# ben-hayes/neural-waveshaping-synthesis

Measured on AMD Instinct MI355X. Metric: audio_samples_per_sec, higher is better.
Workload: dtype f32 (fp16x2-split MFMA contractions = 22-bit products, fp32 accumulate; FiLM interpolation bf16x3-split MFMA = exact fp32 operands); 1 GPU; NEWT forward, vn checkpoint, FastNEWT LUT, batch 64/GPU x 500 frames (4 s @ 16 kHz), torch.rand F0/control, RNG draws on device; batch_per_gpu=64, frames=500, samples_per_utterance=64000, parallelism=batch-shard x1, exciter_opts=0, streams=2

## Files before the change

include/nws_hip.h:

```cpp
#ifndef NWS_HIP_H
#define NWS_HIP_H

#include <stddef.h>
#include <stdint.h>

#ifdef __cplusplus
extern "C" {
#endif

#define NWS_ABI_VERSION 6

#define NWS_N_HARMONICS 101
#define NWS_N_SHAPERS 64
#define NWS_HIDDEN 128
#define NWS_HOP 128
#define NWS_FIR_LEN 256
#define NWS_N_BANDS 129
#define NWS_FIR_HALF 128
#define NWS_SHAPER_WIDTH 8
#define NWS_FILM_CH 256

enum {
  NWS_OK = 0,
  NWS_ERR_UNSUPPORTED = -1,
  NWS_ERR_BAD_ARG = -2,
  NWS_ERR_WORKSPACE = -3
};

typedef struct NwsWeights {
  const float* gru_w_ih;
  const float* gru_w_hh;
  const float* gru_b_ih;
  const float* gru_b_hh;
  const float* proj_w;
  const float* proj_b;
  const float* mixer_w;
  const float* mixer_b;
  const void* mixer_frags;
  const float* newt_mlp_w[4];
  const float* newt_mlp_b[4];
  const float* newt_ln_g[3];
  const float* newt_ln_b[3];
  const float* hgen_w[4];
  const float* hgen_b[4];
  const float* hgen_ln_g[3];
  const float* hgen_ln_b[3];
  const void* mlp_frags;
  const float* shaper_in_scale;
  const float* shaper_w0;
  const float* shaper_b0;
  const float* shaper_w2;
  const float* shaper_b2;
  const float* shaper_w4;
  const float* shaper_b4;
  const float* shaper_w6;
  const float* shaper_b6;
  const float* shaper_turns;
  const float* lut;
  const float* lut_pairs;
  int32_t lut_size;
  float lut_min;
  float lut_max;
  const float* newt_out_w;
  const float* newt_out_b;
  const float* noise_window;
  int32_t exciter_opts;
  const float* exciter_bound;
} NwsWeights;
#define NWS_EXCITER_VALU_FILM 1
#define NWS_EXCITER_ONE_TERM 2
#define NWS_EXCITER_HYBRID 4
#define NWS_EXCITER_HYBRID_W 8
#define NWS_EXCITER_BANK_NOFRACT 16

int nws_abi_version(void);
size_t nws_sizeof(int which);
const char* nws_error_string(int code);

int nws_selftest_mfma(int32_t* bad_out , void* stream);

int nws_sin(const float* x, float* y, int64_t n, void* stream);

int nws_phase_carry(const float* f0, const float* f0_up, int B, int T, double* carry , void* stream);

int nws_exciter_newt(const NwsWeights* w, const float* f0, const float* f0_up, const double* carry,
                     const float* phase_u, const float* rand_phase, const float* film, int B, int T,
                     float sample_rate, float* exciter_out, float* newt_out, void* stream);
int nws_exciter_newt_add(const NwsWeights* w, const float* f0, const float* f0_up, const double* carry,
                         const float* phase_u, const float* rand_phase, const float* film, const float* add_in, int B,
                         int T, float sample_rate, float* exciter_out, float* newt_out, void* stream);

int nws_control_gru(const NwsWeights* w, const float* control, int B, int C, int T, float* gru_out, void* stream);
int nws_control_gru_state(const NwsWeights* w, const float* control, int B, int C, int T, const float* h0, float* gru_out,
                          float* hT, void* stream);
int nws_control_gru_carry(const NwsWeights* w, const float* control, const float* f0, int B, int C, int T, float* gru_out,
                          double* carry_out, void* stream);
int nws_control_gru_batched(const NwsWeights* w, const float* control, int B, int C, int T, const float* h0, float* gru_out,
                            float* hT, void* stream);

int nws_frame_mlps(const NwsWeights* w, const float* gru_out, const float* fir_design, int B, int T,
                   float* emb_out, float* film_out, float* H_out, float* fir_out, void* stream);

#define NWS_MLP_FRAGS_BYTES 1474560
int nws_mlp_frags(const NwsWeights* w, const float* fir_design , void* frags_out, void* stream);

int nws_fir_design_matrix(const float* window , float* D_out, void* stream);

int nws_fir_noise(const float* fir , const float* noise , const float* add_in ,
                  int B, int T, float* out , void* stream);
int nws_fir_noise_window(const float* fir, const float* noise, int noise_len, int origin, const float* add_in, int B, int T,
                         float* out, void* stream);

int nws_fir_noise_grad(const float* noise , const float* grad_out , int B, int T,
                       float* grad_fir , void* stream);
int nws_fir_from_h_grad(const float* grad_fir , const float* fir_design , int B, int T,
                        float* grad_H , void* stream);
int nws_sum_batch_time(const float* x , int B, int C, int T, float* out , void* stream);

typedef struct NwsReverbPlan {
  int32_t L;
  int32_t N1;
  int32_t N2;
  int32_t Lc;
  int32_t hist;
  int32_t nblk;
  int32_t reserved[2];
} NwsReverbPlan;

int nws_reverb_plan(int N, int ir_len_plus1, NwsReverbPlan* plan );
int nws_reverb_plan_serves(const NwsReverbPlan* plan, int N, int ir_len_plus1);
size_t nws_reverb_table_bytes(const NwsReverbPlan* plan);
size_t nws_reverb_spectrum_bytes(const NwsReverbPlan* plan);
size_t nws_reverb_workspace_bytes(const NwsReverbPlan* plan, int B);
int nws_reverb_build_tables(const NwsReverbPlan* plan, void* tables, void* stream);
int nws_reverb_ir_spectrum(const NwsReverbPlan* plan, const void* tables, const float* ir, int ir_len,
                           void* spectrum, void* workspace, size_t workspace_bytes, void* stream);
int nws_reverb(const NwsReverbPlan* plan, const void* tables, const void* spectrum, const float* x ,
               int B, int N, float* y , void* workspace, size_t workspace_bytes, void* stream);

size_t nws_reverb_grad_workspace_bytes(const NwsReverbPlan* plan, int B, int want_ir);
int nws_reverb_grad_x(const NwsReverbPlan* plan, const void* tables, const void* spectrum, const float* g ,
                      int B, int N, float* dx , void* workspace, size_t workspace_bytes, void* stream);
int nws_reverb_grad_ir(const NwsReverbPlan* plan, const void* tables, const float* x , const float* g ,
                       int B, int N, int ir_len, float* dir , void* workspace, size_t workspace_bytes,
                       void* stream);

int nws_reverb_linear_chunk(const NwsReverbPlan* plan, const void* tables, const void* spectrum, const float* x, int B, int M,
                            const float* tail_in, float* tail_out, int tail_len, float* y, void* workspace,
                            size_t workspace_bytes, void* stream);

size_t nws_stream_state_bytes(int B, int max_frames, int ir_len, const NwsReverbPlan* plan);
int nws_stream_reset(void* state, size_t state_bytes, void* stream);
int nws_stream_out_samples(int K, int first, int final);
long long nws_stream_noise_start(int first, long long frames_seen);
int nws_stream_noise_draws(int K, int first, long long frames_seen);
int nws_stream_step(const NwsWeights* w, const float* fir_design, const NwsReverbPlan* plan, const void* reverb_tables,
                    const void* reverb_spectrum, void* state, size_t state_bytes, int B, int max_frames, const float* f0 ,
                    const float* control , int C, int K, int first, int final, long long frames_seen,
                    long long nz_prev_start, float sample_rate, const float* phase_u, const float* rand_phase,
                    const float* noise_new, const float* noise_all, int noise_all_len, const float* ir, int ir_len,
                    float* out , float* pre_out , void* stream);
int nws_stream_reverb_tail(const NwsReverbPlan* plan, const void* reverb_tables, const void* reverb_spectrum, void* state,
                           size_t state_bytes, int B, int max_frames, int ir_len, float* tail_out ,
                           void* workspace, size_t workspace_bytes, void* stream);

size_t nws_stream_counters_offset(int B, int max_frames, int ir_len);
size_t nws_stream_slot_state_bytes(int B, int max_frames, int ir_len);
#define NWS_SLOT_START 1
#define NWS_SLOT_STOP 2
#define NWS_SLOT_RELEASE 4
#define NWS_SLOT_ACTIVE 8
int nws_stream_step_slots(const NwsWeights* w, const float* fir_design, void* state, size_t state_bytes, int B, int max_frames,
                          const float* f0 , const float* control , int C, int K, long long frames_seen,
                          long long nz_prev_start, float sample_rate, const float* phase_u, const float* rand_phase,
                          const float* noise_new, const float* noise_all, int noise_all_len, const float* ir, int ir_len,
                          const int* events , float* out , float* pre_out ,
                          void* stream);

int nws_oscillator(const float* f0_up, const double* carry, const float* phase_u, const float* rand_phase, int B, int N,
                   float sample_rate, float* out, void* stream);
int nws_newt_apply(const NwsWeights* w, const float* exciter, const float* film, int B, int T, float* out, void* stream);
int nws_td_mlp(const float* x, int B, int in_size, int hidden, int out_size, int depth, int T, const float* const* w,
               const float* const* b, const float* const* ln_g, const float* const* ln_b, float ln_eps, float leaky_slope,
               float* y, void* stream);
size_t nws_td_mlp_grad_workspace_bytes(int B, int in_size, int hidden, int out_size, int depth, int T, int want_params);
int nws_td_mlp_grad(const float* x, const float* grad_y, int B, int in_size, int hidden, int out_size, int depth, int T,
                    const float* const* w, const float* const* b, const float* const* ln_g, const float* const* ln_b,
                    float ln_eps, float leaky_slope, float* grad_x , float* const* grad_w, float* const* grad_b,
                    float* const* grad_ln_g, float* const* grad_ln_b, void* workspace, size_t workspace_bytes, void* stream);
int nws_td_layer_norm(const float* x, const float* gain, const float* bias, int B, int C, int T, float eps, float* y,
                      void* stream);
int nws_film(const float* x, const float* gamma, const float* beta, int64_t n, float* y, void* stream);
int nws_fir_from_h(const float* H, const float* fir_design , int B, int T, float* fir_out, void* stream);

int nws_shaper_table(const NwsWeights* w, int table_size, float table_min, float table_max, float* table_out, void* stream);

#define NWS_MIXER_FRAGS_BYTES 28672
int nws_mixer_frags(const float* mixer_w, const float* mixer_b, void* frags_out, void* stream);
int nws_exciter_bound(const float* mixer_w, const float* mixer_b, float* bound_out , void* stream);
#define NWS_SHAPER_TURNS_ROW 176
int nws_shaper_turns(const NwsWeights* w, float* table_out , void* stream);

int nws_lut_pairs(const float* table , int table_size, float* pairs_out , void* stream);

int nws_shaper_apply(const NwsWeights* w, const float* x, int64_t B, int64_t N, float* y, void* stream);

typedef struct NwsForwardAux {
  const float* fir_design;
  const NwsReverbPlan* plan;
  const void* reverb_tables;
  const void* reverb_spectrum;
} NwsForwardAux;

size_t nws_forward_workspace_bytes(const NwsReverbPlan* plan, int B, int T);
int nws_forward(const NwsWeights* w, const NwsForwardAux* aux, const float* f0 , const float* control ,
                int B, int C, int T, float sample_rate, const float* phase_u, const float* rand_phase,
                const float* noise, float* out , void* workspace, size_t workspace_bytes, void* stream);

size_t nws_forward_control_bytes(int B, int T);
int nws_forward_control(const NwsWeights* w, const float* f0, const float* control, int B, int C, int T, int batched_gru,
                        void* workspace, size_t workspace_bytes, void* stream);
int nws_forward_audio(const NwsWeights* w, const NwsForwardAux* aux, const float* f0, int B, int T, float sample_rate,
                      const float* phase_u, const float* rand_phase, const float* noise, float* out, void* workspace,
                      size_t workspace_bytes, void* stream);

int nws_forward_audio_ev(const NwsWeights* w, const NwsForwardAux* aux, const float* f0, int B, int T, float sample_rate,
                         const float* phase_u, const float* rand_phase, const float* noise, float* out, void* workspace,
                         size_t workspace_bytes, void* stream, void* wait_before_exciter, void* record_after_exciter);

int nws_forward_audio_pre(const NwsWeights* w, const NwsForwardAux* aux, const float* f0, int B, int T, float sample_rate,
                          const float* phase_u, const float* rand_phase, const float* noise, void* workspace,
                          size_t workspace_bytes, void* stream);
int nws_forward_reverb_rows(const NwsForwardAux* aux, int B, int T, int row0, int nrows, float* out, void* workspace,
                            size_t workspace_bytes, void* stream);
int nws_forward_audio_blocks(const NwsWeights* w, const NwsForwardAux* aux, const float* f0, int B, int T, float sample_rate,
                             const float* phase_u, const float* rand_phase, const float* noise, float* out, void* workspace,
                             size_t workspace_bytes, void* stream, const int32_t* row0, const int32_t* nrows,
                             void* const* events , int nblocks);

size_t nws_loudness_dft_bytes(int n_fft);
int nws_loudness_dft_matrix(int n_fft, float* dft_out, void* stream);
int nws_loudness_frames(int N, int hop);
size_t nws_loudness_workspace_bytes(int B, int N, int n_fft, int hop);
int nws_loudness(const float* audio, int B, int N, int n_fft, int hop, const float* dft, float amin, float top_db,
                 int normalise, float* out, void* workspace, size_t workspace_bytes, void* stream);

int nws_pyin_frames(int N, int hop);
int nws_pyin_dims(double sample_rate, double fmin, double fmax, int frame_length, int hop, int32_t* dims);
size_t nws_pyin_table_bytes(double sample_rate, double fmin, double fmax, int frame_length, int hop);
int nws_pyin_table(double sample_rate, double fmin, double fmax, int frame_length, int hop, double* table_host);
size_t nws_pyin_workspace_bytes(int B, int N, double sample_rate, double fmin, double fmax, int frame_length, int hop);
int nws_pyin_cmnd(const float* audio, int B, int N, double sample_rate, double fmin, double fmax, int frame_length, int hop,
                  float* yin, void* stream);
int nws_pyin_observe(const float* yin, int B, int T, double sample_rate, double fmin, double fmax, int frame_length, int hop,
                     const double* table, int* cand_bin, double* cand_prob, int* count, double* voiced_prob, void* stream);
int nws_pyin_viterbi(const int* cand_bin, const double* cand_prob, const int* count, const double* voiced_prob, int B, int T,
                     double sample_rate, double fmin, double fmax, int frame_length, int hop, const double* table,
                     int fill_unvoiced, float fill_value, int* states, float* f0, void* workspace, size_t workspace_bytes,
                     void* stream);
int nws_pyin(const float* audio, int B, int N, double sample_rate, double fmin, double fmax, int frame_length, int hop,
             const double* table, int fill_unvoiced, float fill_value, float* f0, double* voiced_prob, int* states,
             void* workspace, size_t workspace_bytes, void* stream);

int nws_resample_dims(int sr_in, int sr_out, int32_t* dims);
int64_t nws_resample_length(int64_t N, int sr_in, int sr_out);
size_t nws_resample_bank_bytes(int sr_in, int sr_out);
int nws_resample_bank(int sr_in, int sr_out, float* bank_host);
int nws_resample(const float* x, int B, int N, int sr_in, int sr_out, const float* bank_dev, float* y, void* stream);

int nws_mfcc_dims(double sample_rate, int n_fft, int n_mfcc, int n_mels, int32_t* dims);
size_t nws_mfcc_table_bytes(double sample_rate, int n_fft, int n_mfcc, int n_mels);
int nws_mfcc_table(double sample_rate, int n_fft, int n_mfcc, int n_mels, float* table_host);
size_t nws_mfcc_workspace_bytes(int B, int N, int n_fft, int hop, int n_mels);
int nws_mfcc(const float* audio, int B, int N, double sample_rate, int n_fft, int hop, int n_mfcc, int n_mels, const float* dft,
             const float* table, float* out, void* workspace, size_t workspace_bytes, void* stream);

#define NWS_STFT_LOSS_MAX_RES 8
size_t nws_stft_loss_dft_bytes(int n_fft, int win_length);
int nws_stft_loss_dft_matrix(int n_fft, int win_length, float* dft_out, void* stream);
size_t nws_stft_loss_workspace_bytes(int B, int N, int R, const int* n_ffts, const int* hops);
int nws_stft_loss(const float* x, const float* y, int B, int N, int R, const int* n_ffts, const int* hops, const int* win_lengths,
                  const float* const* dfts, float w_sc, float w_log_mag, float w_lin_mag, float eps, float* out, void* workspace,
                  size_t workspace_bytes, void* stream);

size_t nws_stft_grad_workspace_bytes(int B, int N, int R, const int* n_ffts, const int* hops, const int* win_lengths);
int nws_stft_grad(const float* x, const float* y, int B, int N, int R, const int* n_ffts, const int* hops, const int* win_lengths,
                  const float* const* dfts, float w_sc, float w_log_mag, float w_lin_mag, float eps, float* grad_out, void* workspace,
                  size_t workspace_bytes, void* stream);

typedef struct NwsShaperDesc {
  int32_t n_shapers, width, depth, lut_size;
  float lut_min, lut_max;
  const float* in_scale;
  const float* w[8];
  const float* b[8];
  const float* lut;
} NwsShaperDesc;

typedef struct NwsGenericModel {
  int32_t control_size;
  int32_t gru_hidden, embedding, n_harmonics, n_shapers;
  int32_t hop;
  int32_t newt_mlp_depth;
  int32_t hgen_depth, hgen_hidden;
  int32_t fir_len;
  int32_t out_channels;
  int32_t ir_len;
  float ln_eps, leaky_slope;
  const float *gru_w_ih, *gru_w_hh, *gru_b_ih, *gru_b_hh;
  const float *proj_w, *proj_b;
  const float *mixer_w, *mixer_b;
  const float* newt_mlp_w[8];
  const float* newt_mlp_b[8];
  const float* newt_ln_g[8];
  const float* newt_ln_b[8];
  const float* hgen_w[8];
  const float* hgen_b[8];
  const float* hgen_ln_g[8];
  const float* hgen_ln_b[8];
  const float *newt_out_w, *newt_out_b;
  const float* noise_window;
  const float* ir;
  NwsShaperDesc shaper;
} NwsGenericModel;

size_t nws_g_gru_workspace_bytes(int hidden);
int nws_g_gru(const float* w_ih, const float* w_hh, const float* b_ih, const float* b_hh, const float* control, int B,
              int C_total, int C_in, int hidden, int T, const float* h0, float* out, float* hT, void* workspace,
              size_t workspace_bytes, void* stream);
int nws_g_bth_to_bht(const float* x, int B, int T, int H, float* y, void* stream);
int nws_g_phase(const float* f0, const float* f0_up, int B, int T, int hop, float sample_rate, float* f0_up_out,
                float* phase_out, void* stream);
int nws_g_upsample(const float* x, int64_t rows, int T, int hop, float* y, void* stream);
int nws_g_oscillator(const float* f0_up, const float* phase, const float* phase_u, const float* rand_phase, int K, int B, int N,
                     float sample_rate, float* out, void* stream);
int nws_g_conv1x1(const float* x, const float* w, const float* bias, int B, int Cin, int Cout, int N, float* y, void* stream);
int nws_g_shaper_apply(const NwsShaperDesc* d, const float* x, int64_t rows, int64_t N, float* y, void* stream);
int nws_g_shaper_table(const NwsShaperDesc* d, int table_size, float table_min, float table_max, float* table_out, void* stream);
int nws_g_film_shaper(const NwsShaperDesc* d, const float* exciter, const float* film, int B, int T, int hop, float* out,
                      void* stream);
int nws_g_fir_design(const float* H, const float* window, int fir_len, int B, int T, float* fir_out, void* stream);
int nws_g_fir_noise(const float* fir, const float* noise, int fir_len, int hop, int B, int T, const float* add_in,
                    int add_channels, float* out, void* stream);
int nws_g_reverb_direct(const float* x, const float* ir, int ir_len, int B, int N, float* y, void* stream);

size_t nws_forward_generic_workspace_bytes(const NwsGenericModel* m, int B, int T);
int nws_forward_generic(const NwsGenericModel* m, const float* f0, const float* control, int B, int C, int T, float sample_rate,
                        const float* phase_u, const float* rand_phase, const float* noise, const NwsReverbPlan* plan,
                        const void* reverb_tables, const void* reverb_spectrum, void* reverb_workspace,
                        size_t reverb_workspace_bytes, float* out, void* workspace, size_t workspace_bytes, void* stream);


#define NWS_N_STAGES 6
int nws_profile_begin(int slots, unsigned stage_mask);
int nws_profile_collect(float* ms_out , int* n_out );
int nws_profile_end(void);

int nws_peer_push(int n, void* const* dst, const void* src, size_t bytes, void* const* streams, void* const* events);
int nws_events_wait(int n, void* const* events);
int nws_streams_wait(int n, void* const* streams);

int nws_queue_probe(void* stream_hold, void* stream_touch, int groups, int spin_us, unsigned long long* scratch, float* frac_out );

#ifdef __cplusplus
}
#endif
#endif
```

neural-waveshaping-synthesis_amd/_cops.py:

```python
from __future__ import annotations

import ctypes as C

import torch

from . import _lib
from ._lib import NwsForwardAux, NwsGenericModel, NwsReverbPlan, NwsShaperDesc, NwsWeights, check, ptr

HOP = _lib.HOP


def _stream(dev):
    return torch.cuda.current_stream(dev).cuda_stream


def _struct(desc: torch.Tensor, cls):
    return cls.from_buffer_copy(desc.numpy())


def _plan(plan: torch.Tensor | None):
    return NwsReverbPlan(*plan.tolist()[:6]) if plan is not None else None


def _ref(struct):
    return C.byref(struct) if struct is not None else None


def _aux(fir_design, plan, tables, spectrum) -> NwsForwardAux:
    aux = NwsForwardAux()
    aux.fir_design = ptr(fir_design)
    aux.plan = C.pointer(_plan(plan))
    aux.reverb_tables = ptr(tables)
    aux.reverb_spectrum = ptr(spectrum)
    return aux


def _new(like: torch.Tensor, *shape, dtype=torch.float32):
    return torch.empty(shape, dtype=dtype, device=like.device)


def _ptrs(tensors):
    return (C.c_void_p * max(1, len(tensors)))(*[t.data_ptr() for t in tensors])


def _pyin_dims(cfg, table=None):
    dims = (C.c_int32 * 8)()
    L = _lib.lib()
    if L.nws_pyin_dims(*cfg, dims) != 0:
        raise RuntimeError(f"pyin: unsupported configuration (sample_rate, fmin, fmax, frame_length, hop) = {cfg}: at most 512 "
                           "lags (frame_length <= 1024), 1024 pitch bins and a transition window of 127; hop <= frame_length")
    n = L.nws_pyin_table_bytes(*cfg) // 8
    if isinstance(table, torch.Tensor) and (not table.is_cuda or table.dtype != torch.float64 or table.numel() != n):
        raise RuntimeError("pyin: table does not belong to this configuration (expected a float64 CUDA tensor of nws_pyin_table)")
    return (*dims, n)


def _resample_dims(sr_in, sr_out):
    dims = (C.c_int32 * 6)()
    if not (1 <= sr_in < 2 ** 31 and 1 <= sr_out < 2 ** 31) or _lib.lib().nws_resample_dims(sr_in, sr_out, dims) != 0:
        raise RuntimeError(f"resample: unsupported rates {sr_in} -> {sr_out}: integers >= 1 whose weight bank (sr_out / gcd rows) "
                           "stays below 64 MB")
    return tuple(dims)


def _mfcc_dims(sample_rate, n_fft, n_mfcc, n_mels):
    dims = (C.c_int32 * 8)()
    ok = all(0 <= v < 2 ** 31 for v in (n_fft, n_mfcc, n_mels))
    if not ok or _lib.lib().nws_mfcc_dims(sample_rate, n_fft, n_mfcc, n_mels, dims) != 0:
        raise RuntimeError(f"mfcc: unsupported configuration (sample_rate {sample_rate}, n_fft {n_fft}, n_mfcc {n_mfcc}, n_mels "
                           f"{n_mels}): sample_rate > 0, n_fft a power of two in [64, 2048], 1 <= n_mfcc <= n_mels <= 1024")
    return tuple(dims)


class CtypesOps:
    def abi_version(self):
        return int(_lib.lib().nws_abi_version())

    def forward(self, wdesc, f0, control, phase_u, rand_phase, noise, fir_design, plan, reverb_tables, reverb_spectrum,
                workspace, sample_rate):
        B, Cc, T = control.shape
        aux = _aux(fir_design, plan, reverb_tables, reverb_spectrum)
        with torch.cuda.device(f0.device):
            out = _new(f0, B, T * HOP)
            check(_lib.lib().nws_forward(C.byref(_struct(wdesc, NwsWeights)), C.byref(aux), ptr(f0), ptr(control), B, Cc, T,
                                         sample_rate, ptr(phase_u), ptr(rand_phase), ptr(noise), ptr(out), ptr(workspace),
                                         workspace.numel(), _stream(f0.device)), "nws_forward")
        return out

    def forward_control(self, wdesc, f0, control, workspace, batched_gru):
        B, Cc, T = control.shape
        with torch.cuda.device(f0.device):
            check(_lib.lib().nws_forward_control(C.byref(_struct(wdesc, NwsWeights)), ptr(f0), ptr(control), B, Cc, T,
                                                 1 if batched_gru else 0, ptr(workspace), workspace.numel(), _stream(f0.device)),
                  "nws_forward_control")

    def forward_audio(self, wdesc, f0, phase_u, rand_phase, noise, fir_design, plan, reverb_tables, reverb_spectrum, workspace,
                      sample_rate, out, wait_event, record_event):
        B, _, T = f0.shape
        aux = _aux(fir_design, plan, reverb_tables, reverb_spectrum)
        with torch.cuda.device(f0.device):
            if out is None:
                out = _new(f0, B, T * HOP)
            check(_lib.lib().nws_forward_audio_ev(C.byref(_struct(wdesc, NwsWeights)), C.byref(aux), ptr(f0), B, T, sample_rate,
                                                  ptr(phase_u), ptr(rand_phase), ptr(noise), ptr(out), ptr(workspace),
                                                  workspace.numel(), _stream(f0.device), wait_event or None, record_event or None),
                  "nws_forward_audio_ev")
        return out

    def forward_audio_pre(self, wdesc, f0, phase_u, rand_phase, noise, fir_design, plan, reverb_tables, reverb_spectrum,
                          workspace, sample_rate):
        B, _, T = f0.shape
        aux = _aux(fir_design, plan, reverb_tables, reverb_spectrum)
        with torch.cuda.device(f0.device):
            check(_lib.lib().nws_forward_audio_pre(C.byref(_struct(wdesc, NwsWeights)), C.byref(aux), ptr(f0), B, T, sample_rate,
                                                   ptr(phase_u), ptr(rand_phase), ptr(noise), ptr(workspace), workspace.numel(),
                                                   _stream(f0.device)), "nws_forward_audio_pre")

    def forward_audio_blocks(self, wdesc, f0, phase_u, rand_phase, noise, fir_design, plan, reverb_tables, reverb_spectrum,
                             workspace, sample_rate, out, row0, nrows, events):
        B, _, T = f0.shape
        n = len(row0)
        aux = _aux(fir_design, plan, reverb_tables, reverb_spectrum)
        with torch.cuda.device(f0.device):
            check(_lib.lib().nws_forward_audio_blocks(C.byref(_struct(wdesc, NwsWeights)), C.byref(aux), ptr(f0), B, T, sample_rate,
                                                      ptr(phase_u), ptr(rand_phase), ptr(noise), ptr(out), ptr(workspace),
                                                      workspace.numel(), _stream(f0.device), (C.c_int32 * n)(*row0),
                                                      (C.c_int32 * n)(*nrows), (C.c_void_p * n)(*events) if events else None, n),
                  "nws_forward_audio_blocks")

    def forward_reverb_rows(self, fir_design, plan, reverb_tables, reverb_spectrum, workspace, T, row0, nrows, out):
        aux = _aux(fir_design, plan, reverb_tables, reverb_spectrum)
        with torch.cuda.device(out.device):
            check(_lib.lib().nws_forward_reverb_rows(C.byref(aux), out.shape[0], T, row0, nrows, ptr(out), ptr(workspace),
                                                     workspace.numel(), _stream(out.device)), "nws_forward_reverb_rows")

    def phase_carry(self, f0, f0_up):
        src = f0 if f0 is not None else f0_up
        B = src.shape[0]
        T = src.shape[-1] if f0 is not None else src.shape[-1] // HOP
        with torch.cuda.device(src.device):
            carry = _new(src, B, T * HOP // 32, dtype=torch.float64)
            check(_lib.lib().nws_phase_carry(ptr(f0), ptr(f0_up), B, T, ptr(carry), _stream(src.device)), "nws_phase_carry")
        return carry

    def exciter_newt(self, wdesc, f0, f0_up, carry, phase_u, rand_phase, film, sample_rate, want_exciter, want_newt):
        src = f0 if f0 is not None else f0_up
        B = src.shape[0]
        T = src.shape[-1] if f0 is not None else src.shape[-1] // HOP
        with torch.cuda.device(src.device):
            exc = _new(src, B, _lib.N_SHAPERS, T * HOP) if want_exciter else None
            out = _new(src, B, T * HOP) if want_newt else None
            check(_lib.lib().nws_exciter_newt(C.byref(_struct(wdesc, NwsWeights)), ptr(f0), ptr(f0_up), ptr(carry), ptr(phase_u),
                                              ptr(rand_phase), ptr(film), B, T, sample_rate, ptr(exc), ptr(out),
                                              _stream(src.device)), "nws_exciter_newt")
        return exc, out

    def oscillator(self, f0_up, phase_u, rand_phase, sample_rate):
        B, N = f0_up.shape
        with torch.cuda.device(f0_up.device):
            st = _stream(f0_up.device)
            carry = _new(f0_up, B, N // 32, dtype=torch.float64)
            out = _new(f0_up, B, _lib.N_HARMONICS, N)
            check(_lib.lib().nws_phase_carry(None, ptr(f0_up), B, N // HOP, ptr(carry), st), "nws_phase_carry")
            check(_lib.lib().nws_oscillator(ptr(f0_up), ptr(carry), ptr(phase_u), ptr(rand_phase), B, N, sample_rate, ptr(out), st),
                  "nws_oscillator")
        return out

    def control_gru(self, wdesc, control, h0, batched):
        B, Cc, T = control.shape
        fn = _lib.lib().nws_control_gru_batched if batched else _lib.lib().nws_control_gru_state
        with torch.cuda.device(control.device):
            out = _new(control, B, T, _lib.HIDDEN)
            hT = _new(control, B, _lib.HIDDEN)
            check(fn(C.byref(_struct(wdesc, NwsWeights)), ptr(control), B, Cc, T, ptr(h0), ptr(out), ptr(hT),
                     _stream(control.device)), "nws_control_gru")
        return out, hT

    def frame_mlps(self, wdesc, gru_out, fir_design, want_emb, want_H):
        B, T, _ = gru_out.shape
        with torch.cuda.device(gru_out.device):
            emb = _new(gru_out, B, _lib.HIDDEN, T) if want_emb else None
            film = _new(gru_out, B, T, _lib.FILM_CH)
            H = _new(gru_out, B, T, _lib.N_BANDS) if want_H else None
            fir = _new(gru_out, B, T, _lib.FIR_HALF)
            check(_lib.lib().nws_frame_mlps(C.byref(_struct(wdesc, NwsWeights)), ptr(gru_out), ptr(fir_design), B, T, ptr(emb),
                                            ptr(film), ptr(H), ptr(fir), _stream(gru_out.device)), "nws_frame_mlps")
        return emb, film, H, fir

    def fir_noise(self, fir, noise, add_in, origin):
        B, T, _ = fir.shape
        with torch.cuda.device(fir.device):
            out = _new(fir, B, T * HOP)
            if origin < 0:
                check(_lib.lib().nws_fir_noise(ptr(fir), ptr(noise), ptr(add_in), B, T, ptr(out), _stream(fir.device)), "nws_fir_noise")
            else:
                check(_lib.lib().nws_fir_noise_window(ptr(fir), ptr(noise), noise.numel(), origin, ptr(add_in), B, T, ptr(out),
                                                      _stream(fir.device)), "nws_fir_noise_window")
        return out

    def fir_from_h(self, H, fir_design):
        B, _, T = H.shape
        with torch.cuda.device(H.device):
            fir = _new(H, B, T, _lib.FIR_HALF)
            check(_lib.lib().nws_fir_from_h(ptr(H), ptr(fir_design), B, T, ptr(fir), _stream(H.device)), "nws_fir_from_h")
        return fir

    def fir_noise_grad(self, noise, grad_out):
        B, N = grad_out.shape
        T = N // HOP
        if N != T * HOP or T < 2 or noise.numel() != N - 1:
            raise RuntimeError(f"fir_noise_grad: grad_out {tuple(grad_out.shape)} must be (B, 128 T) with T >= 2 and noise "
                               f"{tuple(noise.shape)} its {N - 1} samples")
        with torch.cuda.device(grad_out.device):
            grad_fir = _new(grad_out, B, T, _lib.FIR_HALF)
            check(_lib.lib().nws_fir_noise_grad(ptr(noise), ptr(grad_out), B, T, ptr(grad_fir), _stream(grad_out.device)),
                  "nws_fir_noise_grad")
        return grad_fir

    def fir_from_h_grad(self, grad_fir, fir_design):
        B, T, _ = grad_fir.shape
        with torch.cuda.device(grad_fir.device):
            grad_H = _new(grad_fir, B, _lib.N_BANDS, T)
            check(_lib.lib().nws_fir_from_h_grad(ptr(grad_fir), ptr(fir_design), B, T, ptr(grad_H), _stream(grad_fir.device)),
                  "nws_fir_from_h_grad")
        return grad_H

    def sum_batch_time(self, x):
        B, Cc, T = x.shape
        with torch.cuda.device(x.device):
            out = _new(x, Cc)
            check(_lib.lib().nws_sum_batch_time(ptr(x), B, Cc, T, ptr(out), _stream(x.device)), "nws_sum_batch_time")
        return out

    def reverb(self, plan, tables, spectrum, x):
        B, N = x.shape
        p = _plan(plan)
        with torch.cuda.device(x.device):
            nbytes = _lib.lib().nws_reverb_workspace_bytes(C.byref(p), B)
            ws = _new(x, nbytes, dtype=torch.uint8)
            y = torch.empty_like(x)
            check(_lib.lib().nws_reverb(C.byref(p), ptr(tables), ptr(spectrum), ptr(x), B, N, ptr(y), ptr(ws), nbytes,
                                        _stream(x.device)), "nws_reverb")
        return y

    def reverb_grad_x(self, plan, tables, spectrum, grad_out):
        B, N = grad_out.shape
        p = _plan(plan)
        with torch.cuda.device(grad_out.device):
            nbytes = _lib.lib().nws_reverb_grad_workspace_bytes(C.byref(p), B, 0)
            ws = _new(grad_out, nbytes, dtype=torch.uint8)
            dx = torch.empty_like(grad_out)
            check(_lib.lib().nws_reverb_grad_x(C.byref(p), ptr(tables), ptr(spectrum), ptr(grad_out), B, N, ptr(dx), ptr(ws), nbytes,
                                               _stream(grad_out.device)), "nws_reverb_grad_x")
        return dx

    def reverb_grad_ir(self, plan, tables, x, grad_out, ir_len):
        B, N = x.shape
        if tuple(grad_out.shape) != (B, N):
            raise RuntimeError(f"reverb_grad_ir: x {tuple(x.shape)} and grad_out {tuple(grad_out.shape)} differ in shape")
        p = _plan(plan)
        with torch.cuda.device(x.device):
            nbytes = _lib.lib().nws_reverb_grad_workspace_bytes(C.byref(p), B, 1)
            ws = _new(x, nbytes, dtype=torch.uint8)
            dir_ = _new(x, ir_len)
            check(_lib.lib().nws_reverb_grad_ir(C.byref(p), ptr(tables), ptr(x), ptr(grad_out), B, N, ir_len, ptr(dir_), ptr(ws),
                                                nbytes, _stream(x.device)), "nws_reverb_grad_ir")
        return dir_

    def reverb_linear_chunk(self, plan, tables, spectrum, x, tail_in):
        B, M = x.shape
        p = _plan(plan)
        with torch.cuda.device(x.device):
            nfl = (2 * ((B + 1) // 2) + B) * p.L
            ws = _new(x, nfl)
            y, tail_out = torch.empty_like(x), torch.empty_like(tail_in)
            check(_lib.lib().nws_reverb_linear_chunk(C.byref(p), ptr(tables), ptr(spectrum), ptr(x), B, M, ptr(tail_in),
                                                     ptr(tail_out), tail_in.shape[1], ptr(y), ptr(ws), nfl * 4, _stream(x.device)),
                  "nws_reverb_linear_chunk")
        return y, tail_out

    def shaper_apply(self, wdesc, x):
        with torch.cuda.device(x.device):
            y = torch.empty_like(x)
            check(_lib.lib().nws_shaper_apply(C.byref(_struct(wdesc, NwsWeights)), ptr(x), x.shape[0], x.shape[2], ptr(y),
                                              _stream(x.device)), "nws_shaper_apply")
        return y

    def shaper_table(self, wdesc, like, size, tmin, tmax):
        with torch.cuda.device(like.device):
            table = _new(like, _lib.N_SHAPERS, size)
            check(_lib.lib().nws_shaper_table(C.byref(_struct(wdesc, NwsWeights)), size, tmin, tmax, ptr(table), _stream(like.device)),
                  "nws_shaper_table")
        return table

    def newt_apply(self, wdesc, exciter, film):
        B, _, N = exciter.shape
        T = film.shape[2]
        if film.shape[1] != _lib.FILM_CH or N != T * HOP:
            raise RuntimeError(f"NEWT: exciter {tuple(exciter.shape)} and FiLM parameters {tuple(film.shape)} disagree")
        with torch.cuda.device(exciter.device):
            out = _new(exciter, B, 1, N)
            check(_lib.lib().nws_newt_apply(C.byref(_struct(wdesc, NwsWeights)), ptr(exciter), ptr(film), B, T, ptr(out),
                                            _stream(exciter.device)), "nws_newt_apply")
        return out

    def td_mlp(self, x, weights, biases, ln_w, ln_b, eps, slope):
        B, in_size, T = x.shape
        hidden, out_size = weights[0].shape[0], weights[-1].shape[0]
        with torch.cuda.device(x.device):
            y = _new(x, B, out_size, T)
            check(_lib.lib().nws_td_mlp(ptr(x), B, in_size, hidden, out_size, len(weights), T, _ptrs(weights), _ptrs(biases),
                                        _ptrs(ln_w), _ptrs(ln_b), eps, slope, ptr(y), _stream(x.device)), "nws_td_mlp")
        return y

    def td_mlp_grad(self, x, grad_y, weights, biases, ln_w, ln_b, eps, slope, want_params):
        B, in_size, T = x.shape
        depth = len(weights)
        hidden, out_size = weights[0].shape[0], weights[-1].shape[0]
        if tuple(grad_y.shape) != (B, out_size, T):
            raise RuntimeError(f"td_mlp_grad: grad_y {tuple(grad_y.shape)} is not ({B}, {out_size}, {T})")
        if len(biases) != depth or len(ln_w) != depth - 1 or len(ln_b) != depth - 1:
            raise RuntimeError("td_mlp_grad: inconsistent layer lists")
        L = _lib.lib()
        with torch.cuda.device(x.device):
            grad_x = torch.empty_like(x)
            gw, gb, gg, gl, ws, nbytes = [], [], [], [], None, 0
            if want_params:
                gw, gb = [torch.empty_like(t) for t in weights], [torch.empty_like(t) for t in biases]
                gg, gl = [torch.empty_like(t) for t in ln_w], [torch.empty_like(t) for t in ln_b]
                nbytes = L.nws_td_mlp_grad_workspace_bytes(B, in_size, hidden, out_size, depth, T, 1)
                ws = _new(x, max(nbytes, 1), dtype=torch.uint8)
            none = None
            check(L.nws_td_mlp_grad(ptr(x), ptr(grad_y), B, in_size, hidden, out_size, depth, T, _ptrs(weights), _ptrs(biases),
                                    _ptrs(ln_w), _ptrs(ln_b), eps, slope, ptr(grad_x), _ptrs(gw) if want_params else none,
                                    _ptrs(gb) if want_params else none, _ptrs(gg) if want_params else none,
                                    _ptrs(gl) if want_params else none, ptr(ws), nbytes, _stream(x.device)), "nws_td_mlp_grad")
        return [grad_x] + gw + gb + gg + gl

    def td_layer_norm(self, x, weight, bias, eps):
        with torch.cuda.device(x.device):
            y = torch.empty_like(x)
            check(_lib.lib().nws_td_layer_norm(ptr(x), ptr(weight), ptr(bias), x.shape[0], x.shape[1], x.shape[2], eps, ptr(y),
                                               _stream(x.device)), "nws_td_layer_norm")
        return y

    def film(self, x, gamma, beta):
        with torch.cuda.device(x.device):
            y = torch.empty_like(x)
            check(_lib.lib().nws_film(ptr(x), ptr(gamma), ptr(beta), x.numel(), ptr(y), _stream(x.device)), "nws_film")
        return y
# ... 321 lines not shown
```

neural-waveshaping-synthesis_amd/_lib.py:

```python
from __future__ import annotations

import ctypes as C
import os

_HERE = os.path.dirname(os.path.abspath(__file__))
LIB_PATH = os.path.join(_HERE, "libnws_hip.so")

PROBE_LIB_PATH = os.path.join(_HERE, "libnws_probe.so")

ABI_VERSION = 6
EXCITER_VALU_FILM = 1
EXCITER_ONE_TERM = 2
EXCITER_HYBRID = 4
EXCITER_HYBRID_W = 8
EXCITER_BANK_NOFRACT = 16
N_HARMONICS = 101
N_SHAPERS = 64
HIDDEN = 128
HOP = 128
FIR_LEN = 256
FIR_HALF = 128
MLP_FRAGS_BYTES = 1474560
N_BANDS = 129
FILM_CH = 256
SHAPER_WIDTH = 8
SHAPER_TURNS_ROW = 176
FIR_DESIGN_COLS = 132

_fp = C.c_void_p


class NwsWeights(C.Structure):
    _fields_ = [
        ("gru_w_ih", _fp), ("gru_w_hh", _fp), ("gru_b_ih", _fp), ("gru_b_hh", _fp),
        ("proj_w", _fp), ("proj_b", _fp),
        ("mixer_w", _fp), ("mixer_b", _fp), ("mixer_frags", _fp),
        ("newt_mlp_w", _fp * 4), ("newt_mlp_b", _fp * 4), ("newt_ln_g", _fp * 3), ("newt_ln_b", _fp * 3),
        ("hgen_w", _fp * 4), ("hgen_b", _fp * 4), ("hgen_ln_g", _fp * 3), ("hgen_ln_b", _fp * 3),
        ("mlp_frags", _fp),
        ("shaper_in_scale", _fp),
        ("shaper_w0", _fp), ("shaper_b0", _fp), ("shaper_w2", _fp), ("shaper_b2", _fp),
        ("shaper_w4", _fp), ("shaper_b4", _fp), ("shaper_w6", _fp), ("shaper_b6", _fp), ("shaper_turns", _fp),
        ("lut", _fp), ("lut_pairs", _fp), ("lut_size", C.c_int32), ("lut_min", C.c_float), ("lut_max", C.c_float),
        ("newt_out_w", _fp), ("newt_out_b", _fp),
        ("noise_window", _fp),
        ("exciter_opts", C.c_int32),
        ("exciter_bound", _fp),
    ]


class NwsReverbPlan(C.Structure):
    _fields_ = [("L", C.c_int32), ("N1", C.c_int32), ("N2", C.c_int32), ("Lc", C.c_int32), ("hist", C.c_int32), ("nblk", C.c_int32),
                ("reserved", C.c_int32 * 2)]

    def as_tensor(self):
        import torch
        return torch.tensor([self.L, self.N1, self.N2, self.Lc, self.hist, self.nblk, 0, 0], dtype=torch.int32)


class NwsForwardAux(C.Structure):
    _fields_ = [("fir_design", _fp), ("plan", C.POINTER(NwsReverbPlan)), ("reverb_tables", _fp),
                ("reverb_spectrum", _fp)]


class NwsShaperDesc(C.Structure):
    _fields_ = [("n_shapers", C.c_int32), ("width", C.c_int32), ("depth", C.c_int32), ("lut_size", C.c_int32),
                ("lut_min", C.c_float), ("lut_max", C.c_float),
                ("in_scale", _fp), ("w", _fp * 8), ("b", _fp * 8), ("lut", _fp)]


class NwsGenericModel(C.Structure):
    _fields_ = [("control_size", C.c_int32), ("gru_hidden", C.c_int32), ("embedding", C.c_int32), ("n_harmonics", C.c_int32),
                ("n_shapers", C.c_int32), ("hop", C.c_int32), ("newt_mlp_depth", C.c_int32), ("hgen_depth", C.c_int32),
                ("hgen_hidden", C.c_int32), ("fir_len", C.c_int32), ("out_channels", C.c_int32), ("ir_len", C.c_int32),
                ("ln_eps", C.c_float), ("leaky_slope", C.c_float),
                ("gru_w_ih", _fp), ("gru_w_hh", _fp), ("gru_b_ih", _fp), ("gru_b_hh", _fp),
                ("proj_w", _fp), ("proj_b", _fp), ("mixer_w", _fp), ("mixer_b", _fp),
                ("newt_mlp_w", _fp * 8), ("newt_mlp_b", _fp * 8), ("newt_ln_g", _fp * 8), ("newt_ln_b", _fp * 8),
                ("hgen_w", _fp * 8), ("hgen_b", _fp * 8), ("hgen_ln_g", _fp * 8), ("hgen_ln_b", _fp * 8),
                ("newt_out_w", _fp), ("newt_out_b", _fp), ("noise_window", _fp), ("ir", _fp),
                ("shaper", NwsShaperDesc)]


_PYIN_CFG = (C.c_double, C.c_double, C.c_double, C.c_int, C.c_int)

_MFCC_CFG = (C.c_double, C.c_int, C.c_int, C.c_int)

_PROTOTYPES = {
    "nws_abi_version": (C.c_int, []),
    "nws_sizeof": (C.c_size_t, [C.c_int]),
    "nws_error_string": (C.c_char_p, [C.c_int]),
    "nws_selftest_mfma": (C.c_int, [_fp, _fp]),
    "nws_peer_push": (C.c_int, [C.c_int, C.POINTER(C.c_void_p), _fp, C.c_size_t, C.POINTER(C.c_void_p), C.POINTER(C.c_void_p)]),
    "nws_events_wait": (C.c_int, [C.c_int, C.POINTER(C.c_void_p)]),
    "nws_streams_wait": (C.c_int, [C.c_int, C.POINTER(C.c_void_p)]),
    "nws_queue_probe": (C.c_int, [_fp, _fp, C.c_int, C.c_int, _fp, C.POINTER(C.c_float)]),
    "nws_debug_queue_busy": (C.c_int, [C.c_int, C.c_int, _fp, _fp]),
    "nws_sin": (C.c_int, [_fp, _fp, C.c_int64, _fp]),
    "nws_phase_carry": (C.c_int, [_fp, _fp, C.c_int, C.c_int, _fp, _fp]),
    "nws_exciter_newt": (C.c_int, [C.POINTER(NwsWeights), _fp, _fp, _fp, _fp, _fp, _fp, C.c_int, C.c_int, C.c_float,
                                   _fp, _fp, _fp]),
    "nws_exciter_newt_add": (C.c_int, [C.POINTER(NwsWeights), _fp, _fp, _fp, _fp, _fp, _fp, _fp, C.c_int, C.c_int, C.c_float,
                                       _fp, _fp, _fp]),
    "nws_control_gru": (C.c_int, [C.POINTER(NwsWeights), _fp, C.c_int, C.c_int, C.c_int, _fp, _fp]),
    "nws_control_gru_state": (C.c_int, [C.POINTER(NwsWeights), _fp, C.c_int, C.c_int, C.c_int, _fp, _fp, _fp, _fp]),
    "nws_control_gru_carry": (C.c_int, [C.POINTER(NwsWeights), _fp, _fp, C.c_int, C.c_int, C.c_int, _fp, _fp, _fp]),
    "nws_control_gru_batched": (C.c_int, [C.POINTER(NwsWeights), _fp, C.c_int, C.c_int, C.c_int, _fp, _fp, _fp, _fp]),
    "nws_frame_mlps": (C.c_int, [C.POINTER(NwsWeights), _fp, _fp, C.c_int, C.c_int, _fp, _fp, _fp, _fp, _fp]),
    "nws_mlp_frags": (C.c_int, [C.POINTER(NwsWeights), _fp, _fp, _fp]),
    "nws_debug_frame_mlps_kernel": (C.c_int, [C.c_int]),
    "nws_fir_design_matrix": (C.c_int, [_fp, _fp, _fp]),
    "nws_fir_noise": (C.c_int, [_fp, _fp, _fp, C.c_int, C.c_int, _fp, _fp]),
    "nws_fir_noise_window": (C.c_int, [_fp, _fp, C.c_int, C.c_int, _fp, C.c_int, C.c_int, _fp, _fp]),
    "nws_fir_noise_grad": (C.c_int, [_fp, _fp, C.c_int, C.c_int, _fp, _fp]),
    "nws_fir_from_h_grad": (C.c_int, [_fp, _fp, C.c_int, C.c_int, _fp, _fp]),
    "nws_sum_batch_time": (C.c_int, [_fp, C.c_int, C.c_int, C.c_int, _fp, _fp]),
    "nws_reverb_linear_chunk": (C.c_int, [C.POINTER(NwsReverbPlan), _fp, _fp, _fp, C.c_int, C.c_int, _fp, _fp, C.c_int, _fp, _fp,
                                          C.c_size_t, _fp]),
    "nws_reverb_plan": (C.c_int, [C.c_int, C.c_int, C.POINTER(NwsReverbPlan)]),
    "nws_reverb_plan_serves": (C.c_int, [C.POINTER(NwsReverbPlan), C.c_int, C.c_int]),
    "nws_reverb_table_bytes": (C.c_size_t, [C.POINTER(NwsReverbPlan)]),
    "nws_reverb_spectrum_bytes": (C.c_size_t, [C.POINTER(NwsReverbPlan)]),
    "nws_reverb_workspace_bytes": (C.c_size_t, [C.POINTER(NwsReverbPlan), C.c_int]),
    "nws_reverb_build_tables": (C.c_int, [C.POINTER(NwsReverbPlan), _fp, _fp]),
    "nws_reverb_ir_spectrum": (C.c_int, [C.POINTER(NwsReverbPlan), _fp, _fp, C.c_int, _fp, _fp, C.c_size_t, _fp]),
    "nws_reverb": (C.c_int, [C.POINTER(NwsReverbPlan), _fp, _fp, _fp, C.c_int, C.c_int, _fp, _fp, C.c_size_t, _fp]),
    "nws_reverb_grad_workspace_bytes": (C.c_size_t, [C.POINTER(NwsReverbPlan), C.c_int, C.c_int]),
    "nws_reverb_grad_x": (C.c_int, [C.POINTER(NwsReverbPlan), _fp, _fp, _fp, C.c_int, C.c_int, _fp, _fp, C.c_size_t, _fp]),
    "nws_reverb_grad_ir": (C.c_int, [C.POINTER(NwsReverbPlan), _fp, _fp, _fp, C.c_int, C.c_int, C.c_int, _fp, _fp, C.c_size_t, _fp]),
    "nws_shaper_table": (C.c_int, [C.POINTER(NwsWeights), C.c_int, C.c_float, C.c_float, _fp, _fp]),
    "nws_mixer_frags": (C.c_int, [_fp, _fp, _fp, _fp]),
    "nws_exciter_bound": (C.c_int, [_fp, _fp, _fp, _fp]),
    "nws_shaper_turns": (C.c_int, [_fp, _fp, _fp]),
    "nws_lut_pairs": (C.c_int, [_fp, C.c_int, _fp, _fp]),
    "nws_shaper_apply": (C.c_int, [C.POINTER(NwsWeights), _fp, C.c_int64, C.c_int64, _fp, _fp]),
    "nws_forward_workspace_bytes": (C.c_size_t, [C.POINTER(NwsReverbPlan), C.c_int, C.c_int]),
    "nws_forward": (C.c_int, [C.POINTER(NwsWeights), C.POINTER(NwsForwardAux), _fp, _fp, C.c_int, C.c_int, C.c_int,
                              C.c_float, _fp, _fp, _fp, _fp, _fp, C.c_size_t, _fp]),
    "nws_forward_control_bytes": (C.c_size_t, [C.c_int, C.c_int]),
    "nws_forward_control": (C.c_int, [C.POINTER(NwsWeights), _fp, _fp, C.c_int, C.c_int, C.c_int, C.c_int, _fp, C.c_size_t, _fp]),
    "nws_forward_audio": (C.c_int, [C.POINTER(NwsWeights), C.POINTER(NwsForwardAux), _fp, C.c_int, C.c_int, C.c_float,
                                    _fp, _fp, _fp, _fp, _fp, C.c_size_t, _fp]),
    "nws_forward_audio_ev": (C.c_int, [C.POINTER(NwsWeights), C.POINTER(NwsForwardAux), _fp, C.c_int, C.c_int, C.c_float,
                                       _fp, _fp, _fp, _fp, _fp, C.c_size_t, _fp, _fp, _fp]),
    "nws_forward_audio_pre": (C.c_int, [C.POINTER(NwsWeights), C.POINTER(NwsForwardAux), _fp, C.c_int, C.c_int, C.c_float,
                                        _fp, _fp, _fp, _fp, C.c_size_t, _fp]),
    "nws_forward_reverb_rows": (C.c_int, [C.POINTER(NwsForwardAux), C.c_int, C.c_int, C.c_int, C.c_int, _fp, _fp, C.c_size_t, _fp]),
    "nws_forward_audio_blocks": (C.c_int, [C.POINTER(NwsWeights), C.POINTER(NwsForwardAux), _fp, C.c_int, C.c_int, C.c_float, _fp, _fp, _fp, _fp,
                                           _fp, C.c_size_t, _fp, C.POINTER(C.c_int32), C.POINTER(C.c_int32), C.POINTER(C.c_void_p), C.c_int]),
    "nws_loudness_dft_bytes": (C.c_size_t, [C.c_int]),
    "nws_loudness_dft_matrix": (C.c_int, [C.c_int, _fp, _fp]),
    "nws_loudness_frames": (C.c_int, [C.c_int, C.c_int]),
    "nws_loudness_workspace_bytes": (C.c_size_t, [C.c_int, C.c_int, C.c_int, C.c_int]),
    "nws_loudness": (C.c_int, [_fp, C.c_int, C.c_int, C.c_int, C.c_int, _fp, C.c_float, C.c_float, C.c_int, _fp, _fp,
                               C.c_size_t, _fp]),
    "nws_pyin_frames": (C.c_int, [C.c_int, C.c_int]),
    "nws_pyin_dims": (C.c_int, [*_PYIN_CFG, C.POINTER(C.c_int32)]),
    "nws_pyin_table_bytes": (C.c_size_t, [*_PYIN_CFG]),
    "nws_pyin_table": (C.c_int, [*_PYIN_CFG, C.c_void_p]),
    "nws_pyin_workspace_bytes": (C.c_size_t, [C.c_int, C.c_int, *_PYIN_CFG]),
    "nws_pyin_cmnd": (C.c_int, [_fp, C.c_int, C.c_int, *_PYIN_CFG, _fp, _fp]),
    "nws_pyin_observe": (C.c_int, [_fp, C.c_int, C.c_int, *_PYIN_CFG, _fp, _fp, _fp, _fp, _fp, _fp]),
    "nws_pyin_viterbi": (C.c_int, [_fp, _fp, _fp, _fp, C.c_int, C.c_int, *_PYIN_CFG, _fp, C.c_int, C.c_float, _fp, _fp, _fp,
                                   C.c_size_t, _fp]),
    "nws_pyin": (C.c_int, [_fp, C.c_int, C.c_int, *_PYIN_CFG, _fp, C.c_int, C.c_float, _fp, _fp, _fp, _fp, C.c_size_t, _fp]),
    "nws_resample_dims": (C.c_int, [C.c_int, C.c_int, C.POINTER(C.c_int32)]),
    "nws_resample_length": (C.c_int64, [C.c_int64, C.c_int, C.c_int]),
    "nws_resample_bank_bytes": (C.c_size_t, [C.c_int, C.c_int]),
    "nws_resample_bank": (C.c_int, [C.c_int, C.c_int, C.c_void_p]),
    "nws_resample": (C.c_int, [_fp, C.c_int, C.c_int, C.c_int, C.c_int, _fp, _fp, _fp]),
    "nws_mfcc_dims": (C.c_int, [*_MFCC_CFG, C.POINTER(C.c_int32)]),
    "nws_mfcc_table_bytes": (C.c_size_t, [*_MFCC_CFG]),
    "nws_mfcc_table": (C.c_int, [*_MFCC_CFG, C.c_void_p]),
    "nws_mfcc_workspace_bytes": (C.c_size_t, [C.c_int, C.c_int, C.c_int, C.c_int, C.c_int]),
    "nws_mfcc": (C.c_int, [_fp, C.c_int, C.c_int, C.c_double, C.c_int, C.c_int, C.c_int, C.c_int, _fp, _fp, _fp, _fp, C.c_size_t,
                           _fp]),
    "nws_stft_loss_dft_bytes": (C.c_size_t, [C.c_int, C.c_int]),
    "nws_stft_loss_dft_matrix": (C.c_int, [C.c_int, C.c_int, _fp, _fp]),
    "nws_stft_loss_workspace_bytes": (C.c_size_t, [C.c_int, C.c_int, C.c_int, C.POINTER(C.c_int), C.POINTER(C.c_int)]),
    "nws_stft_loss": (C.c_int, [_fp, _fp, C.c_int, C.c_int, C.c_int, C.POINTER(C.c_int), C.POINTER(C.c_int), C.POINTER(C.c_int),
                                C.POINTER(_fp), C.c_float, C.c_float, C.c_float, C.c_float, _fp, _fp, C.c_size_t, _fp]),
    "nws_stft_grad_workspace_bytes": (C.c_size_t, [C.c_int, C.c_int, C.c_int, C.POINTER(C.c_int), C.POINTER(C.c_int),
                                                   C.POINTER(C.c_int)]),
    "nws_stft_grad": (C.c_int, [_fp, _fp, C.c_int, C.c_int, C.c_int, C.POINTER(C.c_int), C.POINTER(C.c_int), C.POINTER(C.c_int),
                                C.POINTER(_fp), C.c_float, C.c_float, C.c_float, C.c_float, _fp, _fp, C.c_size_t, _fp]),
    "nws_oscillator": (C.c_int, [_fp, _fp, _fp, _fp, C.c_int, C.c_int, C.c_float, _fp, _fp]),
    "nws_newt_apply": (C.c_int, [C.POINTER(NwsWeights), _fp, _fp, C.c_int, C.c_int, _fp, _fp]),
    "nws_td_mlp": (C.c_int, [_fp, C.c_int, C.c_int, C.c_int, C.c_int, C.c_int, C.c_int, C.POINTER(_fp), C.POINTER(_fp),
                             C.POINTER(_fp), C.POINTER(_fp), C.c_float, C.c_float, _fp, _fp]),
    "nws_td_mlp_grad_workspace_bytes": (C.c_size_t, [C.c_int, C.c_int, C.c_int, C.c_int, C.c_int, C.c_int, C.c_int]),
    "nws_td_mlp_grad": (C.c_int, [_fp, _fp, C.c_int, C.c_int, C.c_int, C.c_int, C.c_int, C.c_int, C.POINTER(_fp), C.POINTER(_fp),
                                  C.POINTER(_fp), C.POINTER(_fp), C.c_float, C.c_float, _fp, C.POINTER(_fp), C.POINTER(_fp),
                                  C.POINTER(_fp), C.POINTER(_fp), _fp, C.c_size_t, _fp]),
    "nws_td_layer_norm": (C.c_int, [_fp, _fp, _fp, C.c_int, C.c_int, C.c_int, C.c_float, _fp, _fp]),
    "nws_film": (C.c_int, [_fp, _fp, _fp, C.c_int64, _fp, _fp]),
    "nws_fir_from_h": (C.c_int, [_fp, _fp, C.c_int, C.c_int, _fp, _fp]),
    "nws_g_gru_workspace_bytes": (C.c_size_t, [C.c_int]),
    "nws_g_gru": (C.c_int, [_fp, _fp, _fp, _fp, _fp, C.c_int, C.c_int, C.c_int, C.c_int, C.c_int, _fp, _fp, _fp, _fp,
                            C.c_size_t, _fp]),
    "nws_g_bth_to_bht": (C.c_int, [_fp, C.c_int, C.c_int, C.c_int, _fp, _fp]),
    "nws_g_phase": (C.c_int, [_fp, _fp, C.c_int, C.c_int, C.c_int, C.c_float, _fp, _fp, _fp]),
    "nws_g_upsample": (C.c_int, [_fp, C.c_int64, C.c_int, C.c_int, _fp, _fp]),
    "nws_g_oscillator": (C.c_int, [_fp, _fp, _fp, _fp, C.c_int, C.c_int, C.c_int, C.c_float, _fp, _fp]),
    "nws_g_conv1x1": (C.c_int, [_fp, _fp, _fp, C.c_int, C.c_int, C.c_int, C.c_int, _fp, _fp]),
    "nws_g_shaper_apply": (C.c_int, [C.POINTER(NwsShaperDesc), _fp, C.c_int64, C.c_int64, _fp, _fp]),
    "nws_g_shaper_table": (C.c_int, [C.POINTER(NwsShaperDesc), C.c_int, C.c_float, C.c_float, _fp, _fp]),
    "nws_g_film_shaper": (C.c_int, [C.POINTER(NwsShaperDesc), _fp, _fp, C.c_int, C.c_int, C.c_int, _fp, _fp]),
    "nws_g_fir_design": (C.c_int, [_fp, _fp, C.c_int, C.c_int, C.c_int, _fp, _fp]),
    "nws_g_fir_noise": (C.c_int, [_fp, _fp, C.c_int, C.c_int, C.c_int, C.c_int, _fp, C.c_int, _fp, _fp]),
    "nws_g_reverb_direct": (C.c_int, [_fp, _fp, C.c_int, C.c_int, C.c_int, _fp, _fp]),
    "nws_forward_generic_workspace_bytes": (C.c_size_t, [C.POINTER(NwsGenericModel), C.c_int, C.c_int]),
    "nws_debug_generic_exciter_plan": (C.c_int, [C.POINTER(NwsGenericModel), C.c_int, C.c_int, C.POINTER(C.c_int)]),
    "nws_debug_generic_gru_plan": (C.c_int, [C.c_int, C.c_int, C.POINTER(C.c_int)]),
    "nws_forward_generic": (C.c_int, [C.POINTER(NwsGenericModel), _fp, _fp, C.c_int, C.c_int, C.c_int, C.c_float, _fp, _fp, _fp,
                                      C.POINTER(NwsReverbPlan), _fp, _fp, _fp, C.c_size_t, _fp, _fp, C.c_size_t, _fp]),
    "nws_stream_state_bytes": (C.c_size_t, [C.c_int, C.c_int, C.c_int, C.POINTER(NwsReverbPlan)]),
    "nws_stream_reset": (C.c_int, [_fp, C.c_size_t, _fp]),
    "nws_stream_out_samples": (C.c_int, [C.c_int, C.c_int, C.c_int]),
    "nws_stream_noise_start": (C.c_longlong, [C.c_int, C.c_longlong]),
    "nws_stream_noise_draws": (C.c_int, [C.c_int, C.c_int, C.c_longlong]),
    "nws_stream_step": (C.c_int, [C.POINTER(NwsWeights), _fp, C.POINTER(NwsReverbPlan), _fp, _fp, _fp, C.c_size_t, C.c_int, C.c_int,
                                  _fp, _fp, C.c_int, C.c_int, C.c_int, C.c_int, C.c_longlong, C.c_longlong, C.c_float, _fp, _fp,
                                  _fp, _fp, C.c_int, _fp, C.c_int, _fp, _fp, _fp]),
    "nws_stream_counters_offset": (C.c_size_t, [C.c_int, C.c_int, C.c_int]),
    "nws_stream_slot_state_bytes": (C.c_size_t, [C.c_int, C.c_int, C.c_int]),
    "nws_stream_step_slots": (C.c_int, [C.POINTER(NwsWeights), _fp, _fp, C.c_size_t, C.c_int, C.c_int, _fp, _fp, C.c_int, C.c_int,
                                        C.c_longlong, C.c_longlong, C.c_float, _fp, _fp, _fp, _fp, C.c_int, _fp, C.c_int, _fp, _fp,
                                        _fp, _fp]),
    "nws_stream_reverb_tail": (C.c_int, [C.POINTER(NwsReverbPlan), _fp, _fp, _fp, C.c_size_t, C.c_int, C.c_int, C.c_int, _fp, _fp,
                                         C.c_size_t, _fp]),
    "nws_profile_begin": (C.c_int, [C.c_int, C.c_uint]),
    "nws_profile_collect": (C.c_int, [C.POINTER(C.c_float), C.POINTER(C.c_int)]),
    "nws_profile_end": (C.c_int, []),
}

_PROBE_PROTOTYPES = {
    "nws_coexec_pk_probe": (C.c_int, [C.c_int, C.c_int, _fp, _fp]),
    "nws_coexec_pk_probe2": (C.c_int, [C.c_int, C.c_int, _fp, _fp]),
    "nws_coexec_pk_probe_mixed": (C.c_int, [C.c_int, C.c_int, C.c_int, _fp, _fp, _fp]),
    "nws_coexec_mfma_load": (C.c_int, [C.c_int, C.c_int, C.c_int, _fp, _fp]),
}

STAGE_NAMES = ("phase_carry", "control_gru", "frame_mlps", "exciter_newt", "fir_noise", "reverb")

EXPORTED_SYMBOLS = tuple(_PROTOTYPES)
PROBE_SYMBOLS = tuple(_PROBE_PROTOTYPES)

_lib = None
_probe = None


class NwsError(RuntimeError):
    pass


def lib():
    global _lib
    if _lib is None:
        if not os.path.exists(LIB_PATH):
            raise NwsError(
                f"{LIB_PATH} not found: build the HIP kernels first "
                "(python __graft_entry__.py build, or python neural-waveshaping-synthesis_amd/build.py). "
                "There is no CPU/PyTorch fallback for the NEWT forward path.")
        handle = C.CDLL(LIB_PATH)
        for name, (res, args) in _PROTOTYPES.items():
            fn = getattr(handle, name)
            fn.restype = res
            fn.argtypes = args
        if handle.nws_abi_version() != ABI_VERSION:
            raise NwsError(f"{LIB_PATH} has ABI version {handle.nws_abi_version()}, this package binds version "
                           f"{ABI_VERSION}: rebuild it (python __graft_entry__.py build)")
        for which, struct in enumerate((NwsWeights, NwsReverbPlan, NwsForwardAux, NwsShaperDesc, NwsGenericModel)):
            if handle.nws_sizeof(which) != C.sizeof(struct):
                raise NwsError(f"struct layout mismatch for {struct.__name__}: library {handle.nws_sizeof(which)} B, "
                               f"binding {C.sizeof(struct)} B")
        _lib = handle
    return _lib


def probe_lib():
    global _probe
    if _probe is None:
        if not os.path.exists(PROBE_LIB_PATH):
            raise NwsError(f"{PROBE_LIB_PATH} not found: python neural-waveshaping-synthesis_amd/build.py builds it next to libnws_hip.so")
        handle = C.CDLL(PROBE_LIB_PATH)
        for name, (res, args) in _PROBE_PROTOTYPES.items():
            fn = getattr(handle, name)
            fn.restype = res
            fn.argtypes = args
        _probe = handle
    return _probe


# ... 17 lines not shown
```

neural-waveshaping-synthesis_amd/csrc/fir_noise.hip:

```cpp
#include "nws_common.h"
#include "fir_spectral_fft.h"

template <>
struct SpOps<f32x2> {
  static __device__ __forceinline__ f32x2 fma(f32x2 a, f32x2 b, f32x2 c) { return __builtin_elementwise_fma(a, b, c); }
  static __device__ __forceinline__ f32x2 of(float v) { return f32x2{v, v}; }
  static __device__ __forceinline__ f32x2 at(const float* p) { return *reinterpret_cast<const f32x2*>(p); }
};

namespace {

constexpr int kL = NWS_FIR_LEN;
constexpr int kHop = NWS_HOP;
constexpr int kHalf = NWS_FIR_HALF;
constexpr int kHopsPerBlock = 4;

struct NoiseLds {
  float taps[kHopsPerBlock + 1][kL];
  float taps1[kHopsPerBlock + 1][kL];
  float sig[(kHopsPerBlock + 1) * kHop + kHop];
};

__device__ __forceinline__ float padded_noise(const float* __restrict__ noise, int len, int origin, int i) {
  int s = i - origin;
  if (s < 0) s = -s;
  if (s > len - 1) s = 2 * (len - 1) - s;
  s = s < 0 ? 0 : s;
  return noise[s];
}

__device__ __forceinline__ float row_noise(const float* __restrict__ noise, int lo, int hi, int origin, int i) {
  int s = i - origin;
  if (s < lo) s = 2 * lo - s;
  if (s > hi) s = 2 * hi - s;
  s = s < 0 ? 0 : s;
  return noise[s];
}

template <bool ROWS>
__global__ __launch_bounds__(256) void fir_noise_kernel(const float* __restrict__ fir, const float* __restrict__ noise,
                                                        const float* __restrict__ add_in, int T, int len, int origin,
                                                        float* __restrict__ out, const int4* __restrict__ rows) {
  __shared__ __attribute__((aligned(16))) NoiseLds L;
  const int tid = threadIdx.x, lane = tid & 63, wave = tid >> 6;
  const int half = lane >> 5, q = lane & 31;
  const int b = blockIdx.y;
  const int t0 = blockIdx.x * kHopsPerBlock;
  const int N = T * kHop;
  int4 rb = make_int4(0, 0, 0, 0);
  if constexpr (ROWS) rb = rows[b];
  const int t_lo = ROWS ? rb.z : 0;

  for (int e = tid; e < (kHopsPerBlock + 1) * kL; e += 256) {
    const int fr = e >> 8, k = e & 255;
    const int t = t0 - 1 + fr;
    const int d = k >= kHalf ? k - kHalf : kHalf - k;
    const float v = (t >= t_lo && t < T && d < kHalf) ? fir[((size_t)b * T + t) * kHalf + d] : 0.0f;
    L.taps[fr][k] = v;
    L.taps1[fr][(k + 1) & 255] = v;
  }
  for (int e = tid; e < (kHopsPerBlock + 1) * kHop + kHop; e += 256) {
    const int i = (t0 - 1) * kHop + e;
    float v = 0.0f;
    if (i >= 0 && i < N + kL - 1) v = ROWS ? row_noise(noise, rb.x, rb.y, origin, i) : padded_noise(noise, len, origin, i);
    L.sig[e] = v;
  }
  __syncthreads();

  const int t = t0 + wave;
  if (t >= T) return;
  const int slot = wave + 1 - half;
  const int nb = half * kHop + 4 * q;
  const float* f = &L.sig[slot * kHop];
  const float* h = L.taps[slot];

  const float* h1 = L.taps1[slot];
  f32x2 a0 = {0.0f, 0.0f}, a1 = {0.0f, 0.0f}, a2 = {0.0f, 0.0f}, a3 = {0.0f, 0.0f};
  float4 hi0 = *reinterpret_cast<const float4*>(&h[nb & 255]);
  float4 hi1 = *reinterpret_cast<const float4*>(&h1[nb & 255]);
#pragma unroll 4
  for (int m0 = 0; m0 < kL; m0 += 4) {
    const float4 lo0 = *reinterpret_cast<const float4*>(&h[(nb - m0 - 4) & 255]);
    const float4 lo1 = *reinterpret_cast<const float4*>(&h1[(nb - m0 - 4) & 255]);
    const float4 fv = *reinterpret_cast<const float4*>(&f[m0]);
    const f32x2 fs0 = {fv.y, fv.x}, fs1 = {fv.w, fv.z};
    a1 = fma2(fs0, f32x2{hi0.x, hi0.y}, a1);
    a3 = fma2(fs0, f32x2{hi0.z, hi0.w}, a3);
    a1 = fma2(fs1, f32x2{lo0.z, lo0.w}, a1);
    a3 = fma2(fs1, f32x2{hi0.x, hi0.y}, a3);
    a0 = fma2(fs0, f32x2{hi1.x, hi1.y}, a0);
    a2 = fma2(fs0, f32x2{hi1.z, hi1.w}, a2);
    a0 = fma2(fs1, f32x2{lo1.z, lo1.w}, a0);
    a2 = fma2(fs1, f32x2{hi1.x, hi1.y}, a2);
    hi0 = lo0;
    hi1 = lo1;
  }
  const float y0 = a0.x + a0.y, y1 = a1.x + a1.y, y2 = a2.x + a2.y, y3 = a3.x + a3.y;
  const float o0 = y0 + nws_swap_halves(y0);
  const float o1 = y1 + nws_swap_halves(y1);
  const float o2 = y2 + nws_swap_halves(y2);
  const float o3 = y3 + nws_swap_halves(y3);
  if (half == 0) {
    const float inv = t == t_lo ? 1.0f : 0.5f;
    const size_t o = (size_t)b * N + (size_t)t * kHop + 4 * q;
    float4 r = make_float4(o0 * inv, o1 * inv, o2 * inv, o3 * inv);
    if (add_in != nullptr) {
      const float4 a = *reinterpret_cast<const float4*>(&add_in[o]);
      r.x = a.x + r.x;
      r.y = a.y + r.y;
      r.z = a.z + r.z;
      r.w = a.w + r.w;
    }
    *reinterpret_cast<float4*>(&out[o]) = r;
  }
}

constexpr int kSpWaves = 4;
constexpr int kSpUtt = 2 * kSpWaves;
constexpr int kSpPairs = 4;
constexpr int kSpHops = 2 * kSpPairs - 1;

struct SpectralLds {
  float4 sd[kSpPairs][9][16];
  float4 tw[256];
  f32x2 x[kSpWaves][kSpPairs * kSpPlane];
};

__device__ __forceinline__ void sp_wave_sync() {
  __builtin_amdgcn_fence(__ATOMIC_RELEASE, "wavefront");
  __builtin_amdgcn_wave_barrier();
  __builtin_amdgcn_fence(__ATOMIC_ACQUIRE, "wavefront");
}

template <class T>
__device__ __forceinline__ void sp_transpose(T (&v)[16], T* x, int l) {
#pragma unroll
  for (int k = 0; k < 16; ++k) x[k * kSpRow + l] = v[k];
  sp_wave_sync();
#pragma unroll
  for (int j = 0; j < 16; ++j) v[j] = x[l * kSpRow + j];
  sp_wave_sync();
}
template <bool INV, class T>
__device__ __forceinline__ void sp_fft256(C16T<T>& z, const float* tw, T* x, int l) {
  sp_pass1<INV>(z, tw);
  sp_transpose(z.re, x, l);
  sp_transpose(z.im, x, l);
  sp_dft16<INV>(z);
}

__device__ __forceinline__ f32x2 sp_shfl(f32x2 v, int src) { return f32x2{__shfl(v.x, src, 64), __shfl(v.y, src, 64)}; }
__device__ __forceinline__ f32x2 sp_select(bool c, f32x2 a, f32x2 b) { return f32x2{c ? a.x : b.x, c ? a.y : b.y}; }

__device__ __forceinline__ void sp_filter_spectrum(C16T<f32x2>& z, const f32x2 (&ua)[8], const f32x2 (&ub)[8], const float* tw,
                                                   f32x2* x, int lane, int l) {
  const int src = (lane & 48) | ((16 - l) & 15);
  const f32x2 zero = {0.0f, 0.0f};
#pragma unroll
  for (int j = 0; j < 8; ++j) {
    z.re[j] = ua[j];
    z.im[j] = ub[j];
  }
#pragma unroll
  for (int j = 8; j < 16; ++j) {
    const f32x2 ma = sp_shfl(ua[15 - j], src), mb = sp_shfl(ub[15 - j], src);
    const f32x2 oa = j == 8 ? zero : ua[(16 - j) & 7], ob = j == 8 ? zero : ub[(16 - j) & 7];
    z.re[j] = sp_select(l == 0, oa, ma);
    z.im[j] = sp_select(l == 0, ob, mb);
  }
  sp_fft256<false>(z, tw, x, l);
}

__global__ __launch_bounds__(64 * kSpWaves, 3) void fir_noise_spectral_kernel(const float* __restrict__ fir,
                                                                             const float* __restrict__ noise,
                                                                             const float* __restrict__ add_in, int B, int T, int len,
                                                                             int origin, float* __restrict__ out, int nruns, int total) {
  __shared__ __attribute__((aligned(16))) SpectralLds L;
  const int tid = threadIdx.x, lane = tid & 63, wave = tid >> 6;
  const int g = lane >> 4, l = lane & 15;
  const int per_xcd = gridDim.x >> 3;
  const int id = (blockIdx.x & 7) * per_xcd + (blockIdx.x >> 3);
  if (id >= total) return;
  const int run = id % nruns;
  const int b0 = (id / nruns) * kSpUtt + 2 * wave, b1 = b0 + 1;
  const int t0 = run * kSpHops;
  const int ta = t0 - 1 + 2 * g, tb = ta + 1;
  const int N = T * kHop;
  const bool oka = ta >= 0 && ta < T, okb = tb < T;
  const int tac = ta < 0 ? 0 : (ta < T ? ta : T - 1), tbc = tb < T ? tb : T - 1;

  const int bc0 = b0 < B ? b0 : B - 1, bc1 = b1 < B ? b1 : B - 1;
  const float* rowa0 = &fir[((size_t)bc0 * T + tac) * kHalf + l];
  const float* rowb0 = &fir[((size_t)bc0 * T + tbc) * kHalf + l];
  const float* rowa1 = &fir[((size_t)bc1 * T + tac) * kHalf + l];
  const float* rowb1 = &fir[((size_t)bc1 * T + tbc) * kHalf + l];
  f32x2 ua[8], ub[8];
#pragma unroll
  for (int j = 0; j < 8; ++j) {
    ua[j] = f32x2{rowa0[16 * j], rowa1[16 * j]};
    ub[j] = f32x2{rowb0[16 * j], rowb1[16 * j]};
  }
  {
    float c, s;
    sp_twiddle((tid & 15) * (tid >> 4), c, s);
    L.tw[tid] = make_float4(c, c, s, s);
  }
  const float* tw = reinterpret_cast<const float*>(&L.tw[l]);
  __syncthreads();

  f32x2* x = &L.x[wave][g * kSpPlane];
  if (wave == 0) {
    C16 z;
    float* xs = reinterpret_cast<float*>(x);
#pragma unroll
    for (int j = 0; j < 16; ++j) {
      const int i0 = kHop * ta + 16 * j + l, i1 = i0 + kHop;
      const bool in0 = i0 >= 0 && i0 < N + kL - 1, in1 = i1 >= 0 && i1 < N + kL - 1;
      const float v0 = padded_noise(noise, len, origin, in0 ? i0 : origin);
      const float v1 = padded_noise(noise, len, origin, in1 ? i1 : origin);
      z.re[j] = in0 ? v0 : 0.0f;
      z.im[j] = in1 ? v1 : 0.0f;
    }
    sp_fft256<false>(z, tw, xs, l);
    float mr[16], mi[16];
    auto mirror = [&](const float (&v)[16], float (&m)[16]) {
#pragma unroll
      for (int j = 0; j < 16; ++j) xs[l + 16 * j] = v[j];
      sp_wave_sync();
#pragma unroll
      for (int j = 0; j < 16; ++j) m[j] = xs[(256 - (l + 16 * j)) & 255];
      sp_wave_sync();
    };
    mirror(z.re, mr);
    mirror(z.im, mi);
    const float c = (l & 1) ? -(1.0f / 512.0f) : (1.0f / 512.0f);
#pragma unroll
    for (int j = 0; j < 9; ++j)
      L.sd[g][j][l] = make_float4(c * (z.re[j] + mr[j]), c * (z.im[j] - mi[j]), c * (z.re[j] - mr[j]), c * (z.im[j] + mi[j]));
  }
  const f32x2 zero = {0.0f, 0.0f};
#pragma unroll
  for (int j = 0; j < 8; ++j) {
    ua[j] = sp_select(oka, ua[j], zero);
    ub[j] = sp_select(okb, ub[j], zero);
  }
  C16T<f32x2> z;
  sp_filter_spectrum(z, ua, ub, tw, x, lane, l);
  __syncthreads();

  const bool has_add = add_in != nullptr;
  const bool sta = g > 0 && ta < T, stb = tb < T;
  const size_t oa0 = (size_t)bc0 * N + (size_t)tac * kHop + l, ob0 = (size_t)bc0 * N + (size_t)tbc * kHop + l;
  const size_t oa1 = (size_t)bc1 * N + (size_t)tac * kHop + l, ob1 = (size_t)bc1 * N + (size_t)tbc * kHop + l;
  f32x2 adda[8], addb[8];
  if (has_add) {
#pragma unroll
    for (int j = 0; j < 8; ++j) {
      adda[j] = f32x2{add_in[oa0 + 16 * j], add_in[oa1 + 16 * j]};
      addb[j] = f32x2{add_in[ob0 + 16 * j], add_in[ob1 + 16 * j]};
    }
  }
  const float4* sdm = &L.sd[g][l == 0 ? 1 : 0][(16 - l) & 15];
#pragma unroll
  for (int j = 0; j < 16; ++j) {
    const f32x2 ga = z.re[j], gb = z.im[j];
    if (j < 9) {
      const float4 sd = L.sd[g][j][l];
      z.re[j] = f32x2{fmaf(ga.x, sd.x, gb.x * sd.z), fmaf(ga.y, sd.x, gb.y * sd.z)};
      z.im[j] = f32x2{fmaf(ga.x, sd.y, gb.x * sd.w), fmaf(ga.y, sd.y, gb.y * sd.w)};
    } else {
      const float4 sd = sdm[(15 - j) * 16];
      z.re[j] = f32x2{fmaf(ga.x, sd.x, -(gb.x * sd.z)), fmaf(ga.y, sd.x, -(gb.y * sd.z))};
      z.im[j] = f32x2{fmaf(gb.x, sd.w, -(ga.x * sd.y)), fmaf(gb.y, sd.w, -(ga.y * sd.y))};
    }
  }
  sp_fft256<true>(z, tw, x, l);
  const float invb = tb == 0 ? 1.0f : 0.5f;
  f32x2 ha[8], hb[8];
#pragma unroll
  for (int j = 0; j < 8; ++j) {
    const f32x2 ya0 = sp_select(oka, z.re[j], zero), ya1 = sp_select(oka, z.re[j + 8], zero);
    const f32x2 yb0 = sp_select(okb, z.im[j], zero), yb1 = sp_select(okb, z.im[j + 8], zero);
    const f32x2 prev = sp_shfl(yb1, (lane - 16) & 63);
    ha[j] = (ya0 + prev) * 0.5f;
    hb[j] = (yb0 + ya1) * invb;
    if (has_add) {
      ha[j] = adda[j] + ha[j];
      hb[j] = addb[j] + hb[j];
    }
  }
  if (sta) {
    if (b0 < B) {
#pragma unroll
      for (int j = 0; j < 8; ++j) out[oa0 + 16 * j] = ha[j].x;
    }
    if (b1 < B) {
#pragma unroll
      for (int j = 0; j < 8; ++j) out[oa1 + 16 * j] = ha[j].y;
    }
  }
  if (stb) {
    if (b0 < B) {
#pragma unroll
      for (int j = 0; j < 8; ++j) out[ob0 + 16 * j] = hb[j].x;
    }
    if (b1 < B) {
#pragma unroll
      for (int j = 0; j < 8; ++j) out[ob1 + 16 * j] = hb[j].y;
    }
  }
}

}

extern "C" int nws_fir_noise_window(const float* fir, const float* noise, int noise_len, int origin, const float* add_in,
                                    int B, int T, float* out, void* stream) {
  if (!fir || !noise || !out || B <= 0 || T <= 0 || noise_len < 2 || origin < 0) return NWS_ERR_BAD_ARG;
  if (B > 65535) return NWS_ERR_UNSUPPORTED;
  if (B >= 16) {
    const long long nruns = (T + kSpHops - 1) / kSpHops, total = nruns * ((B + kSpUtt - 1) / kSpUtt);
    if (total > (1ll << 30)) return NWS_ERR_UNSUPPORTED;
    const dim3 grid((unsigned)(8 * ((total + 7) / 8)));
    fir_noise_spectral_kernel<<<grid, 64 * kSpWaves, 0, (hipStream_t)stream>>>(fir, noise, add_in, B, T, noise_len, origin, out,
                                                                             (int)nruns, (int)total);
    NWS_CHECK_LAUNCH();
    return NWS_OK;
  }
  const dim3 grid((T + kHopsPerBlock - 1) / kHopsPerBlock, B);
  fir_noise_kernel<false><<<grid, 256, 0, (hipStream_t)stream>>>(fir, noise, add_in, T, noise_len, origin, out, nullptr);
  NWS_CHECK_LAUNCH();
  return NWS_OK;
}

extern "C" int nws_fir_noise_window_rows(const float* fir, const float* noise, int origin, const int4* rows, int B, int T,
                                         float* out, void* stream) {
  if (!fir || !noise || !out || !rows || B <= 0 || T <= 0 || origin < 0) return NWS_ERR_BAD_ARG;
  if (B > 65535) return NWS_ERR_UNSUPPORTED;
  const dim3 grid((T + kHopsPerBlock - 1) / kHopsPerBlock, B);
  fir_noise_kernel<true><<<grid, 256, 0, (hipStream_t)stream>>>(fir, noise, nullptr, T, 0, origin, out, rows);
  NWS_CHECK_LAUNCH();
  return NWS_OK;
}

extern "C" int nws_fir_noise(const float* fir, const float* noise, const float* add_in, int B, int T, float* out,
                             void* stream) {
  return nws_fir_noise_window(fir, noise, T * kHop - 1, kL / 2, add_in, B, T, out, stream);
}
```

neural-waveshaping-synthesis_amd/csrc/forward.hip:

```cpp
#include "nws_common.h"

namespace {

struct Carve {
  char* p;
  size_t left;
  bool ok = true;
  void* take(size_t bytes) {
    bytes = (bytes + 255) & ~size_t(255);
    if (bytes > left) {
      ok = false;
      return nullptr;
    }
    void* r = p;
    p += bytes;
    left -= bytes;
    return r;
  }
};

size_t aligned(size_t b) { return (b + 255) & ~size_t(255); }

constexpr int kStages = 6;
struct Profile {
  int slots = 0;
  int used = 0;
  unsigned mask = 0;
  hipEvent_t* ev = nullptr;
} g_prof;

inline hipEvent_t* prof_events(int stage) {
  if (g_prof.ev == nullptr || g_prof.used >= g_prof.slots || !(g_prof.mask & (1u << stage))) return nullptr;
  return g_prof.ev + ((size_t)g_prof.used * kStages + stage) * 2;
}

}

extern "C" {

size_t nws_forward_workspace_bytes(const NwsReverbPlan* plan, int B, int T) {
  if (!plan || B <= 0 || T <= 0) return 0;
  const size_t N = (size_t)T * NWS_HOP;
  size_t total = 0;
  total += aligned((size_t)B * (N / 32) * sizeof(double));
  total += aligned((size_t)B * T * NWS_HIDDEN * sizeof(float));
  total += aligned((size_t)B * T * NWS_FILM_CH * sizeof(float));
  total += aligned((size_t)B * T * NWS_FIR_HALF * sizeof(float));
  total += aligned((size_t)B * N * sizeof(float));
  total += aligned((size_t)B * N * sizeof(float));
  total += aligned(nws_reverb_workspace_bytes(plan, B));
  return total;
}

}

namespace {

struct Arena {
  double* carry;
  float *gru_out, *film, *fir, *noise_out, *pre;
  void* rv_ws;
  size_t rv_bytes;
  bool ok;
};

Arena carve_arena(const NwsReverbPlan* plan, void* workspace, size_t bytes, int B, int T, bool head_only) {
  const size_t N = (size_t)T * NWS_HOP;
  Carve cv{static_cast<char*>(workspace), bytes};
  Arena a{};
  a.carry = static_cast<double*>(cv.take((size_t)B * (N / 32) * sizeof(double)));
  a.gru_out = static_cast<float*>(cv.take((size_t)B * T * NWS_HIDDEN * sizeof(float)));
  if (!head_only) {
    a.film = static_cast<float*>(cv.take((size_t)B * T * NWS_FILM_CH * sizeof(float)));
    a.fir = static_cast<float*>(cv.take((size_t)B * T * NWS_FIR_HALF * sizeof(float)));
    a.noise_out = static_cast<float*>(cv.take((size_t)B * N * sizeof(float)));
    a.pre = static_cast<float*>(cv.take((size_t)B * N * sizeof(float)));
    a.rv_bytes = nws_reverb_workspace_bytes(plan, B);
    a.rv_ws = cv.take(a.rv_bytes);
  }
  a.ok = cv.ok;
  return a;
}

#define NWS_STAGE(idx, call)                                   \
  do {                                                         \
    hipEvent_t* e__ = prof_events(idx);                        \
    if (e__) (void)hipEventRecord(e__[0], st);                 \
    rc = (call);                                               \
    if (e__) (void)hipEventRecord(e__[1], st);                 \
    if (rc != NWS_OK) return rc;                               \
  } while (0)

int control_half(const NwsWeights* w, const float* f0, const float* control, int B, int C, int T, int batched_gru,
                 const Arena& a, void* stream) {
  hipStream_t st = (hipStream_t)stream;
  int rc = NWS_OK;
  if (batched_gru) {
    NWS_STAGE(0, nws_phase_carry(f0, nullptr, B, T, a.carry, stream));
    NWS_STAGE(1, nws_control_gru_batched(w, control, B, C, T, nullptr, a.gru_out, nullptr, stream));
  } else {
    NWS_STAGE(0, NWS_OK);
    NWS_STAGE(1, nws_control_gru_carry(w, control, f0, B, C, T, a.gru_out, a.carry, stream));
  }
  return NWS_OK;
}

int audio_half(const NwsWeights* w, const NwsForwardAux* aux, const float* f0, int B, int T, float sample_rate,
               const float* phase_u, const float* rand_phase, const float* noise, float* out, const Arena& a, void* stream,
               void* wait_before_exciter = nullptr, void* record_after_exciter = nullptr, bool with_reverb = true) {
  hipStream_t st = (hipStream_t)stream;
  int rc = NWS_OK;
  const size_t N = (size_t)T * NWS_HOP;
  NWS_STAGE(2, nws_frame_mlps(w, a.gru_out, aux->fir_design, B, T, nullptr, a.film, nullptr, a.fir, stream));
  NWS_STAGE(4, nws_fir_noise(a.fir, noise, nullptr, B, T, a.noise_out, stream));
  if (wait_before_exciter != nullptr) {
    const hipError_t e = hipStreamWaitEvent(st, (hipEvent_t)wait_before_exciter, 0);
    if (e != hipSuccess) return (int)e;
  }
  NWS_STAGE(3, nws_exciter_newt_add(w, f0, nullptr, a.carry, phase_u, rand_phase, a.film, a.noise_out, B, T, sample_rate, nullptr, a.pre, stream));
  if (record_after_exciter != nullptr) {
    const hipError_t e = hipEventRecord((hipEvent_t)record_after_exciter, st);
    if (e != hipSuccess) return (int)e;
  }
  if (with_reverb)
    NWS_STAGE(5, nws_reverb(aux->plan, aux->reverb_tables, aux->reverb_spectrum, a.pre, B, (int)N, out, a.rv_ws, a.rv_bytes, stream));
  if (g_prof.ev != nullptr && g_prof.used < g_prof.slots) ++g_prof.used;
  return NWS_OK;
}
#undef NWS_STAGE

bool aux_ok(const NwsForwardAux* aux) {
  return aux && aux->plan && aux->fir_design && aux->reverb_tables && aux->reverb_spectrum;
}

}

extern "C" {

size_t nws_sizeof(int which) {
  switch (which) {
    case 0: return sizeof(NwsWeights);
    case 1: return sizeof(NwsReverbPlan);
    case 2: return sizeof(NwsForwardAux);
    case 3: return sizeof(NwsShaperDesc);
    case 4: return sizeof(NwsGenericModel);
    default: return 0;
  }
}

size_t nws_forward_control_bytes(int B, int T) {
  if (B <= 0 || T <= 0) return 0;
  const size_t N = (size_t)T * NWS_HOP;
  return aligned((size_t)B * (N / 32) * sizeof(double)) + aligned((size_t)B * T * NWS_HIDDEN * sizeof(float));
}

int nws_forward(const NwsWeights* w, const NwsForwardAux* aux, const float* f0, const float* control, int B, int C,
                int T, float sample_rate, const float* phase_u, const float* rand_phase, const float* noise, float* out,
                void* workspace, size_t workspace_bytes, void* stream) {
  if (!w || !aux_ok(aux)) return NWS_ERR_BAD_ARG;
  if (!f0 || !control || !phase_u || !rand_phase || !noise || !out || !workspace) return NWS_ERR_BAD_ARG;
  if (B <= 0 || T < 2 || C < 2) return NWS_ERR_BAD_ARG;
  if (T > (1 << 23) || !nws_reverb_plan_serves(aux->plan, T * NWS_HOP, 0)) return NWS_ERR_BAD_ARG;
  const Arena a = carve_arena(aux->plan, workspace, workspace_bytes, B, T, false);
  if (!a.ok) return NWS_ERR_WORKSPACE;
  const int rc = control_half(w, f0, control, B, C, T, 0, a, stream);
  if (rc != NWS_OK) return rc;
  return audio_half(w, aux, f0, B, T, sample_rate, phase_u, rand_phase, noise, out, a, stream);
}

int nws_forward_control(const NwsWeights* w, const float* f0, const float* control, int B, int C, int T, int batched_gru,
                        void* workspace, size_t workspace_bytes, void* stream) {
  if (!w || !f0 || !control || !workspace) return NWS_ERR_BAD_ARG;
  if (B <= 0 || T < 2 || C < 2) return NWS_ERR_BAD_ARG;
  const Arena a = carve_arena(nullptr, workspace, workspace_bytes, B, T, true);
  if (!a.ok) return NWS_ERR_WORKSPACE;
  return control_half(w, f0, control, B, C, T, batched_gru, a, stream);
}

int nws_forward_audio(const NwsWeights* w, const NwsForwardAux* aux, const float* f0, int B, int T, float sample_rate,
                      const float* phase_u, const float* rand_phase, const float* noise, float* out, void* workspace,
                      size_t workspace_bytes, void* stream) {
  if (!w || !aux_ok(aux)) return NWS_ERR_BAD_ARG;
  if (!f0 || !phase_u || !rand_phase || !noise || !out || !workspace) return NWS_ERR_BAD_ARG;
  if (B <= 0 || T < 2) return NWS_ERR_BAD_ARG;
  if (T > (1 << 23) || !nws_reverb_plan_serves(aux->plan, T * NWS_HOP, 0)) return NWS_ERR_BAD_ARG;
  const Arena a = carve_arena(aux->plan, workspace, workspace_bytes, B, T, false);
  if (!a.ok) return NWS_ERR_WORKSPACE;
  return audio_half(w, aux, f0, B, T, sample_rate, phase_u, rand_phase, noise, out, a, stream);
}

int nws_forward_audio_ev(const NwsWeights* w, const NwsForwardAux* aux, const float* f0, int B, int T, float sample_rate,
                         const float* phase_u, const float* rand_phase, const float* noise, float* out, void* workspace,
                         size_t workspace_bytes, void* stream, void* wait_before_exciter, void* record_after_exciter) {
  if (!w || !aux_ok(aux)) return NWS_ERR_BAD_ARG;
  if (!f0 || !phase_u || !rand_phase || !noise || !out || !workspace) return NWS_ERR_BAD_ARG;
  if (B <= 0 || T < 2) return NWS_ERR_BAD_ARG;
  if (T > (1 << 23) || !nws_reverb_plan_serves(aux->plan, T * NWS_HOP, 0)) return NWS_ERR_BAD_ARG;
  const Arena a = carve_arena(aux->plan, workspace, workspace_bytes, B, T, false);
  if (!a.ok) return NWS_ERR_WORKSPACE;
  return audio_half(w, aux, f0, B, T, sample_rate, phase_u, rand_phase, noise, out, a, stream, wait_before_exciter,
                    record_after_exciter);
}

int nws_forward_audio_pre(const NwsWeights* w, const NwsForwardAux* aux, const float* f0, int B, int T, float sample_rate,
                          const float* phase_u, const float* rand_phase, const float* noise, void* workspace,
                          size_t workspace_bytes, void* stream) {
  if (!w || !aux_ok(aux)) return NWS_ERR_BAD_ARG;
  if (!f0 || !phase_u || !rand_phase || !noise || !workspace) return NWS_ERR_BAD_ARG;
  if (B <= 0 || T < 2) return NWS_ERR_BAD_ARG;
  if (T > (1 << 23) || !nws_reverb_plan_serves(aux->plan, T * NWS_HOP, 0)) return NWS_ERR_BAD_ARG;
  const Arena a = carve_arena(aux->plan, workspace, workspace_bytes, B, T, false);
  if (!a.ok) return NWS_ERR_WORKSPACE;
  return audio_half(w, aux, f0, B, T, sample_rate, phase_u, rand_phase, noise, nullptr, a, stream, nullptr, nullptr, false);
}

int nws_forward_reverb_rows(const NwsForwardAux* aux, int B, int T, int row0, int nrows, float* out ,
                            void* workspace, size_t workspace_bytes, void* stream) {
  if (!aux_ok(aux) || !out || !workspace || B <= 0 || T < 2 || row0 < 0 || nrows <= 0 || row0 + nrows > B) return NWS_ERR_BAD_ARG;
  const Arena a = carve_arena(aux->plan, workspace, workspace_bytes, B, T, false);
  if (!a.ok) return NWS_ERR_WORKSPACE;
  const size_t N = (size_t)T * NWS_HOP;
  if (row0 & 1) return NWS_ERR_BAD_ARG;
  const size_t per_pair = 2 * (size_t)aux->plan->nblk * (size_t)aux->plan->L * sizeof(float);
  char* rv = static_cast<char*>(a.rv_ws) + (size_t)(row0 / 2) * per_pair;
  const size_t left = a.rv_bytes - (size_t)(row0 / 2) * per_pair;
  return nws_reverb(aux->plan, aux->reverb_tables, aux->reverb_spectrum, a.pre + (size_t)row0 * N, nrows, (int)N, out + (size_t)row0 * N, rv,
                    left, stream);
}

int nws_forward_audio_blocks(const NwsWeights* w, const NwsForwardAux* aux, const float* f0, int B, int T, float sample_rate,
                             const float* phase_u, const float* rand_phase, const float* noise, float* out, void* workspace,
                             size_t workspace_bytes, void* stream, const int32_t* row0, const int32_t* nrows, void* const* events,
                             int nblocks) {
  if (!row0 || !nrows || nblocks <= 0 || !out) return NWS_ERR_BAD_ARG;
  int next = 0;
  for (int q = 0; q < nblocks; ++q) {
    if (row0[q] != next || nrows[q] <= 0 || ((nrows[q] & 1) && q != nblocks - 1)) return NWS_ERR_BAD_ARG;
    next += nrows[q];
  }
  if (next != B) return NWS_ERR_BAD_ARG;
  int rc = nws_forward_audio_pre(w, aux, f0, B, T, sample_rate, phase_u, rand_phase, noise, workspace, workspace_bytes, stream);
  if (rc != NWS_OK) return rc;
  for (int q = 0; q < nblocks; ++q) {
    rc = nws_forward_reverb_rows(aux, B, T, row0[q], nrows[q], out, workspace, workspace_bytes, stream);
    if (rc != NWS_OK) return rc;
    if (events != nullptr && events[q] != nullptr) {
      const hipError_t e = hipEventRecord((hipEvent_t)events[q], (hipStream_t)stream);
      if (e != hipSuccess) return (int)e;
    }
  }
  return NWS_OK;
}

int nws_profile_begin(int slots, unsigned stage_mask) {
  nws_profile_end();
  if (slots <= 0) return NWS_ERR_BAD_ARG;
  g_prof.ev = new hipEvent_t[(size_t)slots * kStages * 2];
  for (size_t i = 0; i < (size_t)slots * kStages * 2; ++i) {
    hipError_t e = hipEventCreateWithFlags(&g_prof.ev[i], hipEventDisableSystemFence);
    if (e != hipSuccess) return (int)e;
  }
  g_prof.slots = slots;
  g_prof.used = 0;
  g_prof.mask = stage_mask;
  return NWS_OK;
}

int nws_profile_collect(float* ms_out, int* n_out) {
  if (!ms_out || !n_out) return NWS_ERR_BAD_ARG;
  const int n = g_prof.used;
  for (int i = 0; i < n; ++i)
    for (int s = 0; s < kStages; ++s) {
      float ms = -1.0f;
      if (g_prof.mask & (1u << s)) {
        hipEvent_t* e = g_prof.ev + ((size_t)i * kStages + s) * 2;
        hipError_t err = hipEventSynchronize(e[1]);
        if (err != hipSuccess) return (int)err;
        err = hipEventElapsedTime(&ms, e[0], e[1]);
        if (err != hipSuccess) return (int)err;
      }
      ms_out[(size_t)i * kStages + s] = ms;
    }
  *n_out = n;
  g_prof.used = g_prof.slots;
  return NWS_OK;
}

int nws_profile_end(void) {
  if (g_prof.ev != nullptr) {
    for (size_t i = 0; i < (size_t)g_prof.slots * kStages * 2; ++i) (void)hipEventDestroy(g_prof.ev[i]);
    delete[] g_prof.ev;
  }
  g_prof = Profile();
  return NWS_OK;
}

}
```

neural-waveshaping-synthesis_amd/csrc/nws_common.h:

```cpp
#pragma once

#include <hip/hip_runtime.h>
#include <stdint.h>

#include "../../include/nws_hip.h"
#include "../../include/nws_hip_debug.h"

#define NWS_WAVE 64

typedef float f32x2 __attribute__((ext_vector_type(2)));
typedef float f32x4 __attribute__((ext_vector_type(4)));
typedef float f32x16 __attribute__((ext_vector_type(16)));

#define NWS_CHECK_LAUNCH()                      \
  do {                                          \
    hipError_t e__ = hipGetLastError();         \
    if (e__ != hipSuccess) return (int)e__;     \
  } while (0)

inline bool nws_first_use_on_device(unsigned long long& mask) {
  int d = 0;
  if (hipGetDevice(&d) != hipSuccess || d < 0 || d > 63) return true;
  if ((mask >> d) & 1ull) return false;
  mask |= 1ull << d;
// ... 215 lines not shown
  }
  hs[tid] = 256 * p + tid < ir_len ? ir[256 * p + tid] : 0.0f;
  __syncthreads();
  float acc0 = 0.0f, acc1 = 0.0f;
#pragma unroll 8
  for (int i = 0; i < 256; i += 4) {
    const float4 h4 = *reinterpret_cast<const float4*>(&hs[i]);
    acc0 = nws_fma_scalar(h4.x, xs[tid + 255 - i], acc0);
    acc1 = nws_fma_scalar(h4.y, xs[tid + 254 - i], acc1);
    acc0 = nws_fma_scalar(h4.z, xs[tid + 253 - i], acc0);
    acc1 = nws_fma_scalar(h4.w, xs[tid + 252 - i], acc1);
  }
  return nws_add_scalar(acc0, acc1);
}

struct NwsStreamNoiseWin {
  float* nzwin;
  const float* noise_new;
  const float* noise_all;
  long long* counters;
  int nz_shift, nz_keep, n_new, noise_all_len, first, K;
};
template <int NT, bool ADVANCE = true>
__device__ __forceinline__ void nws_stream_noise_window_block(const NwsStreamNoiseWin& Z, int tid) {
  const int Tw = Z.first ? Z.K : Z.K + 1;
  const long long F = Z.counters[1] + Z.counters[3];
  __syncthreads();
  if (ADVANCE && tid == 0) {
    Z.counters[0] += Z.counters[2];
    Z.counters[1] = F;
    Z.counters[2] = 0;
    Z.counters[3] = 0;
  }
  if (Z.noise_all != nullptr) {
    const long long A0 = Z.first ? 0 : F - 1;
    const long long start = A0 <= 0 ? 0 : 128 * (A0 - 1);
    const int want = 128 * (Tw + 1) + 1;
    for (int i = tid; i < want; i += NT) Z.nzwin[i] = start + i < Z.noise_all_len ? Z.noise_all[start + i] : 0.0f;
  } else {
    for (int i0 = 0; i0 < Z.nz_keep; i0 += NT) {
      const int i = i0 + tid;
      const float v = i < Z.nz_keep ? Z.nzwin[i + Z.nz_shift] : 0.0f;
      __syncthreads();
      if (i < Z.nz_keep) Z.nzwin[i] = v;
      __syncthreads();
    }
    for (int i = tid; i < Z.n_new; i += NT) Z.nzwin[Z.nz_keep + i] = Z.noise_new[i];
  }
}

struct NwsStreamSide {
  const float* ring;
  const float* ir;
  float* partial;
  const long long* counters;
  int ir_len, M, B, parts;
  const float* f0_new;
  float* prev_f0;
  const float* prev_film;
  const float* prev_fir;
  double* S;
  float* f0_w;
  float* film_w;
  float* fir_w;
  double* carry;
  int K, first, final;
  long long* gru_flag;
  long long* counters_rw;
  const float* gru_out;
  int out_T, out_off;
  NwsStreamNoiseWin win;
  const int* ev;
  int* vage;
  int4* nzrows;
  float* film_junk;
  float* fir_junk;
  int n_len;
};

__device__ __forceinline__ void nws_stream_head_block_slots(const NwsStreamSide& H, int b, int tid, double* wave_tot) {
  const int K = H.K, Tw = H.first ? K : K + 1, off = H.first ? 0 : 1;
  const int e = H.ev[b];
  for (int i = tid; i < Tw; i += 256) {
    int s;
    if (e & NWS_SLOT_RELEASE) s = -1;
    else if (!(e & NWS_SLOT_ACTIVE)) s = -2;
    else if (e & NWS_SLOT_START) s = i < off ? 0 : i - off;
    else s = i < off ? -1 : i - off;
    H.f0_w[(size_t)b * Tw + i] = s >= 0 ? H.f0_new[(size_t)b * K + s] : (s == -1 ? H.prev_f0[b] : 0.0f);
  }
  const bool hold = (e & NWS_SLOT_RELEASE) != 0;
  const int rows = !(e & NWS_SLOT_ACTIVE) ? Tw : ((e & NWS_SLOT_START) ? 0 : off);
  for (int i = tid; i < rows * NWS_FILM_CH; i += 256) {
    const int c = i % NWS_FILM_CH;
    H.film_w[(size_t)b * Tw * NWS_FILM_CH + i] = (hold || (e & NWS_SLOT_ACTIVE)) ? H.prev_film[(size_t)b * NWS_FILM_CH + c] : 0.0f;
  }
  for (int i = tid; i < rows * NWS_FIR_HALF; i += 256) {
    const int c = i % NWS_FIR_HALF;
    H.fir_w[(size_t)b * Tw * NWS_FIR_HALF + i] = (hold || (e & NWS_SLOT_ACTIVE)) ? H.prev_fir[(size_t)b * NWS_FIR_HALF + c] : 0.0f;
  }
  if (tid == 0) {
    const int age = (e & NWS_SLOT_START) ? 0 : H.vage[b];
    const int lo = 256 - 128 * (age < 2 ? age : 2);
    const int hi = (e & NWS_SLOT_STOP) ? 128 * (Tw + 1) - 2 : H.n_len - 1;
    const bool live = !H.first && (e & NWS_SLOT_ACTIVE);
    H.nzrows[b] = make_int4(live ? lo : 0, live ? hi : H.n_len - 1, (!H.first && (e & NWS_SLOT_START)) ? 1 : 0, 0);
    H.vage[b] = (e & NWS_SLOT_ACTIVE) ? (age + K < (1 << 20) ? age + K : (1 << 20)) : 0;
  }
  __syncthreads();
  if (tid == 0) H.prev_f0[b] = H.f0_w[(size_t)b * Tw + Tw - 1];
  nws_phase_carry_block<4>(H.f0_w, nullptr, Tw, H.carry, b, tid, wave_tot);
  __syncthreads();
  const int nch = 4 * Tw;
  double* cb = H.carry + (size_t)b * nch;
  if (!H.first) {
    const bool start = (e & NWS_SLOT_START) != 0;
    const double base = start ? cb[4] : cb[2], s0 = start ? 0.0 : H.S[b];
    __syncthreads();
    for (int c = tid; c < nch; c += 256) cb[c] = start ? cb[c] - base : s0 + (cb[c] - base);
    __syncthreads();
  }
  if (!H.final && tid == 0) H.S[b] = cb[nch - 2];
}

__device__ __forceinline__ void nws_stream_head_block(const NwsStreamSide& H, int b, int tid, double* wave_tot) {
  if (H.ev != nullptr) {
    nws_stream_head_block_slots(H, b, tid, wave_tot);
    return;
  }
  const int K = H.K, Tw = H.first ? K : K + 1, off = H.first ? 0 : 1;
  for (int i = tid; i < Tw; i += 256) H.f0_w[(size_t)b * Tw + i] = (i < off) ? H.prev_f0[b] : H.f0_new[(size_t)b * K + i - off];
  if (off) {
    for (int c = tid; c < NWS_FILM_CH; c += 256) H.film_w[(size_t)b * Tw * NWS_FILM_CH + c] = H.prev_film[(size_t)b * NWS_FILM_CH + c];
    for (int c = tid; c < NWS_FIR_HALF; c += 256) H.fir_w[(size_t)b * Tw * NWS_FIR_HALF + c] = H.prev_fir[(size_t)b * NWS_FIR_HALF + c];
  }
  __syncthreads();
  if (tid == 0) H.prev_f0[b] = H.f0_new[(size_t)b * K + K - 1];
  nws_phase_carry_block<4>(H.f0_w, nullptr, Tw, H.carry, b, tid, wave_tot);
  __syncthreads();
  const int nch = 4 * Tw;
  double* cb = H.carry + (size_t)b * nch;
  if (!H.first) {
    const double base = cb[2], s0 = H.S[b];
    __syncthreads();
    for (int c = tid; c < nch; c += 256) cb[c] = s0 + (cb[c] - base);
    __syncthreads();
  }
  if (!H.final && tid == 0) H.S[b] = cb[nch - 2];
}

extern "C" __attribute__((visibility("hidden"))) int nws_fir_noise_window_rows(const float* fir, const float* noise, int origin,
                                                                               const int4* rows, int B, int T, float* out,
                                                                               void* stream);
extern "C" __attribute__((visibility("hidden"))) int nws_control_gru_stream(const NwsWeights* w, const float* control, int B, int C,
                                                                            int T, const float* h0, float* gru_out, float* hT,
                                                                            const NwsStreamSide* side, void* stream);
extern "C" __attribute__((visibility("hidden"))) int nws_frame_mlps_stream(const NwsWeights* w, const float* gru_out, int B, int T,
                                                                           float* film_w, float* fir_w, int out_T, int out_off,
                                                                           const NwsStreamNoiseWin* win, void* stream);
extern "C" __attribute__((visibility("hidden"))) int nws_stft_power_pass(const float* audio, int B, int N, int n_fft, int hop,
                                                                         const float* dft, float* power, unsigned* max_bits,
                                                                         void* stream);
```

neural-waveshaping-synthesis_amd/csrc/torch_ops.cpp:

```cpp
#include <ATen/ATen.h>
#include <ATen/hip/impl/HIPGuardImplMasqueradingAsCUDA.h>
#include <ATen/hip/impl/HIPStreamMasqueradingAsCUDA.h>
#include <torch/library.h>

#include <algorithm>
#include <cstdlib>
#include <tuple>
#include <vector>

#include "../../include/nws_hip.h"
#include "../../include/nws_hip_debug.h"

namespace {

using at::Tensor;
using OptTensor = c10::optional<at::Tensor>;

const NwsWeights* weights_of(const Tensor& wdesc) {
  TORCH_CHECK(wdesc.device().is_cpu() && wdesc.scalar_type() == at::kByte && wdesc.is_contiguous() &&
                  (size_t)wdesc.numel() == sizeof(NwsWeights),
              "wdesc: expected a contiguous CPU uint8 tensor of ", sizeof(NwsWeights), " bytes (one NwsWeights struct), got ",
              wdesc.sizes(), " ", wdesc.scalar_type(), " on ", wdesc.device());
  return reinterpret_cast<const NwsWeights*>(wdesc.data_ptr());
}

void check_dev(const Tensor& t, const char* name, at::ScalarType st = at::kFloat) {
  TORCH_CHECK(t.is_cuda(), name, " lives on ", t.device(),
              ": the NEWT forward path only runs as HIP kernels on an AMD GPU (there is no CPU fallback)");
  TORCH_CHECK(t.scalar_type() == st, name, ": expected ", st, ", got ", t.scalar_type());
  TORCH_CHECK(t.is_contiguous(), name, ": expected a contiguous tensor");
}

void check_same_device(const Tensor& a, const char* an, const Tensor& b, const char* bn) {
  TORCH_CHECK(a.device() == b.device(), an, " is on ", a.device(), " but ", bn, " is on ", b.device(),
              ": all tensors of one call must live on the same GPU");
}

void nws_check(int rc, const char* what) {
  TORCH_CHECK(rc == NWS_OK, what, " failed (", rc, "): ", nws_error_string(rc));
}

const float* fptr(const OptTensor& t) { return t.has_value() ? t->data_ptr<float>() : nullptr; }

struct Launch {
  c10::hip::HIPGuardMasqueradingAsCUDA guard;
  void* stream;
  explicit Launch(const Tensor& t)
      : guard(t.device()), stream(c10::hip::getCurrentHIPStreamMasqueradingAsCUDA(t.device().index()).stream()) {}
};

NwsReverbPlan plan_of(const Tensor& plan) {
  TORCH_CHECK(plan.device().is_cpu() && plan.scalar_type() == at::kInt && plan.is_contiguous() && plan.numel() == 8,
              "plan: expected a CPU int32 tensor [L, N1, N2, Lc, hist, nblk, 0, 0] (the NwsReverbPlan of nws_reverb_plan)");
  const int32_t* p = plan.data_ptr<int32_t>();
  return NwsReverbPlan{p[0], p[1], p[2], p[3], p[4], p[5], {p[6], p[7]}};
}

void check_reverb_buffers(const NwsReverbPlan& plan, const Tensor& tables, const Tensor& spectrum) {
  TORCH_CHECK(plan.L > 0 && plan.N1 > 0 && plan.N2 > 0 && (int64_t)plan.N1 * plan.N2 == plan.L, "plan: inconsistent [L, N1, N2] = [",
              plan.L, ", ", plan.N1, ", ", plan.N2, "]");
  TORCH_CHECK((size_t)tables.numel() * tables.element_size() == nws_reverb_table_bytes(&plan), "reverb_tables: ",
              (size_t)tables.numel() * tables.element_size(), " bytes, the plan (L = ", plan.L, ") needs ", nws_reverb_table_bytes(&plan));
  TORCH_CHECK((size_t)spectrum.numel() * spectrum.element_size() == nws_reverb_spectrum_bytes(&plan), "reverb_spectrum: ",
              (size_t)spectrum.numel() * spectrum.element_size(), " bytes, the plan (L = ", plan.L, ") needs ",
              nws_reverb_spectrum_bytes(&plan), " (Sre | Sim | ir_)");
}

struct Aux {
  NwsReverbPlan plan;
  NwsForwardAux aux;
  Aux(const Tensor& fir_design, const Tensor& plan_t, const Tensor& tables, const Tensor& spectrum) : plan(plan_of(plan_t)) {
    check_dev(fir_design, "fir_design");
    check_dev(tables, "reverb_tables");
    check_dev(spectrum, "reverb_spectrum");
    TORCH_CHECK(fir_design.numel() == NWS_FIR_LEN * 132, "fir_design: expected (256, 132)");
    check_reverb_buffers(plan, tables, spectrum);
    aux.fir_design = fir_design.data_ptr<float>();
    aux.plan = &plan;
    aux.reverb_tables = tables.data_ptr();
    aux.reverb_spectrum = spectrum.data_ptr();
  }
};

void check_inputs(const Tensor& f0, const Tensor& control, int64_t& B, int64_t& C, int64_t& T) {
  check_dev(f0, "f0");
  check_dev(control, "control");
  check_same_device(f0, "f0", control, "control");
  TORCH_CHECK(f0.dim() == 3 && f0.size(1) == 1, "f0: expected (B, 1, T), got ", f0.sizes());
  TORCH_CHECK(control.dim() == 3 && control.size(1) >= 2, "control: expected (B, C>=2, T), got ", control.sizes());
  B = f0.size(0);
  T = f0.size(2);
  C = control.size(1);
  TORCH_CHECK(control.size(0) == B && control.size(2) == T, "f0 ", f0.sizes(), " and control ", control.sizes(),
              " disagree on batch / frames");
  TORCH_CHECK(T >= 2, "need at least 2 control frames (reflect padding of the noise STFT, generators.py:31)");
}

void check_draws(const Tensor& phase_u, const Tensor& rand_phase, const Tensor& noise, int64_t T, const Tensor& like) {
  check_dev(phase_u, "phase_u");
  check_dev(rand_phase, "rand_phase");
  check_dev(noise, "noise");
  check_same_device(like, "f0", phase_u, "phase_u");
  check_same_device(like, "f0", noise, "noise");
  check_same_device(like, "f0", rand_phase, "osc.rand_phase");
  TORCH_CHECK(phase_u.numel() == NWS_N_HARMONICS, "phase_u: expected 101 elements, got ", phase_u.sizes());
  TORCH_CHECK(rand_phase.numel() == NWS_N_HARMONICS, "rand_phase: expected 101 elements, got ", rand_phase.sizes());
  TORCH_CHECK(noise.numel() == NWS_HOP * T - 1, "noise: expected ", NWS_HOP * T - 1, " elements, got ", noise.sizes());
}

struct AudioShape {
  int64_t B, T;
  AudioShape(const Tensor& f0, const Tensor& phase_u, const Tensor& rand_phase, const Tensor& noise, const Tensor& workspace) {
    check_dev(f0, "f0");
    TORCH_CHECK(f0.dim() == 3 && f0.size(1) == 1 && f0.size(2) >= 2, "f0: expected (B, 1, T>=2), got ", f0.sizes());
    B = f0.size(0);
    T = f0.size(2);
    check_draws(phase_u, rand_phase, noise, T, f0);
    check_dev(workspace, "workspace", at::kByte);
    check_same_device(f0, "f0", workspace, "workspace");
  }
};

struct AudioArgs : AudioShape, Aux {
  AudioArgs(const Tensor& f0, const Tensor& phase_u, const Tensor& rand_phase, const Tensor& noise, const Tensor& fir_design,
            const Tensor& plan_t, const Tensor& tables, const Tensor& spectrum, const Tensor& workspace)
      : AudioShape(f0, phase_u, rand_phase, noise, workspace), Aux(fir_design, plan_t, tables, spectrum) {}
};

Tensor forward(const Tensor& wdesc, const Tensor& f0, const Tensor& control, const Tensor& phase_u, const Tensor& rand_phase,
               const Tensor& noise, const Tensor& fir_design, const Tensor& plan, const Tensor& reverb_tables,
               const Tensor& reverb_spectrum, Tensor& workspace, double sample_rate) {
  const NwsWeights* w = weights_of(wdesc);
  int64_t B, C, T;
  check_inputs(f0, control, B, C, T);
  check_draws(phase_u, rand_phase, noise, T, f0);
  check_dev(workspace, "workspace", at::kByte);
  check_same_device(f0, "f0", workspace, "workspace");
  Aux a(fir_design, plan, reverb_tables, reverb_spectrum);
  check_same_device(f0, "f0", fir_design, "the model's tables");
  Launch L(f0);
  Tensor out = at::empty({B, T * NWS_HOP}, f0.options());
  nws_check(nws_forward(w, &a.aux, f0.data_ptr<float>(), control.data_ptr<float>(), (int)B, (int)C, (int)T, (float)sample_rate,
                        phase_u.data_ptr<float>(), rand_phase.data_ptr<float>(), noise.data_ptr<float>(), out.data_ptr<float>(),
                        workspace.data_ptr(), (size_t)workspace.numel(), L.stream),
            "nws_forward");
  return out;
}

void forward_control(const Tensor& wdesc, const Tensor& f0, const Tensor& control, Tensor& workspace, bool batched_gru) {
  const NwsWeights* w = weights_of(wdesc);
  int64_t B, C, T;
  check_inputs(f0, control, B, C, T);
  check_dev(workspace, "workspace", at::kByte);
  check_same_device(f0, "f0", workspace, "workspace");
  Launch L(f0);
  nws_check(nws_forward_control(w, f0.data_ptr<float>(), control.data_ptr<float>(), (int)B, (int)C, (int)T, batched_gru ? 1 : 0,
                                workspace.data_ptr(), (size_t)workspace.numel(), L.stream),
            "nws_forward_control");
}

Tensor forward_audio(const Tensor& wdesc, const Tensor& f0, const Tensor& phase_u, const Tensor& rand_phase, const Tensor& noise,
                     const Tensor& fir_design, const Tensor& plan, const Tensor& reverb_tables, const Tensor& reverb_spectrum,
                     Tensor& workspace, double sample_rate, const OptTensor& out_opt, int64_t wait_event, int64_t record_event) {
  const NwsWeights* w = weights_of(wdesc);
  AudioArgs a(f0, phase_u, rand_phase, noise, fir_design, plan, reverb_tables, reverb_spectrum, workspace);
  const int64_t B = a.B, T = a.T;
  Launch L(f0);
  Tensor out;
  if (out_opt.has_value()) {
    out = *out_opt;
    check_dev(out, "out");
    check_same_device(f0, "f0", out, "out");
    TORCH_CHECK(out.dim() == 2 && out.size(0) == B && out.size(1) == T * NWS_HOP, "out: expected (", B, ", ", T * NWS_HOP, ")");
  } else {
    out = at::empty({B, T * NWS_HOP}, f0.options());
  }
  nws_check(nws_forward_audio_ev(w, &a.aux, f0.data_ptr<float>(), (int)B, (int)T, (float)sample_rate, phase_u.data_ptr<float>(),
                                 rand_phase.data_ptr<float>(), noise.data_ptr<float>(), out.data_ptr<float>(), workspace.data_ptr(),
                                 (size_t)workspace.numel(), L.stream, reinterpret_cast<void*>(wait_event),
                                 reinterpret_cast<void*>(record_event)),
            "nws_forward_audio");
  return out;
}

void forward_audio_pre(const Tensor& wdesc, const Tensor& f0, const Tensor& phase_u, const Tensor& rand_phase, const Tensor& noise,
                       const Tensor& fir_design, const Tensor& plan, const Tensor& reverb_tables, const Tensor& reverb_spectrum,
                       Tensor& workspace, double sample_rate) {
  const NwsWeights* w = weights_of(wdesc);
  AudioArgs a(f0, phase_u, rand_phase, noise, fir_design, plan, reverb_tables, reverb_spectrum, workspace);
  const int64_t B = a.B, T = a.T;
  Launch L(f0);
  nws_check(nws_forward_audio_pre(w, &a.aux, f0.data_ptr<float>(), (int)B, (int)T, (float)sample_rate, phase_u.data_ptr<float>(),
                                  rand_phase.data_ptr<float>(), noise.data_ptr<float>(), workspace.data_ptr(),
                                  (size_t)workspace.numel(), L.stream), "nws_forward_audio_pre");
}

void forward_reverb_rows(const Tensor& fir_design, const Tensor& plan, const Tensor& reverb_tables, const Tensor& reverb_spectrum,
                         Tensor& workspace, int64_t T, int64_t row0, int64_t nrows, Tensor& out) {
  check_dev(workspace, "workspace", at::kByte);
  check_dev(out, "out");
  check_same_device(out, "out", workspace, "workspace");
  TORCH_CHECK(out.dim() == 2 && out.size(1) == T * NWS_HOP, "out: expected (B, ", T * NWS_HOP, "), got ", out.sizes());
  TORCH_CHECK(row0 >= 0 && nrows > 0 && row0 + nrows <= out.size(0) && (row0 & 1) == 0, "forward_reverb_rows: bad row block");
  Aux a(fir_design, plan, reverb_tables, reverb_spectrum);
  Launch L(out);
  nws_check(nws_forward_reverb_rows(&a.aux, (int)out.size(0), (int)T, (int)row0, (int)nrows, out.data_ptr<float>(), workspace.data_ptr(),
                                    (size_t)workspace.numel(), L.stream), "nws_forward_reverb_rows");
}

void forward_audio_blocks(const Tensor& wdesc, const Tensor& f0, const Tensor& phase_u, const Tensor& rand_phase, const Tensor& noise,
                          const Tensor& fir_design, const Tensor& plan, const Tensor& reverb_tables, const Tensor& reverb_spectrum,
                          Tensor& workspace, double sample_rate, Tensor& out, at::IntArrayRef row0, at::IntArrayRef nrows,
                          at::IntArrayRef events) {
  const NwsWeights* w = weights_of(wdesc);
  AudioArgs a(f0, phase_u, rand_phase, noise, fir_design, plan, reverb_tables, reverb_spectrum, workspace);
  const int64_t B = a.B, T = a.T;
  check_dev(out, "out");
  check_same_device(f0, "f0", out, "out");
  TORCH_CHECK(out.dim() == 2 && out.size(0) == B && out.size(1) == T * NWS_HOP && out.is_contiguous(), "out: expected a contiguous (", B, ", ",
              T * NWS_HOP, "), got ", out.sizes());
  TORCH_CHECK(!row0.empty() && row0.size() == nrows.size() && (events.empty() || events.size() == row0.size()),
              "forward_audio_blocks: row0 / nrows / events must have one entry per block");
  std::vector<int32_t> r0(row0.begin(), row0.end()), nr(nrows.begin(), nrows.end());
  std::vector<void*> ev(events.size());
  for (size_t q = 0; q < events.size(); ++q) ev[q] = reinterpret_cast<void*>(static_cast<uintptr_t>(events[q]));
  Launch L(f0);
  nws_check(nws_forward_audio_blocks(w, &a.aux, f0.data_ptr<float>(), (int)B, (int)T, (float)sample_rate, phase_u.data_ptr<float>(),
                                     rand_phase.data_ptr<float>(), noise.data_ptr<float>(), out.data_ptr<float>(), workspace.data_ptr(),
                                     (size_t)workspace.numel(), L.stream, r0.data(), nr.data(), ev.empty() ? nullptr : ev.data(), (int)r0.size()),
            "nws_forward_audio_blocks");
}

Tensor phase_carry(const OptTensor& f0, const OptTensor& f0_up) {
  TORCH_CHECK(f0.has_value() != f0_up.has_value(), "phase_carry: give exactly one of f0 (B, T) and f0_up (B, 128 T)");
  const Tensor& src = f0.has_value() ? *f0 : *f0_up;
  check_dev(src, f0.has_value() ? "f0" : "f0_up");
  TORCH_CHECK(src.dim() == 2, "phase_carry: expected a 2-D tensor, got ", src.sizes());
  const int64_t B = src.size(0);
  TORCH_CHECK(f0.has_value() || src.size(1) % NWS_HOP == 0, "f0_up: the sample count must be a multiple of ", NWS_HOP);
  const int64_t T = f0.has_value() ? src.size(1) : src.size(1) / NWS_HOP;
  Launch L(src);
  Tensor carry = at::empty({B, T * NWS_HOP / 32}, src.options().dtype(at::kDouble));
  nws_check(nws_phase_carry(fptr(f0), fptr(f0_up), (int)B, (int)T, carry.data_ptr<double>(), L.stream), "nws_phase_carry");
  return carry;
}

std::tuple<Tensor, Tensor> exciter_newt(const Tensor& wdesc, const OptTensor& f0, const OptTensor& f0_up, const Tensor& carry,
                                        const Tensor& phase_u, const Tensor& rand_phase, const OptTensor& film,
                                        double sample_rate, bool want_exciter, bool want_newt) {
  const NwsWeights* w = weights_of(wdesc);
  TORCH_CHECK(f0.has_value() != f0_up.has_value(), "exciter_newt: give exactly one of f0 (B, T) and f0_up (B, 128 T)");
  TORCH_CHECK(want_exciter || want_newt, "exciter_newt: nothing to compute");
  const Tensor& src = f0.has_value() ? *f0 : *f0_up;
  check_dev(src, "f0");
  check_dev(carry, "carry", at::kDouble);
  check_dev(phase_u, "phase_u");
  check_dev(rand_phase, "rand_phase");
  check_same_device(src, "f0", carry, "carry");
  check_same_device(src, "f0", phase_u, "phase_u");
  TORCH_CHECK(src.dim() == 2, "exciter_newt: f0 / f0_up must be 2-D, got ", src.sizes());
  const int64_t B = src.size(0);
  const int64_t T = f0.has_value() ? src.size(1) : src.size(1) / NWS_HOP;
  const int64_t N = T * NWS_HOP;
  TORCH_CHECK(f0.has_value() || src.size(1) == N, "f0_up: the sample count must be a multiple of ", NWS_HOP);
  TORCH_CHECK(carry.numel() == B * (N / 32), "carry: expected (", B, ", ", N / 32, "), got ", carry.sizes());
  TORCH_CHECK(phase_u.numel() == NWS_N_HARMONICS && rand_phase.numel() == NWS_N_HARMONICS, "phase_u / rand_phase: 101 elements each");
  if (want_newt) {
    TORCH_CHECK(film.has_value(), "exciter_newt: the waveshaper bank needs the FiLM parameters (film)");
    check_dev(*film, "film");
    check_same_device(src, "f0", *film, "film");
    TORCH_CHECK(film->numel() == B * T * NWS_FILM_CH, "film: expected (", B, ", ", T, ", 256), got ", film->sizes());
  }
  Launch L(src);
  Tensor exc = want_exciter ? at::empty({B, NWS_N_SHAPERS, N}, src.options()) : at::empty({0}, src.options());
  Tensor out = want_newt ? at::empty({B, N}, src.options()) : at::empty({0}, src.options());
  nws_check(nws_exciter_newt(w, fptr(f0), fptr(f0_up), carry.data_ptr<double>(), phase_u.data_ptr<float>(),
                             rand_phase.data_ptr<float>(), fptr(film), (int)B, (int)T, (float)sample_rate,
                             want_exciter ? exc.data_ptr<float>() : nullptr, want_newt ? out.data_ptr<float>() : nullptr, L.stream),
            "nws_exciter_newt");
  return {exc, out};
}

Tensor oscillator(const Tensor& f0_up, const Tensor& phase_u, const Tensor& rand_phase, double sample_rate) {
  check_dev(f0_up, "f0");
  check_dev(phase_u, "phase_u");
  check_dev(rand_phase, "rand_phase");
  check_same_device(f0_up, "f0", phase_u, "phase_u");
  check_same_device(f0_up, "f0", rand_phase, "rand_phase");
  TORCH_CHECK(f0_up.dim() == 2, "HarmonicOscillator: expected f0 of shape (B, N), got ", f0_up.sizes());
  TORCH_CHECK(f0_up.size(1) % NWS_HOP == 0 && f0_up.size(1) > 0,
              "HarmonicOscillator on the HIP path: the sample count must be a multiple of ", NWS_HOP, ", got ", f0_up.size(1));
  TORCH_CHECK(phase_u.numel() == NWS_N_HARMONICS && rand_phase.numel() == NWS_N_HARMONICS,
              "kernels are specialised for 101 harmonics (gin/models/newt.gin)");
  const int64_t B = f0_up.size(0), N = f0_up.size(1);
  Launch L(f0_up);
  Tensor carry = at::empty({B, N / 32}, f0_up.options().dtype(at::kDouble));
  nws_check(nws_phase_carry(nullptr, f0_up.data_ptr<float>(), (int)B, (int)(N / NWS_HOP), carry.data_ptr<double>(), L.stream),
            "nws_phase_carry");
  Tensor out = at::empty({B, NWS_N_HARMONICS, N}, f0_up.options());
  nws_check(nws_oscillator(f0_up.data_ptr<float>(), carry.data_ptr<double>(), phase_u.data_ptr<float>(),
                           rand_phase.data_ptr<float>(), (int)B, (int)N, (float)sample_rate, out.data_ptr<float>(), L.stream),
            "nws_oscillator");
  return out;
}

std::tuple<Tensor, Tensor> control_gru(const Tensor& wdesc, const Tensor& control, const OptTensor& h0, bool batched) {
  const NwsWeights* w = weights_of(wdesc);
  check_dev(control, "control");
  TORCH_CHECK(control.dim() == 3 && control.size(1) >= 2, "control: expected (B, C>=2, T), got ", control.sizes());
  const int64_t B = control.size(0), C = control.size(1), T = control.size(2);
  TORCH_CHECK(T >= 1, "control: need at least one frame");
  if (h0.has_value()) {
    check_dev(*h0, "h0");
    check_same_device(control, "control", *h0, "h0");
    TORCH_CHECK(h0->numel() == B * NWS_HIDDEN, "h0: expected (", B, ", 128), got ", h0->sizes());
  }
  Launch L(control);
  Tensor out = at::empty({B, T, NWS_HIDDEN}, control.options());
  Tensor hT = at::empty({B, NWS_HIDDEN}, control.options());
  if (batched)
    nws_check(nws_control_gru_batched(w, control.data_ptr<float>(), (int)B, (int)C, (int)T, fptr(h0), out.data_ptr<float>(),
                                      hT.data_ptr<float>(), L.stream), "nws_control_gru_batched");
  else
    nws_check(nws_control_gru_state(w, control.data_ptr<float>(), (int)B, (int)C, (int)T, fptr(h0), out.data_ptr<float>(),
                                    hT.data_ptr<float>(), L.stream), "nws_control_gru_state");
  return {out, hT};
}

std::tuple<Tensor, Tensor, Tensor, Tensor> frame_mlps(const Tensor& wdesc, const Tensor& gru_out, const Tensor& fir_design,
                                                       bool want_emb, bool want_H) {
  const NwsWeights* w = weights_of(wdesc);
  check_dev(gru_out, "gru_out");
  check_dev(fir_design, "fir_design");
  check_same_device(gru_out, "gru_out", fir_design, "fir_design");
  TORCH_CHECK(gru_out.dim() == 3 && gru_out.size(2) == NWS_HIDDEN, "gru_out: expected (B, T, 128), got ", gru_out.sizes());
  TORCH_CHECK(fir_design.numel() == NWS_FIR_LEN * 132, "fir_design: expected (256, 132)");
  const int64_t B = gru_out.size(0), T = gru_out.size(1);
  Launch L(gru_out);
  const auto o = gru_out.options();
  Tensor emb = want_emb ? at::empty({B, NWS_HIDDEN, T}, o) : at::empty({0}, o);
  Tensor film = at::empty({B, T, NWS_FILM_CH}, o);
  Tensor H = want_H ? at::empty({B, T, NWS_N_BANDS}, o) : at::empty({0}, o);
  Tensor fir = at::empty({B, T, NWS_FIR_HALF}, o);
  nws_check(nws_frame_mlps(w, gru_out.data_ptr<float>(), fir_design.data_ptr<float>(), (int)B, (int)T,
                           want_emb ? emb.data_ptr<float>() : nullptr, film.data_ptr<float>(),
                           want_H ? H.data_ptr<float>() : nullptr, fir.data_ptr<float>(), L.stream), "nws_frame_mlps");
  return {emb, film, H, fir};
}

Tensor fir_noise(const Tensor& fir, const Tensor& noise, const OptTensor& add_in, int64_t origin) {
  check_dev(fir, "fir");
  check_dev(noise, "noise");
  check_same_device(fir, "fir", noise, "noise");
  TORCH_CHECK(fir.dim() == 3 && fir.size(2) == NWS_FIR_HALF, "fir: expected (B, T, 128) upper half-taps (nws_frame_mlps), got ", fir.sizes());
  const int64_t B = fir.size(0), T = fir.size(1);
  if (add_in.has_value()) {
    check_dev(*add_in, "add_in");
    check_same_device(fir, "fir", *add_in, "add_in");
    TORCH_CHECK(add_in->numel() == B * T * NWS_HOP, "add_in: expected (", B, ", ", T * NWS_HOP, "), got ", add_in->sizes());
  }
  Launch L(fir);
  Tensor out = at::empty({B, T * NWS_HOP}, fir.options());
  if (origin < 0) {
    TORCH_CHECK(noise.numel() == T * NWS_HOP - 1, "noise: expected ", T * NWS_HOP - 1, " samples, got ", noise.sizes());
    nws_check(nws_fir_noise(fir.data_ptr<float>(), noise.data_ptr<float>(), fptr(add_in), (int)B, (int)T, out.data_ptr<float>(),
                            L.stream), "nws_fir_noise");
  } else {
    nws_check(nws_fir_noise_window(fir.data_ptr<float>(), noise.data_ptr<float>(), (int)noise.numel(), (int)origin, fptr(add_in),
                                   (int)B, (int)T, out.data_ptr<float>(), L.stream), "nws_fir_noise_window");
  }
  return out;
}

Tensor fir_from_h(const Tensor& H, const Tensor& fir_design) {
  check_dev(H, "H");
  check_dev(fir_design, "fir_design");
  check_same_device(H, "H", fir_design, "fir_design");
  TORCH_CHECK(H.dim() == 3 && H.size(1) == NWS_N_BANDS, "FIRNoiseSynth: expected H of shape (B, 129, T), got ", H.sizes());
  TORCH_CHECK(fir_design.numel() == NWS_FIR_LEN * 132, "fir_design: expected (256, 132)");
  Launch L(H);
  Tensor fir = at::empty({H.size(0), H.size(2), NWS_FIR_HALF}, H.options());
  nws_check(nws_fir_from_h(H.data_ptr<float>(), fir_design.data_ptr<float>(), (int)H.size(0), (int)H.size(2), fir.data_ptr<float>(),
                           L.stream), "nws_fir_from_h");
  return fir;
}

Tensor fir_noise_grad(const Tensor& noise, const Tensor& grad_out) {
  check_dev(noise, "noise");
  check_dev(grad_out, "grad_out");
  check_same_device(grad_out, "grad_out", noise, "noise");
  TORCH_CHECK(grad_out.dim() == 2 && grad_out.size(1) % NWS_HOP == 0 && grad_out.size(1) >= 2 * NWS_HOP,
              "fir_noise_grad: expected grad_out (B, 128 T) with T >= 2, got ", grad_out.sizes());
  const int64_t B = grad_out.size(0), T = grad_out.size(1) / NWS_HOP;
  TORCH_CHECK(noise.numel() == T * NWS_HOP - 1, "noise: expected ", T * NWS_HOP - 1, " samples, got ", noise.sizes());
  Launch L(grad_out);
  Tensor grad_fir = at::empty({B, T, NWS_FIR_HALF}, grad_out.options());
  nws_check(nws_fir_noise_grad(noise.data_ptr<float>(), grad_out.data_ptr<float>(), (int)B, (int)T, grad_fir.data_ptr<float>(),
                               L.stream), "nws_fir_noise_grad");
  return grad_fir;
}

Tensor fir_from_h_grad(const Tensor& grad_fir, const Tensor& fir_design) {
  check_dev(grad_fir, "grad_fir");
  check_dev(fir_design, "fir_design");
  check_same_device(grad_fir, "grad_fir", fir_design, "fir_design");
  TORCH_CHECK(grad_fir.dim() == 3 && grad_fir.size(2) == NWS_FIR_HALF, "fir_from_h_grad: expected grad_fir (B, T, 128), got ", grad_fir.sizes());
  TORCH_CHECK(fir_design.numel() == NWS_FIR_LEN * 132, "fir_design: expected (256, 132)");
  Launch L(grad_fir);
  Tensor grad_H = at::empty({grad_fir.size(0), NWS_N_BANDS, grad_fir.size(1)}, grad_fir.options());
  nws_check(nws_fir_from_h_grad(grad_fir.data_ptr<float>(), fir_design.data_ptr<float>(), (int)grad_fir.size(0), (int)grad_fir.size(1),
                                grad_H.data_ptr<float>(), L.stream), "nws_fir_from_h_grad");
  return grad_H;
}

Tensor sum_batch_time(const Tensor& x) {
  check_dev(x, "x");
  TORCH_CHECK(x.dim() == 3, "sum_batch_time: expected (B, C, T), got ", x.sizes());
  Launch L(x);
  Tensor out = at::empty({x.size(1)}, x.options());
  nws_check(nws_sum_batch_time(x.data_ptr<float>(), (int)x.size(0), (int)x.size(1), (int)x.size(2), out.data_ptr<float>(), L.stream),
            "nws_sum_batch_time");
  return out;
}

Tensor reverb(const Tensor& plan_t, const Tensor& tables, const Tensor& spectrum, const Tensor& x) {
  NwsReverbPlan plan = plan_of(plan_t);
  check_dev(x, "x");
  check_dev(tables, "reverb_tables");
  check_dev(spectrum, "reverb_spectrum");
  check_same_device(x, "x", tables, "reverb tables");
  check_same_device(x, "x", spectrum, "reverb.ir spectrum");
  TORCH_CHECK(x.dim() == 2, "Reverb: expected (B, N), got ", x.sizes());
  check_reverb_buffers(plan, tables, spectrum);
  const int64_t B = x.size(0), N = x.size(1);
  TORCH_CHECK(nws_reverb_plan_serves(&plan, (int)N, 0), "Reverb: the plan [L ", plan.L, ", Lc ", plan.Lc, ", hist ", plan.hist, ", nblk ", plan.nblk,
              "] was not made for ", N, " samples");
  Launch L(x);
  const size_t nbytes = nws_reverb_workspace_bytes(&plan, (int)B);
  Tensor ws = at::empty({(int64_t)nbytes}, x.options().dtype(at::kByte));
  Tensor y = at::empty_like(x);
  nws_check(nws_reverb(&plan, tables.data_ptr(), spectrum.data_ptr(), x.data_ptr<float>(), (int)B, (int)N, y.data_ptr<float>(),
                       ws.data_ptr(), nbytes, L.stream), "nws_reverb");
  return y;
}

Tensor reverb_grad_x(const Tensor& plan_t, const Tensor& tables, const Tensor& spectrum, const Tensor& grad_out) {
  NwsReverbPlan plan = plan_of(plan_t);
  check_dev(grad_out, "grad_out");
  check_dev(tables, "reverb_tables");
  check_dev(spectrum, "reverb_spectrum");
  check_same_device(grad_out, "grad_out", tables, "reverb tables");
  check_same_device(grad_out, "grad_out", spectrum, "reverb.ir spectrum");
  TORCH_CHECK(grad_out.dim() == 2, "reverb_grad_x: expected (B, N), got ", grad_out.sizes());
  check_reverb_buffers(plan, tables, spectrum);
  const int64_t B = grad_out.size(0), N = grad_out.size(1);
  TORCH_CHECK(nws_reverb_plan_serves(&plan, (int)N, 0), "reverb_grad_x: the plan [L ", plan.L, ", Lc ", plan.Lc, ", hist ", plan.hist,
              ", nblk ", plan.nblk, "] was not made for ", N, " samples");
  Launch L(grad_out);
  const size_t nbytes = nws_reverb_grad_workspace_bytes(&plan, (int)B, 0);
  Tensor ws = at::empty({(int64_t)nbytes}, grad_out.options().dtype(at::kByte));
  Tensor dx = at::empty_like(grad_out);
  nws_check(nws_reverb_grad_x(&plan, tables.data_ptr(), spectrum.data_ptr(), grad_out.data_ptr<float>(), (int)B, (int)N,
                              dx.data_ptr<float>(), ws.data_ptr(), nbytes, L.stream), "nws_reverb_grad_x");
  return dx;
}

Tensor reverb_grad_ir(const Tensor& plan_t, const Tensor& tables, const Tensor& x, const Tensor& grad_out, int64_t ir_len) {
  NwsReverbPlan plan = plan_of(plan_t);
  check_dev(x, "x");
  check_dev(grad_out, "grad_out");
  check_dev(tables, "reverb_tables");
  check_same_device(x, "x", tables, "reverb tables");
  check_same_device(x, "x", grad_out, "grad_out");
  TORCH_CHECK(x.dim() == 2 && grad_out.sizes() == x.sizes(), "reverb_grad_ir: x ", x.sizes(), " and grad_out ", grad_out.sizes(),
              " differ in shape");
  TORCH_CHECK((size_t)tables.numel() * tables.element_size() == nws_reverb_table_bytes(&plan), "reverb_tables: ",
              (size_t)tables.numel() * tables.element_size(), " bytes, the plan (L = ", plan.L, ") needs ", nws_reverb_table_bytes(&plan));
  const int64_t B = x.size(0), N = x.size(1);
  TORCH_CHECK(ir_len > 0 && ir_len < (1 << 30) && nws_reverb_plan_serves(&plan, (int)N, (int)ir_len + 1), "reverb_grad_ir: the plan [L ",
              plan.L, ", Lc ", plan.Lc, ", hist ", plan.hist, ", nblk ", plan.nblk, "] was not made for ", N, " samples and an impulse response of ",
              ir_len);
  Launch L(x);
  const size_t nbytes = nws_reverb_grad_workspace_bytes(&plan, (int)B, 1);
  Tensor ws = at::empty({(int64_t)nbytes}, x.options().dtype(at::kByte));
  Tensor dir = at::empty({ir_len}, x.options());
  nws_check(nws_reverb_grad_ir(&plan, tables.data_ptr(), x.data_ptr<float>(), grad_out.data_ptr<float>(), (int)B, (int)N, (int)ir_len,
                               dir.data_ptr<float>(), ws.data_ptr(), nbytes, L.stream), "nws_reverb_grad_ir");
  return dir;
}

std::tuple<Tensor, Tensor> reverb_linear_chunk(const Tensor& plan_t, const Tensor& tables, const Tensor& spectrum, const Tensor& x,
                                               const Tensor& tail_in) {
  NwsReverbPlan plan = plan_of(plan_t);
  check_dev(x, "x");
  check_dev(tail_in, "tail_in");
  check_dev(tables, "reverb_tables");
  check_dev(spectrum, "reverb_spectrum");
  check_same_device(x, "x", tail_in, "tail_in");
  check_same_device(x, "x", tables, "reverb tables");
  TORCH_CHECK(x.dim() == 2 && tail_in.dim() == 2 && tail_in.size(0) == x.size(0), "reverb_linear_chunk: x (B, M), tail_in (B, tail)");
  const int64_t B = x.size(0), M = x.size(1), tail_len = tail_in.size(1);
  check_reverb_buffers(plan, tables, spectrum);
  check_same_device(x, "x", spectrum, "reverb.ir spectrum");
  TORCH_CHECK(plan.Lc == 0, "reverb_linear_chunk: needs a direct plan (one transform of M + tail_len samples)");
  TORCH_CHECK(M + tail_len <= plan.L, "reverb_linear_chunk: chunk of ", M, " + tail of ", tail_len, " samples wraps around L = ", plan.L);
  Launch L(x);
  const size_t nbytes = (size_t)(2 * ((B + 1) / 2) * plan.L + B * plan.L) * sizeof(float);
  Tensor ws = at::empty({(int64_t)nbytes}, x.options().dtype(at::kByte));
  Tensor y = at::empty_like(x);
  Tensor tail_out = at::empty_like(tail_in);
  nws_check(nws_reverb_linear_chunk(&plan, tables.data_ptr(), spectrum.data_ptr(), x.data_ptr<float>(), (int)B, (int)M,
                                    tail_in.data_ptr<float>(), tail_out.data_ptr<float>(), (int)tail_len, y.data_ptr<float>(),
                                    ws.data_ptr(), nbytes, L.stream), "nws_reverb_linear_chunk");
  return {y, tail_out};
}

Tensor shaper_apply(const Tensor& wdesc, const Tensor& x) {
  const NwsWeights* w = weights_of(wdesc);
  check_dev(x, "x");
  TORCH_CHECK(x.dim() == 3 && x.size(1) == NWS_N_SHAPERS, "expected (B, 64, N), got ", x.sizes());
  Launch L(x);
  Tensor y = at::empty_like(x);
  nws_check(nws_shaper_apply(w, x.data_ptr<float>(), x.size(0), x.size(2), y.data_ptr<float>(), L.stream), "nws_shaper_apply");
// ... 617 lines not shown
  const int64_t B = exciter.size(0), N = exciter.size(2), T = film.size(2);
  TORCH_CHECK(T > 0 && N % T == 0, "NEWT: ", N, " samples are not a whole multiple of ", T, " control frames");
  TORCH_CHECK(mix_w.numel() % S == 0 && mix_b.numel() == mix_w.numel() / S, "NEWT: mixer weight ", mix_w.sizes(), " / bias ", mix_b.sizes());
  const int64_t O = mix_w.numel() / S;
  Launch L(exciter);
  Tensor shaped = at::empty_like(exciter);
  nws_check(nws_g_film_shaper(d, exciter.data_ptr<float>(), film.data_ptr<float>(), (int)B, (int)T, (int)(N / T),
                              shaped.data_ptr<float>(), L.stream), "nws_g_film_shaper");
  Tensor out = at::empty({B, O, N}, exciter.options());
  nws_check(nws_g_conv1x1(shaped.data_ptr<float>(), mix_w.data_ptr<float>(), mix_b.data_ptr<float>(), (int)B, (int)S, (int)O, (int)N,
                          out.data_ptr<float>(), L.stream), "nws_g_conv1x1");
  return out;
}

Tensor g_fir_noise(const Tensor& H, const Tensor& window, const Tensor& noise, int64_t hop) {
  check_dev(H, "H");
  check_dev(window, "window");
  check_dev(noise, "noise");
  check_same_device(H, "H", window, "noise_synth.window");
  check_same_device(H, "H", noise, "noise");
  const int64_t Lf = window.numel();
  TORCH_CHECK(H.dim() == 3 && H.size(1) == Lf / 2 + 1, "FIRNoiseSynth: expected H of shape (B, ", Lf / 2 + 1, ", T), got ", H.sizes());
  const int64_t B = H.size(0), T = H.size(2);
  TORCH_CHECK(noise.numel() == hop * T - 1, "noise: expected ", hop * T - 1, " samples, got ", noise.sizes());
  Launch L(H);
  Tensor fir = at::empty({B, T, Lf}, H.options());
  nws_check(nws_g_fir_design(H.data_ptr<float>(), window.data_ptr<float>(), (int)Lf, (int)B, (int)T, fir.data_ptr<float>(), L.stream),
            "nws_g_fir_design");
  Tensor out = at::empty({B, hop * T}, H.options());
  nws_check(nws_g_fir_noise(fir.data_ptr<float>(), noise.data_ptr<float>(), (int)Lf, (int)hop, (int)B, (int)T, nullptr, 0,
                            out.data_ptr<float>(), L.stream), "nws_g_fir_noise");
  return out;
}

Tensor g_reverb_direct(const Tensor& x, const Tensor& ir) {
  check_dev(x, "x");
  check_dev(ir, "reverb.ir");
  check_same_device(x, "x", ir, "reverb.ir");
  TORCH_CHECK(x.dim() == 2, "Reverb: expected (B, N), got ", x.sizes());
  Launch L(x);
  Tensor y = at::empty_like(x);
  nws_check(nws_g_reverb_direct(x.data_ptr<float>(), ir.data_ptr<float>(), (int)ir.numel(), (int)x.size(0), (int)x.size(1),
                                y.data_ptr<float>(), L.stream), "nws_g_reverb_direct");
  return y;
}

struct StepDims {
  int64_t B, K, C;
};

StepDims check_step_tensors(const char* op, const Tensor& f0, const Tensor& control, const Tensor& fir_design, const Tensor& state,
                            const Tensor& phase_u, const Tensor& rand_phase, const Tensor& ir, const Tensor& out) {
  check_dev(f0, "f0");
  check_dev(control, "control");
  check_dev(fir_design, "fir_design");
  check_dev(state, "state", at::kByte);
  check_dev(phase_u, "phase_u");
  check_dev(rand_phase, "rand_phase");
  check_dev(ir, "reverb.ir");
  check_dev(out, "out");
  check_same_device(f0, "f0", control, "control");
  check_same_device(f0, "f0", state, "state");
  check_same_device(f0, "f0", out, "out");
  check_same_device(f0, "f0", ir, "reverb.ir");
  TORCH_CHECK(f0.dim() == 2 && control.dim() == 3 && control.size(0) == f0.size(0) && control.size(2) == f0.size(1) && control.size(1) >= 2,
              op, ": f0 (B, K), control (B, C>=2, K); got ", f0.sizes(), " / ", control.sizes());
  return {f0.size(0), f0.size(1), control.size(1)};
}

void check_step_io(const char* op, const StepDims& d, bool first, bool final, int64_t frames_seen, const Tensor& phase_u,
                   const Tensor& rand_phase, const OptTensor& noise_new, const OptTensor& noise_all, const Tensor& out,
                   const OptTensor& pre_out) {
  TORCH_CHECK(phase_u.numel() == NWS_N_HARMONICS && rand_phase.numel() == NWS_N_HARMONICS, "phase_u / rand_phase: 101 elements each");
  TORCH_CHECK(noise_new.has_value() != noise_all.has_value(), op, ": give exactly one of noise_new and noise_all");
  const int M = nws_stream_out_samples((int)d.K, first, final);
  TORCH_CHECK(out.numel() == d.B * M, "out: expected (", d.B, ", ", M, "), got ", out.sizes());
  if (pre_out.has_value()) {
    check_dev(*pre_out, "pre_out");
    TORCH_CHECK(pre_out->numel() == d.B * M, "pre_out: expected (", d.B, ", ", M, ")");
  }
  if (noise_new.has_value()) {
    check_dev(*noise_new, "noise_new");
    TORCH_CHECK(noise_new->numel() >= nws_stream_noise_draws((int)d.K, first, frames_seen), "noise_new: expected ",
                nws_stream_noise_draws((int)d.K, first, frames_seen), " fresh samples");
  } else {
    check_dev(*noise_all, "noise_all");
  }
}

void stream_step(const Tensor& wdesc, const Tensor& fir_design, const OptTensor& plan_t, const OptTensor& tables,
                 const OptTensor& spectrum, Tensor& state, int64_t max_frames, const Tensor& f0, const Tensor& control, bool first,
                 bool final, int64_t frames_seen, int64_t nz_prev_start, double sample_rate, const Tensor& phase_u,
                 const Tensor& rand_phase, const OptTensor& noise_new, const OptTensor& noise_all, const Tensor& ir, Tensor& out,
                 const OptTensor& pre_out) {
  const NwsWeights* w = weights_of(wdesc);
  const StepDims d = check_step_tensors("stream_step", f0, control, fir_design, state, phase_u, rand_phase, ir, out);
  const int64_t B = d.B, K = d.K, C = d.C;
  TORCH_CHECK(K >= 1 && K <= max_frames, "stream_step: chunk of ", K, " frames, the stream was sized for ", max_frames);
  check_step_io("stream_step", d, first, final, frames_seen, phase_u, rand_phase, noise_new, noise_all, out, pre_out);
  NwsReverbPlan plan{};
  const bool fft = plan_t.has_value();
  if (fft) {
    TORCH_CHECK(tables.has_value() && spectrum.has_value(), "stream_step: plan without tables / spectrum");
    plan = plan_of(*plan_t);
    check_dev(*tables, "reverb_tables");
    check_dev(*spectrum, "reverb_spectrum");
    check_reverb_buffers(plan, *tables, *spectrum);
  }
  TORCH_CHECK((size_t)state.numel() >= nws_stream_state_bytes((int)B, (int)max_frames, (int)ir.numel(), fft ? &plan : nullptr),
              "stream_step: state blob too small");
  Launch L(f0);
  nws_check(nws_stream_step(w, fir_design.data_ptr<float>(), fft ? &plan : nullptr, fft ? tables->data_ptr() : nullptr,
                            fft ? spectrum->data_ptr() : nullptr, state.data_ptr(), (size_t)state.numel(), (int)B, (int)max_frames,
                            f0.data_ptr<float>(), control.data_ptr<float>(), (int)C, (int)K, first ? 1 : 0, final ? 1 : 0,
                            (long long)frames_seen, (long long)nz_prev_start, (float)sample_rate, phase_u.data_ptr<float>(),
                            rand_phase.data_ptr<float>(), fptr(noise_new), fptr(noise_all),
                            noise_all.has_value() ? (int)noise_all->numel() : 0, ir.data_ptr<float>(), (int)ir.numel(),
                            out.data_ptr<float>(), pre_out.has_value() ? pre_out->data_ptr<float>() : nullptr, L.stream),
            "nws_stream_step");
}

void stream_step_slots(const Tensor& wdesc, const Tensor& fir_design, Tensor& state, int64_t max_frames, const Tensor& f0,
                       const Tensor& control, int64_t frames_seen, int64_t nz_prev_start, double sample_rate, const Tensor& phase_u,
                       const Tensor& rand_phase, const OptTensor& noise_new, const OptTensor& noise_all, const Tensor& ir,
                       const Tensor& events, Tensor& out, const OptTensor& pre_out) {
  const NwsWeights* w = weights_of(wdesc);
  const StepDims d = check_step_tensors("stream_step_slots", f0, control, fir_design, state, phase_u, rand_phase, ir, out);
  const int64_t B = d.B, K = d.K, C = d.C;
  check_dev(events, "events", at::kInt);
  check_same_device(f0, "f0", events, "events");
  TORCH_CHECK(K >= 1 && K <= 16 && K <= max_frames, "stream_step_slots: hops of 1 .. 16 frames (sized for ", max_frames, "), got ", K);
  TORCH_CHECK(events.numel() == B, "stream_step_slots: events: one int32 word per slot, expected ", B, ", got ", events.numel());
  check_step_io("stream_step_slots", d, frames_seen == 0, false, frames_seen, phase_u, rand_phase, noise_new, noise_all, out, pre_out);
  TORCH_CHECK((size_t)state.numel() >= nws_stream_slot_state_bytes((int)B, (int)max_frames, (int)ir.numel()),
              "stream_step_slots: state blob too small");
  Launch L(f0);
  nws_check(nws_stream_step_slots(w, fir_design.data_ptr<float>(), state.data_ptr(), (size_t)state.numel(), (int)B, (int)max_frames,
                                  f0.data_ptr<float>(), control.data_ptr<float>(), (int)C, (int)K, (long long)frames_seen,
                                  (long long)nz_prev_start, (float)sample_rate, phase_u.data_ptr<float>(), rand_phase.data_ptr<float>(),
                                  fptr(noise_new), fptr(noise_all), noise_all.has_value() ? (int)noise_all->numel() : 0,
                                  ir.data_ptr<float>(), (int)ir.numel(), events.data_ptr<int>(), out.data_ptr<float>(),
                                  pre_out.has_value() ? pre_out->data_ptr<float>() : nullptr, L.stream),
            "nws_stream_step_slots");
}

int64_t abi_version() { return nws_abi_version(); }

}

TORCH_LIBRARY(newt_hip, m) {
  m.def("abi_version() -> int", &abi_version);
  m.def("forward(Tensor wdesc, Tensor f0, Tensor control, Tensor phase_u, Tensor rand_phase, Tensor noise, Tensor fir_design, "
        "Tensor plan, Tensor reverb_tables, Tensor reverb_spectrum, Tensor(a!) workspace, float sample_rate) -> Tensor", &forward);
  m.def("forward_control(Tensor wdesc, Tensor f0, Tensor control, Tensor(a!) workspace, bool batched_gru) -> ()", &forward_control);
  m.def("forward_audio(Tensor wdesc, Tensor f0, Tensor phase_u, Tensor rand_phase, Tensor noise, Tensor fir_design, Tensor plan, "
        "Tensor reverb_tables, Tensor reverb_spectrum, Tensor(a!) workspace, float sample_rate, Tensor? out, int wait_event, "
        "int record_event) -> Tensor", &forward_audio);
  m.def("forward_audio_pre(Tensor wdesc, Tensor f0, Tensor phase_u, Tensor rand_phase, Tensor noise, Tensor fir_design, Tensor plan, "
        "Tensor reverb_tables, Tensor reverb_spectrum, Tensor(a!) workspace, float sample_rate) -> ()", &forward_audio_pre);
  m.def("forward_audio_blocks(Tensor wdesc, Tensor f0, Tensor phase_u, Tensor rand_phase, Tensor noise, Tensor fir_design, Tensor plan, "
        "Tensor reverb_tables, Tensor reverb_spectrum, Tensor(a!) workspace, float sample_rate, Tensor(b!) out, int[] row0, int[] nrows, "
        "int[] events) -> ()", &forward_audio_blocks);
  m.def("forward_reverb_rows(Tensor fir_design, Tensor plan, Tensor reverb_tables, Tensor reverb_spectrum, Tensor(a!) workspace, int T, "
        "int row0, int nrows, Tensor(b!) out) -> ()", &forward_reverb_rows);
  m.def("phase_carry(Tensor? f0, Tensor? f0_up) -> Tensor", &phase_carry);
  m.def("exciter_newt(Tensor wdesc, Tensor? f0, Tensor? f0_up, Tensor carry, Tensor phase_u, Tensor rand_phase, Tensor? film, "
        "float sample_rate, bool want_exciter, bool want_newt) -> (Tensor, Tensor)", &exciter_newt);
  m.def("oscillator(Tensor f0_up, Tensor phase_u, Tensor rand_phase, float sample_rate) -> Tensor", &oscillator);
  m.def("control_gru(Tensor wdesc, Tensor control, Tensor? h0, bool batched) -> (Tensor, Tensor)", &control_gru);
  m.def("frame_mlps(Tensor wdesc, Tensor gru_out, Tensor fir_design, bool want_emb, bool want_H) -> (Tensor, Tensor, Tensor, Tensor)",
        &frame_mlps);
  m.def("fir_noise(Tensor fir, Tensor noise, Tensor? add_in, int origin) -> Tensor", &fir_noise);
  m.def("fir_from_h(Tensor H, Tensor fir_design) -> Tensor", &fir_from_h);
  m.def("fir_noise_grad(Tensor noise, Tensor grad_out) -> Tensor", &fir_noise_grad);
  m.def("fir_from_h_grad(Tensor grad_fir, Tensor fir_design) -> Tensor", &fir_from_h_grad);
  m.def("sum_batch_time(Tensor x) -> Tensor", &sum_batch_time);
  m.def("reverb(Tensor plan, Tensor tables, Tensor spectrum, Tensor x) -> Tensor", &reverb);
  m.def("reverb_grad_x(Tensor plan, Tensor tables, Tensor spectrum, Tensor grad_out) -> Tensor", &reverb_grad_x);
  m.def("reverb_grad_ir(Tensor plan, Tensor tables, Tensor x, Tensor grad_out, int ir_len) -> Tensor", &reverb_grad_ir);
  m.def("reverb_linear_chunk(Tensor plan, Tensor tables, Tensor spectrum, Tensor x, Tensor tail_in) -> (Tensor, Tensor)",
        &reverb_linear_chunk);
  m.def("shaper_apply(Tensor wdesc, Tensor x) -> Tensor", &shaper_apply);
  m.def("shaper_table(Tensor wdesc, Tensor like, int size, float tmin, float tmax) -> Tensor", &shaper_table);
  m.def("newt_apply(Tensor wdesc, Tensor exciter, Tensor film) -> Tensor", &newt_apply);
  m.def("td_mlp(Tensor x, Tensor[] weights, Tensor[] biases, Tensor[] ln_w, Tensor[] ln_b, float eps, float slope) -> Tensor", &td_mlp);
  m.def("td_mlp_grad(Tensor x, Tensor grad_y, Tensor[] weights, Tensor[] biases, Tensor[] ln_w, Tensor[] ln_b, float eps, float slope, "
        "bool want_params) -> Tensor[]", &td_mlp_grad);
  m.def("td_layer_norm(Tensor x, Tensor weight, Tensor bias, float eps) -> Tensor", &td_layer_norm);
  m.def("film(Tensor x, Tensor gamma, Tensor beta) -> Tensor", &film);
  m.def("sine(Tensor x) -> Tensor", &sine);
  m.def("forward_generic(Tensor gdesc, Tensor f0, Tensor control, Tensor phase_u, Tensor rand_phase, Tensor noise, Tensor? plan, "
        "Tensor? reverb_tables, Tensor? reverb_spectrum, Tensor(a!) reverb_workspace, Tensor(b!) workspace, float sample_rate) -> Tensor",
        &forward_generic);
  m.def("g_gru(Tensor w_ih, Tensor w_hh, Tensor b_ih, Tensor b_hh, Tensor control, Tensor? h0) -> (Tensor, Tensor)", &g_gru);
  m.def("g_oscillator(Tensor f0_up, Tensor phase_u, Tensor rand_phase, float sample_rate) -> Tensor", &g_oscillator);
  m.def("g_conv1x1(Tensor x, Tensor weight, Tensor? bias) -> Tensor", &g_conv1x1);
  m.def("g_upsample(Tensor x, int hop) -> Tensor", &g_upsample);
  m.def("g_shaper_apply(Tensor sdesc, Tensor x) -> Tensor", &g_shaper_apply);
  m.def("g_shaper_table(Tensor sdesc, Tensor like, int size, float tmin, float tmax) -> Tensor", &g_shaper_table);
  m.def("g_newt_apply(Tensor sdesc, Tensor exciter, Tensor film, Tensor mix_w, Tensor mix_b) -> Tensor", &g_newt_apply);
  m.def("g_fir_noise(Tensor H, Tensor window, Tensor noise, int hop) -> Tensor", &g_fir_noise);
  m.def("g_reverb_direct(Tensor x, Tensor ir) -> Tensor", &g_reverb_direct);
  m.def("stream_step(Tensor wdesc, Tensor fir_design, Tensor? plan, Tensor? reverb_tables, Tensor? reverb_spectrum, Tensor(a!) state, "
        "int max_frames, Tensor f0, Tensor control, bool first, bool final, int frames_seen, int nz_prev_start, float sample_rate, "
        "Tensor phase_u, Tensor rand_phase, Tensor? noise_new, Tensor? noise_all, Tensor ir, Tensor(b!) out, Tensor(c!)? pre_out) -> ()",
        &stream_step);
  m.def("stream_step_slots(Tensor wdesc, Tensor fir_design, Tensor(a!) state, int max_frames, Tensor f0, Tensor control, int frames_seen, "
        "int nz_prev_start, float sample_rate, Tensor phase_u, Tensor rand_phase, Tensor? noise_new, Tensor? noise_all, Tensor ir, "
        "Tensor events, Tensor(b!) out, Tensor(c!)? pre_out) -> ()",
        &stream_step_slots);
  m.def("loudness(Tensor audio, Tensor dft, int n_fft, int hop, float amin, float top_db, bool normalise) -> Tensor", &loudness);
  m.def("pyin_table(float sample_rate, float fmin, float fmax, int frame_length, int hop) -> Tensor", &pyin_table);
  m.def("pyin_cmnd(Tensor audio, float sample_rate, float fmin, float fmax, int frame_length, int hop) -> Tensor", &pyin_cmnd);
  m.def("pyin_observe(Tensor yin, Tensor table, float sample_rate, float fmin, float fmax, int frame_length, int hop) -> "
        "(Tensor, Tensor, Tensor, Tensor)", &pyin_observe);
  m.def("pyin_viterbi(Tensor cand_bin, Tensor cand_prob, Tensor count, Tensor voiced_prob, Tensor table, float sample_rate, "
        "float fmin, float fmax, int frame_length, int hop, bool fill_unvoiced, float fill_value) -> (Tensor, Tensor)", &pyin_viterbi);
  m.def("pyin(Tensor audio, Tensor table, float sample_rate, float fmin, float fmax, int frame_length, int hop, bool fill_unvoiced, "
        "float fill_value) -> (Tensor, Tensor, Tensor)", &pyin);
  m.def("resample_bank(int sr_in, int sr_out) -> Tensor", &resample_bank);
  m.def("resample(Tensor audio, Tensor bank, int sr_in, int sr_out) -> Tensor", &resample);
  m.def("mfcc_table(float sample_rate, int n_fft, int n_mfcc, int n_mels) -> Tensor", &mfcc_table);
  m.def("stft_loss_dft(int n_fft, int win_length) -> Tensor", &stft_loss_dft);
  m.def("stft_loss(Tensor x, Tensor y, Tensor[] dfts, int[] n_ffts, int[] hops, int[] win_lengths, float w_sc, float w_log_mag, "
        "float w_lin_mag, float eps) -> Tensor[]", &stft_loss);
  m.def("stft_loss_grad(Tensor x, Tensor y, Tensor[] dfts, int[] n_ffts, int[] hops, int[] win_lengths, float w_sc, float w_log_mag, "
        "float w_lin_mag, float eps) -> Tensor", &stft_loss_grad);
  m.def("mfcc(Tensor audio, Tensor dft, Tensor table, float sample_rate, int n_fft, int hop, int n_mfcc, int n_mels) -> Tensor", &mfcc);
}
```

neural-waveshaping-synthesis_amd/engine.py:

```python
from __future__ import annotations

import ctypes as C
import itertools
import math
import os
from typing import NamedTuple

import torch

from . import _lib
from ._lib import NwsReverbPlan, NwsWeights, check, ptr


def _req(t: torch.Tensor, name: str, numel: int | None = None) -> torch.Tensor:
    if not isinstance(t, torch.Tensor):
        raise TypeError(f"{name}: expected a tensor")
    if t.device.type != "cuda":
        raise _lib.NwsError(
            f"{name} lives on {t.device}: the NEWT forward path only runs as HIP kernels on an AMD GPU "
            "(move the model and inputs with .to('cuda')); there is no CPU fallback.")
    if t.dtype != torch.float32:
        raise TypeError(f"{name}: expected float32, got {t.dtype}")
    if not t.is_contiguous():
        raise ValueError(f"{name}: expected a contiguous tensor")
# ... 262 lines not shown
                turns = torch.empty((64, _lib.SHAPER_TURNS_ROW), dtype=torch.float32, device=dev)
                check(L.nws_shaper_turns(C.byref(w), ptr(turns), st), "nws_shaper_turns")
                keep.append(turns)
                w.shaper_turns = turns.data_ptr()
            table = getattr(m.newt, "lookup_table", None)
            if table is not None:
                size = int(m.newt.table_size)
                w.lut = P(table, "newt.lookup_table", 64 * size)
                pairs = torch.empty((64, size, 2), dtype=torch.float32, device=table.device)
                check(L.nws_lut_pairs(w.lut, size, ptr(pairs), st), "nws_lut_pairs")
                keep.append(pairs)
                w.lut_pairs = pairs.data_ptr()
                w.lut_size = size
                w.lut_min = float(m.newt.table_min)
                w.lut_max = float(m.newt.table_max)
            else:
                w.lut = None
                w.lut_pairs = None
                w.lut_size, w.lut_min, w.lut_max = 0, 0.0, 0.0
            w.exciter_opts = self.exciter_opts()
            if getattr(m.newt, "lookup_table", None) is None and self.bank_nofract_safe():
                w.exciter_opts |= _lib.EXCITER_BANK_NOFRACT
            w.newt_out_w = P(m.newt.mixer[0].weight, "newt.mixer.0.weight", 64)
            w.newt_out_b = P(m.newt.mixer[0].bias, "newt.mixer.0.bias", 1)
            w.noise_window = P(m.noise_synth.window, "noise_synth.window", 256)
            fd = torch.empty(_lib.FIR_LEN * _lib.FIR_DESIGN_COLS, dtype=torch.float32, device=dev)
            check(L.nws_fir_design_matrix(w.noise_window, ptr(fd), st), "nws_fir_design_matrix")
            keep.append(fd)
            w.mlp_frags = None
            if self.fp16_mlp_safe():
                frags = torch.empty(_lib.MLP_FRAGS_BYTES, dtype=torch.uint8, device=dev)
                check(L.nws_mlp_frags(C.byref(w), ptr(fd), ptr(frags), st), "nws_mlp_frags")
                keep.append(frags)
                w.mlp_frags = frags.data_ptr()
            rand_phase = _req(m.osc.rand_phase.detach(), "osc.rand_phase", 101)
            ir = _req(m.reverb.ir.detach(), "reverb.ir")
            keep += [rand_phase, ir]
            devs = {t.device for t in keep}
            if len(devs) != 1:
                raise RuntimeError(f"model parameters are spread over several devices: {devs}")
            torch.cuda.current_stream(dev).synchronize()
        wdesc = torch.frombuffer(bytearray(bytes(w)), dtype=torch.uint8)
        self._w = Weights(w, wdesc, dev, rand_phase, ir, fd, keep)
        self._fp = fp
        return self._w

    HYBRID_W_BOUND = 1e-5

    def exciter_opts(self) -> int:
        v = getattr(self._model_ref, "exciter_opts", None)
        if v is None:
            v = os.environ.get("NWS_EXCITER_OPTS")
        if v is not None and str(v) != "auto":
            return int(v)
        b = self.hybrid_w_bound()
        return _lib.EXCITER_HYBRID_W if (b is not None and b["bound"] <= self.HYBRID_W_BOUND) else 0

    def bank_nofract_safe(self, limit_turns: float = 128.0) -> bool:
        sh = self._model_ref.newt._modules.get("shaping_fn")
        if sh is None or getattr(sh, "depth", 0) != 4:
            return False
        with torch.no_grad():
            worst = 0.0
            for i in (2, 4, 6):
                wt, b = sh.net[i].weight.detach(), sh.net[i].bias.detach()
                worst = max(worst, float((wt.abs().flatten(1).sum(1) + b.abs()).max()) / (2.0 * math.pi))
        return math.isfinite(worst) and worst < limit_turns

    def hybrid_w_bound(self):
        from . import precision

        m = self._model_ref
        table = getattr(m.newt, "lookup_table", None)
        if table is None:
            return None
        return precision.hybrid_w_error_bound(m, table, float(m.newt.table_min), float(m.newt.table_max))

    def fp16_mlp_safe(self, limit: float = 3.0e4) -> bool:
        m = self._model_ref
        with torch.no_grad():
            def l1(wt, b, scale):
                return float((wt.detach().abs().flatten(1).sum(1) * scale + b.detach().abs()).max())

            def ln(mod):
                return float(math.sqrt(_lib.HIDDEN - 1) * mod.layer_norm.weight.detach().abs().max()
                             + mod.layer_norm.bias.detach().abs().max())

            bounds = [l1(m.embedding.proj.weight, m.embedding.proj.bias, 1.0)]
            for mlp in (m.newt.mlp, m.h_generator):
                bounds += [ln(mlp.net[1]), ln(mlp.net[4]), ln(mlp.net[7])]
            bounds.append(l1(m.h_generator.net[9].weight, m.h_generator.net[9].bias, ln(m.h_generator.net[7])))
            wmax = max(float(p.detach().abs().max()) for mlp in (m.newt.mlp, m.h_generator) for p in mlp.parameters())
        return max(bounds + [wmax]) < limit and all(b == b for b in bounds)

    @property
    def device(self):
        return self._wd().device

    def rand_phase(self):
        return self._wd().rand_phase

    def ir(self):
        return self._wd().ir

    def fir_design(self):
        return self._wd().fir_design

    def osc_sample_rate(self) -> float:
        m = self._model_ref
        return float(getattr(getattr(m, "osc", None), "sample_rate", m.sample_rate))

    def reverb_aux(self, n_samples: int):
        self._wd()
        return self._reverb_aux(n_samples)

    def _reverb_aux(self, n_samples: int):
        ir, dev = self._w.ir, self._w.device
        plan, tables, plan_t = reverb_plan_and_tables(dev, n_samples, ir.numel() + 1)
        skey = (plan.L, plan.N1, plan.N2)
        spec = self._spectra.get(skey)
        if spec is None:
            with torch.cuda.device(dev):
                spec = torch.empty(_lib.lib().nws_reverb_spectrum_bytes(C.byref(plan)) // 4, dtype=torch.float32, device=dev)
                nbytes = _lib.lib().nws_reverb_workspace_bytes(C.byref(plan), 1)
                ws = torch.empty(nbytes, dtype=torch.uint8, device=dev)
                check(_lib.lib().nws_reverb_ir_spectrum(C.byref(plan), ptr(tables), ptr(ir), ir.numel(), ptr(spec), ptr(ws),
                                                        nbytes, stream_ptr(dev)), "nws_reverb_ir_spectrum")
                torch.cuda.current_stream(dev).synchronize()
            self._spectra[skey] = spec
        return plan, tables, spec, plan_t

    def phase_carry(self, f0=None, f0_up=None):
        return binding().phase_carry(f0, f0_up)

    def exciter_newt(self, f0, f0_up, carry, phase_u, film, want_exciter=False, want_newt=True):
        r = self._wd()
        same_device(r.device, f0=f0 if f0 is not None else f0_up, carry=carry, phase_u=phase_u, film=film)
        exc, out = binding().exciter_newt(r.wdesc, f0, f0_up, carry, phase_u, r.rand_phase, film, self.osc_sample_rate(),
                                          want_exciter, want_newt)
        return (exc if want_exciter else None), (out if want_newt else None)

    def control_gru(self, control, batched=False, h0=None, return_state=False):
        r = self._wd()
        same_device(r.device, control=control, h0=h0)
        out, hT = binding().control_gru(r.wdesc, control, h0, bool(batched))
        return (out, hT) if return_state else out

    def frame_mlps(self, gru_out, want_emb=False, want_H=False):
        r = self._wd()
        same_device(r.device, gru_out=gru_out)
        emb, film, H, fir = binding().frame_mlps(r.wdesc, gru_out, r.fir_design, want_emb, want_H)
        return (emb if want_emb else None), film, (H if want_H else None), fir

    def fir_noise(self, fir, noise, add_in=None, origin=None, noise_len=None):
        same_device(fir.device, noise=noise, add_in=add_in)
        nz = noise if noise_len is None or noise_len == noise.numel() else noise[:noise_len]
        return binding().fir_noise(fir, nz, add_in, -1 if origin is None else int(origin))

    def reverb(self, x):
        same_device(self._wd().device, x=x)
        _, tables, spec, plan_t = self._reverb_aux(x.shape[1])
        return binding().reverb(plan_t, tables, spec, x)

    def reverb_linear_chunk(self, plan_aux, x, tail_in):
        _, tables, spec, plan_t = plan_aux
        same_device(tables.device, x=x, tail_in=tail_in)
        return binding().reverb_linear_chunk(plan_t, tables, spec, x, tail_in)

    def shaper_table(self, size, tmin, tmax):
        r = self._wd()
        return binding().shaper_table(r.wdesc, r.rand_phase, int(size), float(tmin), float(tmax))

    def shaper_apply(self, x):
        r = self._wd()
        same_device(r.device, x=x)
        return binding().shaper_apply(r.wdesc, x)

    def newt_apply(self, exciter, film):
        r = self._wd()
        same_device(r.device, exciter=exciter, film=film)
        return binding().newt_apply(r.wdesc, exciter, film)

    def new_workspace(self, B, T):
        dev = self._wd().device
        plan, _, _, _ = self._reverb_aux(T * _lib.HOP)
        return torch.empty(_lib.lib().nws_forward_workspace_bytes(C.byref(plan), B, T), dtype=torch.uint8, device=dev)

    def forward_control(self, f0, control, ws, batched_gru=True):
        r = self._wd()
        same_device(r.device, f0=f0, control=control, workspace=ws)
        binding().forward_control(r.wdesc, f0, control, ws, bool(batched_gru))

    def forward_audio(self, f0, B, T, phase_u, noise, ws, out=None, wait_event=None, record_event=None, row_blocks=None,
                      on_block=None, block_events=None):
        r = self._wd()
        dev = r.device
        same_device(dev, f0=f0, phase_u=phase_u, noise=noise, workspace=ws, out=out)
        if block_events is not None and (row_blocks is None or len(row_blocks) < 2 or on_block is not None):
            raise RuntimeError("block_events are recorded by the one-call block path only: pass row_blocks of two or more blocks and "
                               "no on_block callback")
        N = T * _lib.HOP
        _, tables, spec, plan_t = self._reverb_aux(N)
        b = binding()
        audio = (r.wdesc, f0, phase_u, r.rand_phase, noise, r.fir_design, plan_t, tables, spec, ws, self.osc_sample_rate())
        if row_blocks is None or len(row_blocks) < 2:
            return b.forward_audio(*audio, out, wait_event.cuda_event if wait_event is not None else 0,
                                   record_event.cuda_event if record_event is not None else 0)
        nxt = 0
        for k, (row0, nrows) in enumerate(row_blocks):
            if int(row0) != nxt or int(nrows) <= 0 or (int(nrows) % 2 and k != len(row_blocks) - 1):
                raise RuntimeError(f"row_blocks must tile [0, {B}) in order, even sizes except the last, got {list(row_blocks)}")
            nxt += int(nrows)
        if nxt != B:
            raise RuntimeError(f"row_blocks cover {nxt} of {B} rows: {list(row_blocks)}")
        if wait_event is not None or record_event is not None:
            raise RuntimeError("wait_event / record_event hook the single-call form; they cannot be combined with row_blocks")
        if block_events is not None and len(block_events) != len(row_blocks):
            raise RuntimeError("block_events: one torch.cuda.Event per row block")
        with torch.cuda.device(dev):
            if out is None:
                out = torch.empty((B, N), dtype=torch.float32, device=dev)
            if block_events is not None:
                for ev in block_events:
                    if not ev.cuda_event:
                        ev.record()
                b.forward_audio_blocks(*audio, out, [int(r0) for r0, _ in row_blocks], [int(n) for _, n in row_blocks],
                                       [int(ev.cuda_event) for ev in block_events])
                return out
            b.forward_audio_pre(*audio)
            for row0, nrows in row_blocks:
                b.forward_reverb_rows(r.fir_design, plan_t, tables, spec, ws, T, int(row0), int(nrows), out)
                if on_block is not None:
                    on_block(int(row0), int(nrows), out)
        return out

    def forward(self, f0, control, phase_u, noise):
        if not self.specialised():
            return self.generic.forward(f0, control, phase_u, noise)
        r = self._wd()
        dev = r.device
        same_device(dev, f0=f0, control=control, phase_u=phase_u, noise=noise)
        B, _, T = control.shape
        plan, tables, spec, plan_t = self._reverb_aux(T * _lib.HOP)
        key = (B, T, stream_ptr(dev))
        ws = self._workspaces.get(key)
        if ws is None:
            nbytes = _lib.lib().nws_forward_workspace_bytes(C.byref(plan), B, T)
            ws = torch.empty(nbytes, dtype=torch.uint8, device=dev)
            if len(self._workspaces) >= 16:
                self._workspaces.pop(next(iter(self._workspaces)))
            self._workspaces[key] = ws
        return binding().forward(r.wdesc, f0, control, phase_u, r.rand_phase, noise, r.fir_design, plan_t, tables, spec, ws,
                                 self.osc_sample_rate())
```

neural-waveshaping-synthesis_amd/pipeline.py:

```python
from __future__ import annotations

import os

import torch

from . import _lib
from .engine import _req


class _Slot:
    __slots__ = ("ws", "ev_control", "ev_audio", "ev_exciter", "used", "keep", "pu", "nz")

    def __init__(self):
        self.ws = None
        self.pu = None
        self.nz = None
        self.ev_control = torch.cuda.Event()
        self.ev_audio = torch.cuda.Event()
        self.ev_exciter = torch.cuda.Event()
        self.used = False
        self.keep = None


_PLACED = {}
# ... 144 lines not shown
                          f"every kernel launch slows down by an order of magnitude; 16 is what this package is measured with",
                          RuntimeWarning, stacklevel=2)
        got, kept = None, []
        with torch.cuda.device(key):
            if mode != "order" and not os.environ.get("NWS_STREAM_ORDER"):
                got = _place_by_measurement(d, rep)
                kept = rep.pop("spare", [])
                if got is None or not rep.get("verified"):
                    rep["ok"] = False
                    warnings.warn(f"ForwardPipeline: no verified placement of the stream set on the command processor's pipes ({rep}); "
                                  f"{'falling back to first-use order' if got is None else 'using the unverified choice'} - the step can "
                                  f"be 12-35 % slower", RuntimeWarning, stacklevel=2)
            if got is None:
                rep["mode"] = "order" if (mode == "order" or os.environ.get("NWS_STREAM_ORDER")) else "order (fallback)"
                got = _place_in_fixed_order(d, rep)
                got = got[:3] + (got[3] + kept,)
        pl.exchange, pl.audio, pl.control, pl.spare = got
        pl.audio_anchors = rep.pop("_audio_anchors", None)
        pl.side = []
        pl.cur = torch.cuda.current_stream(d)
        rep["ms"] = round((time.perf_counter() - t0) * 1e3, 2)
        pl.report = rep
        _PLACED[key] = pl
    return pl.exchange, pl.audio[:audio_streams], pl.control[:control_streams]


def side_streams(dev, n: int, max_candidates: int = 0):
    d = torch.device(dev)
    key = d.index if d.index is not None else torch.cuda.current_device()
    placed_streams(d)
    pl = _PLACED[key]
    max_candidates = max_candidates or 2 * n + 2
    rep = pl.report.setdefault("side", {"kept": 0, "rejected": 0, "plain": 0, "reused": 0})
    with torch.cuda.device(key):
        if len(pl.side) < n and pl.audio_anchors:
            touch = torch.zeros(64, device=d)
            scratch = torch.zeros(4, dtype=torch.int64, device=d)
            torch.cuda.synchronize(d)
            while len(pl.side) < n and rep["kept"] + rep["rejected"] < max_candidates:
                st = torch.cuda.Stream(device=d)
                _first_use(st, touch)
                if any(_blocks(h, st, scratch) for h in pl.audio_anchors):
                    pl.spare.append(st)
                    rep["rejected"] += 1
                else:
                    pl.side.append(st)
                    rep["kept"] += 1
        if len(pl.side) < n:
            if pl.side and pl.audio_anchors:
                k = len(pl.side)
                rep["reused"] = n - k
                return [pl.side[i % k] for i in range(n)]
            while len(pl.side) < n:
                pl.side.append(torch.cuda.Stream(device=d))
                rep["plain"] += 1
    return pl.side[:n]


def placement_report(dev=None):
    d = torch.device(dev if dev is not None else "cuda")
    pl = _PLACED.get(d.index if d.index is not None else torch.cuda.current_device())
    return dict(pl.report) if pl is not None else None


def verify_placement(dev=None):
    d = torch.device(dev if dev is not None else "cuda")
    key = d.index if d.index is not None else torch.cuda.current_device()
    pl = _PLACED[key]
    with torch.cuda.device(key):
        scratch = torch.zeros(4, dtype=torch.int64, device=d)
        torch.cuda.synchronize(d)
        named = {"cur": pl.cur, "x": pl.exchange, "a0": pl.audio[0], "a1": pl.audio[1]}
        want = {"c0 blocks cur": True, "c0 blocks x": False, "c0 blocks a0": False, "c0 blocks a1": False,
                "c1 blocks cur": False, "c1 blocks x": True, "c1 blocks a0": False, "c1 blocks a1": False}
        seen = {k: _blocks(pl.control[int(k[1])], named[k.split()[-1]], scratch) for k in want}
    return {"ok": seen == want, "seen": seen, "want": want}


class ForwardPipeline:

    def __init__(self, model, depth: int = 4, audio_streams: int = 2, control_streams: int = 2, batched_gru: bool = False,
                 chain_exciters: bool = False, streams=None):
        if depth < 2 or audio_streams < 1 or control_streams < 1:
            raise ValueError("need depth >= 2 and at least one stream of each kind")
        self.model = model
        self.eng = model._engine
        _, _, dev = self.eng.weights()
        self.dev = dev
        if streams is not None:
            xs, au, co = streams
            if not au or not co:
                raise ValueError("streams=(exchange, audio streams, control streams) needs at least one stream of each kind")
            self.exchange, self.audio, self.control = xs, list(au), list(co)
            audio_streams = len(self.audio)
        else:
            self.exchange, self.audio, self.control = placed_streams(dev, audio_streams, control_streams)
        self.slots = [_Slot() for _ in range(depth)]
        self.batched_gru = batched_gru
        self.chain_exciters = bool(chain_exciters) and audio_streams > 1
        self._last_exciter = None
        self._n = 0
        self._shape = None
        self._outstanding = []

    def _prepare(self, B, T):
        if self._shape != (B, T):
            self.synchronize()
            for s in self.slots:
                s.ws = self.eng.new_workspace(B, T)
                s.used = False
                s.pu = torch.empty(_lib.N_HARMONICS, dtype=torch.float32, device=self.dev)
                s.nz = torch.empty(_lib.HOP * T - 1, dtype=torch.float32, device=self.dev)
            self._shape = (B, T)

    def next_audio_stream(self):
        return self.audio[self._n % len(self.audio)]

    @staticmethod
    def row_blocks(B: int, chunks: int):
        if chunks <= 1 or B % chunks or (B // chunks) % 2 or B // chunks < 4:
            return None
        n = B // chunks
        return [(q * n, n) for q in range(chunks)]

    def submit(self, f0, control, *, phase_u=None, noise=None, out=None, row_blocks=None, on_block=None, generator=None,
               block_events=None):
        m = self.model
        f0 = _req(f0 if f0.is_contiguous() else f0.contiguous(), "f0")
        control = _req(control if control.is_contiguous() else control.contiguous(), "control")
        if f0.dim() != 3 or f0.shape[1] != 1 or control.dim() != 3 or control.shape[1] < 2:
            raise RuntimeError(f"expected f0 (B,1,T) and control (B,C>=2,T), got {tuple(f0.shape)} / {tuple(control.shape)}")
        B, _, T = f0.shape
        if control.shape[0] != B or control.shape[2] != T or T < 2:
            raise RuntimeError("f0 and control disagree on batch / frames (or fewer than 2 frames)")
        if block_events is not None and (self.chain_exciters or on_block is not None or row_blocks is None or len(row_blocks) < 2):
            raise ValueError("block_events are recorded by the one-call block path only: they need row_blocks of two or more blocks, "
                             "no on_block callback and chain_exciters off")
        self._prepare(B, T)
        i = self._n
        self._n += 1
        slot = self.slots[i % len(self.slots)]
        cs = self.control[i % len(self.control)]
        au = self.audio[i % len(self.audio)]
        batched = bool(self.batched_gru)
        ready = torch.cuda.current_stream(self.dev).record_event()
        with torch.cuda.stream(cs):
            cs.wait_event(ready)
            if slot.used:
                cs.wait_event(slot.ev_audio)
            pu = torch.rand(_lib.N_HARMONICS, out=slot.pu, generator=generator) if phase_u is None else phase_u
            pu = _req(pu.reshape(-1), "phase_u", _lib.N_HARMONICS)
            nz = torch.rand(m.control_hop * T - 1, out=slot.nz, generator=generator) if noise is None else noise
            nz = _req(nz, "noise", m.control_hop * T - 1)
            self.eng.forward_control(f0, control, slot.ws, batched_gru=batched)
            slot.ev_control.record(cs)
        with torch.cuda.stream(au):
            au.wait_event(ready)
            au.wait_event(slot.ev_control)
            if self.chain_exciters:
                out = self.eng.forward_audio(f0, B, T, pu, nz, slot.ws, out=out, wait_event=self._last_exciter,
                                             record_event=slot.ev_exciter)
                self._last_exciter = slot.ev_exciter
            else:
                out = self.eng.forward_audio(f0, B, T, pu, nz, slot.ws, out=out, row_blocks=row_blocks, on_block=on_block,
                                             block_events=block_events)
            slot.ev_audio.record(au)
        slot.used = True
        slot.keep = (f0, control, pu, nz)
        self._outstanding.append((out, slot.ev_audio))
        if len(self._outstanding) > len(self.slots):
            del self._outstanding[:-len(self.slots)]
        return out

    def join_current_stream(self):
        cur = torch.cuda.current_stream(self.dev)
        for out, ev in self._outstanding[-len(self.slots):]:
            cur.wait_event(ev)
            out.record_stream(cur)
        self._outstanding.clear()

    def synchronize(self):
        for s in self.audio + self.control:
            s.synchronize()
        self._outstanding.clear()
```

Baseline: 10.43 billion samples/s.

## Precompute noise spectra on the control stream and load them in the FIR-noise kernel

Adds a small kernel that computes the FFT spectra of the shared noise once per run and writes them to a table. The control stream now receives the noise and builds this table. The audio-side spectral FIR kernel then copies the table straight into LDS through global_load_lds instead of having wave 0 of every block redo the noise FFT. The aim is to remove the redundant per-block noise FFTs from the critical audio path and overlap that work with the GRU. In exchange it adds workspace, a stamp flag checked on the device, and an extra launch on the control stream.

New measurement: 10.44 billion samples/s (median of 3 runs). Within noise of the previous version (+0.1%).

```diff
diff --git a/include/nws_hip.h b/include/nws_hip.h
--- a/include/nws_hip.h
+++ b/include/nws_hip.h
@@ -110,6 +110,9 @@
                   int B, int T, float* out , void* stream);
 int nws_fir_noise_window(const float* fir, const float* noise, int noise_len, int origin, const float* add_in, int B, int T,
                          float* out, void* stream);
+size_t nws_fir_noise_spectra_bytes(int T);
+int nws_fir_noise_spectra(const float* noise, int noise_len, int origin, int T, float* table, void* stream);
+int nws_fir_noise_tabled(const float* fir, const float* table, const float* add_in, int B, int T, float* out, void* stream);
 
 int nws_fir_noise_grad(const float* noise , const float* grad_out , int B, int T,
                        float* grad_fir , void* stream);
@@ -220,6 +223,8 @@
 size_t nws_forward_control_bytes(int B, int T);
 int nws_forward_control(const NwsWeights* w, const float* f0, const float* control, int B, int C, int T, int batched_gru,
                         void* workspace, size_t workspace_bytes, void* stream);
+int nws_forward_control_noise(const NwsWeights* w, const float* f0, const float* control, const float* noise, int B, int C,
+                              int T, int batched_gru, void* workspace, size_t workspace_bytes, void* stream);
 int nws_forward_audio(const NwsWeights* w, const NwsForwardAux* aux, const float* f0, int B, int T, float sample_rate,
                       const float* phase_u, const float* rand_phase, const float* noise, float* out, void* workspace,
                       size_t workspace_bytes, void* stream);
diff --git a/neural-waveshaping-synthesis_amd/_cops.py b/neural-waveshaping-synthesis_amd/_cops.py
--- a/neural-waveshaping-synthesis_amd/_cops.py
+++ b/neural-waveshaping-synthesis_amd/_cops.py
@@ -87,12 +87,14 @@
                                          workspace.numel(), _stream(f0.device)), "nws_forward")
         return out
 
-    def forward_control(self, wdesc, f0, control, workspace, batched_gru):
+    def forward_control(self, wdesc, f0, control, noise, workspace, batched_gru):
         B, Cc, T = control.shape
-        with torch.cuda.device(f0.device):
-            check(_lib.lib().nws_forward_control(C.byref(_struct(wdesc, NwsWeights)), ptr(f0), ptr(control), B, Cc, T,
-                                                 1 if batched_gru else 0, ptr(workspace), workspace.numel(), _stream(f0.device)),
-                  "nws_forward_control")
+        if noise is not None and noise.numel() != HOP * T - 1:
+            raise RuntimeError(f"noise: expected {HOP * T - 1} elements, got {tuple(noise.shape)}")
+        with torch.cuda.device(f0.device):
+            check(_lib.lib().nws_forward_control_noise(C.byref(_struct(wdesc, NwsWeights)), ptr(f0), ptr(control), ptr(noise), B, Cc,
+                                                       T, 1 if batched_gru else 0, ptr(workspace), workspace.numel(),
+                                                       _stream(f0.device)), "nws_forward_control_noise")
 
     def forward_audio(self, wdesc, f0, phase_u, rand_phase, noise, fir_design, plan, reverb_tables, reverb_spectrum, workspace,
                       sample_rate, out, wait_event, record_event):
@@ -196,6 +198,28 @@
             else:
                 check(_lib.lib().nws_fir_noise_window(ptr(fir), ptr(noise), noise.numel(), origin, ptr(add_in), B, T, ptr(out),
                                                       _stream(fir.device)), "nws_fir_noise_window")
+        return out
+
+    def fir_noise_spectra(self, noise, T):
+        if not 2 <= T <= 1 << 23 or noise.numel() != T * HOP - 1:
+            raise RuntimeError(f"noise: expected {T * HOP - 1} samples (T >= 2), got {tuple(noise.shape)}")
+        with torch.cuda.device(noise.device):
+            table = _new(noise, _lib.lib().nws_fir_noise_spectra_bytes(T) // (4 * 9 * 16 * 4 * 4), 4, 9, 16, 4)
+            check(_lib.lib().nws_fir_noise_spectra(ptr(noise), noise.numel(), _lib.FIR_LEN // 2, T, ptr(table), _stream(noise.device)),
+                  "nws_fir_noise_spectra")
+        return table
+
+    def fir_noise_tabled(self, fir, table, add_in):
+        B, T, _ = fir.shape
+        if B < 16:
+            raise RuntimeError(f"fir_noise_tabled: the kernel that reads noise spectra serves B >= 16, got B = {B}")
+        if table.numel() * 4 != _lib.lib().nws_fir_noise_spectra_bytes(T):
+            raise RuntimeError(f"table: expected the {_lib.lib().nws_fir_noise_spectra_bytes(T)} bytes of fir_noise_spectra for T = {T}, "
+                               f"got {tuple(table.shape)}")
+        with torch.cuda.device(fir.device):
+            out = _new(fir, B, T * HOP)
+            check(_lib.lib().nws_fir_noise_tabled(ptr(fir), ptr(table), ptr(add_in), B, T, ptr(out), _stream(fir.device)),
+                  "nws_fir_noise_tabled")
         return out
 
     def fir_from_h(self, H, fir_design):
diff --git a/neural-waveshaping-synthesis_amd/_lib.py b/neural-waveshaping-synthesis_amd/_lib.py
--- a/neural-waveshaping-synthesis_amd/_lib.py
+++ b/neural-waveshaping-synthesis_amd/_lib.py
@@ -112,6 +112,9 @@
     "nws_fir_design_matrix": (C.c_int, [_fp, _fp, _fp]),
     "nws_fir_noise": (C.c_int, [_fp, _fp, _fp, C.c_int, C.c_int, _fp, _fp]),
     "nws_fir_noise_window": (C.c_int, [_fp, _fp, C.c_int, C.c_int, _fp, C.c_int, C.c_int, _fp, _fp]),
+    "nws_fir_noise_spectra_bytes": (C.c_size_t, [C.c_int]),
+    "nws_fir_noise_spectra": (C.c_int, [_fp, C.c_int, C.c_int, C.c_int, _fp, _fp]),
+    "nws_fir_noise_tabled": (C.c_int, [_fp, _fp, _fp, C.c_int, C.c_int, _fp, _fp]),
     "nws_fir_noise_grad": (C.c_int, [_fp, _fp, C.c_int, C.c_int, _fp, _fp]),
     "nws_fir_from_h_grad": (C.c_int, [_fp, _fp, C.c_int, C.c_int, _fp, _fp]),
     "nws_sum_batch_time": (C.c_int, [_fp, C.c_int, C.c_int, C.c_int, _fp, _fp]),
@@ -139,6 +142,8 @@
                               C.c_float, _fp, _fp, _fp, _fp, _fp, C.c_size_t, _fp]),
     "nws_forward_control_bytes": (C.c_size_t, [C.c_int, C.c_int]),
     "nws_forward_control": (C.c_int, [C.POINTER(NwsWeights), _fp, _fp, C.c_int, C.c_int, C.c_int, C.c_int, _fp, C.c_size_t, _fp]),
+    "nws_forward_control_noise": (C.c_int, [C.POINTER(NwsWeights), _fp, _fp, _fp, C.c_int, C.c_int, C.c_int, C.c_int, _fp,
+                                            C.c_size_t, _fp]),
     "nws_forward_audio": (C.c_int, [C.POINTER(NwsWeights), C.POINTER(NwsForwardAux), _fp, C.c_int, C.c_int, C.c_float,
                                     _fp, _fp, _fp, _fp, _fp, C.c_size_t, _fp]),
     "nws_forward_audio_ev": (C.c_int, [C.POINTER(NwsWeights), C.POINTER(NwsForwardAux), _fp, C.c_int, C.c_int, C.c_float,
diff --git a/neural-waveshaping-synthesis_amd/csrc/fir_noise.hip b/neural-waveshaping-synthesis_amd/csrc/fir_noise.hip
--- a/neural-waveshaping-synthesis_amd/csrc/fir_noise.hip
+++ b/neural-waveshaping-synthesis_amd/csrc/fir_noise.hip
@@ -171,10 +171,67 @@
   sp_fft256<false>(z, tw, x, l);
 }
 
+__device__ __forceinline__ void sp_noise_spectra(const float* __restrict__ noise, int len, int origin, int N, int ta,
+                                                 const float* tw, float* xs, int l, float4 (&sd)[9]) {
+  C16 z;
+#pragma unroll
+  for (int j = 0; j < 16; ++j) {
+    const int i0 = kHop * ta + 16 * j + l, i1 = i0 + kHop;
+    const bool in0 = i0 >= 0 && i0 < N + kL - 1, in1 = i1 >= 0 && i1 < N + kL - 1;
+    const float v0 = padded_noise(noise, len, origin, in0 ? i0 : origin);
+    const float v1 = padded_noise(noise, len, origin, in1 ? i1 : origin);
+    z.re[j] = in0 ? v0 : 0.0f;
+    z.im[j] = in1 ? v1 : 0.0f;
+  }
+  sp_fft256<false>(z, tw, xs, l);
+  float mr[16], mi[16];
+  auto mirror = [&](const float (&v)[16], float (&m)[16]) {
+#pragma unroll
+    for (int j = 0; j < 16; ++j) xs[l + 16 * j] = v[j];
+    sp_wave_sync();
+#pragma unroll
+    for (int j = 0; j < 16; ++j) m[j] = xs[(256 - (l + 16 * j)) & 255];
+    sp_wave_sync();
+  };
+  mirror(z.re, mr);
+  mirror(z.im, mi);
+  const float c = (l & 1) ? -(1.0f / 512.0f) : (1.0f / 512.0f);
+#pragma unroll
+  for (int j = 0; j < 9; ++j)
+    sd[j] = make_float4(c * (z.re[j] + mr[j]), c * (z.im[j] - mi[j]), c * (z.re[j] - mr[j]), c * (z.im[j] + mi[j]));
+}
+
+constexpr int kSpRunEntries = kSpPairs * 9 * 16;
+static_assert(kSpRunEntries == 2 * 64 * kSpWaves + 64, "the copy into SpectralLds::sd: two wave-instructions per wave and one more");
+
+__global__ __launch_bounds__(64) void fir_noise_spectra_kernel(const float* __restrict__ noise, int T, int len, int origin,
+                                                               float4* __restrict__ table, unsigned* __restrict__ stamp) {
+  __shared__ __attribute__((aligned(16))) float4 tw4[256];
+  __shared__ float xs[kSpPairs][kSpPlane];
+  const int lane = threadIdx.x, g = lane >> 4, l = lane & 15;
+  const int run = blockIdx.x;
+#pragma unroll
+  for (int e = lane; e < 256; e += 64) {
+    float c, s;
+    sp_twiddle((e & 15) * (e >> 4), c, s);
+    tw4[e] = make_float4(c, c, s, s);
+  }
+  __syncthreads();
+  float4 sd[9];
+  sp_noise_spectra(noise, len, origin, T * kHop, run * kSpHops - 1 + 2 * g, reinterpret_cast<const float*>(&tw4[l]), xs[g], l, sd);
+  float4* dst = table + (size_t)run * kSpRunEntries + g * (9 * 16) + l;
+#pragma unroll
+  for (int j = 0; j < 9; ++j) dst[16 * j] = sd[j];
+  if (stamp != nullptr && run == 0 && lane == 0) *stamp = 1u;
+}
+
+template <bool TABLE>
 __global__ __launch_bounds__(64 * kSpWaves, 3) void fir_noise_spectral_kernel(const float* __restrict__ fir,
                                                                              const float* __restrict__ noise,
                                                                              const float* __restrict__ add_in, int B, int T, int len,
-                                                                             int origin, float* __restrict__ out, int nruns, int total) {
+                                                                             int origin, float* __restrict__ out, int nruns, int total,
+                                                                             const float4* __restrict__ table,
+                                                                             const unsigned* __restrict__ stamp) {
   __shared__ __attribute__((aligned(16))) SpectralLds L;
   const int tid = threadIdx.x, lane = tid & 63, wave = tid >> 6;
   const int g = lane >> 4, l = lane & 15;
@@ -200,6 +257,7 @@
     ua[j] = f32x2{rowa0[16 * j], rowa1[16 * j]};
     ub[j] = f32x2{rowb0[16 * j], rowb1[16 * j]};
   }
+  const bool tabled = TABLE && (stamp == nullptr || *stamp != 0u);
   {
     float c, s;
     sp_twiddle((tid & 15) * (tid >> 4), c, s);
@@ -209,41 +267,31 @@
   __syncthreads();
 
   f32x2* x = &L.x[wave][g * kSpPlane];
-  if (wave == 0) {
-    C16 z;
-    float* xs = reinterpret_cast<float*>(x);
-#pragma unroll
-    for (int j = 0; j < 16; ++j) {
-      const int i0 = kHop * ta + 16 * j + l, i1 = i0 + kHop;
-      const bool in0 = i0 >= 0 && i0 < N + kL - 1, in1 = i1 >= 0 && i1 < N + kL - 1;
-      const float v0 = padded_noise(noise, len, origin, in0 ? i0 : origin);
-      const float v1 = padded_noise(noise, len, origin, in1 ? i1 : origin);
-      z.re[j] = in0 ? v0 : 0.0f;
-      z.im[j] = in1 ? v1 : 0.0f;
-    }
-    sp_fft256<false>(z, tw, xs, l);
-    float mr[16], mi[16];
-    auto mirror = [&](const float (&v)[16], float (&m)[16]) {
-#pragma unroll
-      for (int j = 0; j < 16; ++j) xs[l + 16 * j] = v[j];
-      sp_wave_sync();
-#pragma unroll
-      for (int j = 0; j < 16; ++j) m[j] = xs[(256 - (l + 16 * j)) & 255];
-      sp_wave_sync();
-    };
-    mirror(z.re, mr);
-    mirror(z.im, mi);
-    const float c = (l & 1) ? -(1.0f / 512.0f) : (1.0f / 512.0f);
-#pragma unroll
-    for (int j = 0; j < 9; ++j)
-      L.sd[g][j][l] = make_float4(c * (z.re[j] + mr[j]), c * (z.im[j] - mi[j]), c * (z.re[j] - mr[j]), c * (z.im[j] + mi[j]));
-  }
   const f32x2 zero = {0.0f, 0.0f};
-#pragma unroll
-  for (int j = 0; j < 8; ++j) {
-    ua[j] = sp_select(oka, ua[j], zero);
-    ub[j] = sp_select(okb, ub[j], zero);
-  }
+  const auto silence = [&]() {
+#pragma unroll
+    for (int j = 0; j < 8; ++j) {
+      ua[j] = sp_select(oka, ua[j], zero);
+      ub[j] = sp_select(okb, ub[j], zero);
+    }
+  };
+  if (tabled) {
+    silence();
+    typedef const __attribute__((address_space(1))) void* GlobalPtr;
+    typedef __attribute__((address_space(3))) void* LdsPtr;
+    const float4* src = table + (size_t)run * kSpRunEntries + lane;
+    float4* dst = &L.sd[0][0][0];
+    const int w64 = __builtin_amdgcn_readfirstlane(wave) * 64;
+    __builtin_amdgcn_global_load_lds((GlobalPtr)(src + w64), (LdsPtr)(dst + w64), 16, 0, 0);
+    __builtin_amdgcn_global_load_lds((GlobalPtr)(src + w64 + 256), (LdsPtr)(dst + w64 + 256), 16, 0, 0);
+    if (w64 == 0) __builtin_amdgcn_global_load_lds((GlobalPtr)(src + 512), (LdsPtr)(dst + 512), 16, 0, 0);
+  } else if (wave == 0) {
+    float4 sd[9];
+    sp_noise_spectra(noise, len, origin, N, ta, tw, reinterpret_cast<float*>(x), l, sd);
+#pragma unroll
+    for (int j = 0; j < 9; ++j) L.sd[g][j][l] = sd[j];
+  }
+  if (!tabled) silence();
   C16T<f32x2> z;
   sp_filter_spectrum(z, ua, ub, tw, x, lane, l);
   __syncthreads();
@@ -313,16 +361,19 @@
 
 }
 
-extern "C" int nws_fir_noise_window(const float* fir, const float* noise, int noise_len, int origin, const float* add_in,
-                                    int B, int T, float* out, void* stream) {
-  if (!fir || !noise || !out || B <= 0 || T <= 0 || noise_len < 2 || origin < 0) return NWS_ERR_BAD_ARG;
+extern "C" int nws_fir_noise_window_table(const float* fir, const float* noise, int noise_len, int origin, const float* table,
+                                          const unsigned* stamp, const float* add_in, int B, int T, float* out, void* stream) {
+  if (!fir || !out || B <= 0 || T <= 0 || noise_len < 2 || origin < 0) return NWS_ERR_BAD_ARG;
+  if (!noise && (!table || stamp || B < 16)) return NWS_ERR_BAD_ARG;
+  if (table && (B < 16 || (reinterpret_cast<uintptr_t>(table) & 15))) return NWS_ERR_BAD_ARG;
   if (B > 65535) return NWS_ERR_UNSUPPORTED;
   if (B >= 16) {
     const long long nruns = (T + kSpHops - 1) / kSpHops, total = nruns * ((B + kSpUtt - 1) / kSpUtt);
     if (total > (1ll << 30)) return NWS_ERR_UNSUPPORTED;
     const dim3 grid((unsigned)(8 * ((total + 7) / 8)));
-    fir_noise_spectral_kernel<<<grid, 64 * kSpWaves, 0, (hipStream_t)stream>>>(fir, noise, add_in, B, T, noise_len, origin, out,
-                                                                             (int)nruns, (int)total);
+    const auto kernel = table != nullptr ? fir_noise_spectral_kernel<true> : fir_noise_spectral_kernel<false>;
+    kernel<<<grid, 64 * kSpWaves, 0, (hipStream_t)stream>>>(fir, noise, add_in, B, T, noise_len, origin, out, (int)nruns, (int)total,
+                                                            reinterpret_cast<const float4*>(table), stamp);
     NWS_CHECK_LAUNCH();
     return NWS_OK;
   }
@@ -330,6 +381,39 @@
   fir_noise_kernel<false><<<grid, 256, 0, (hipStream_t)stream>>>(fir, noise, add_in, T, noise_len, origin, out, nullptr);
   NWS_CHECK_LAUNCH();
   return NWS_OK;
+}
+
+extern "C" int nws_fir_noise_window(const float* fir, const float* noise, int noise_len, int origin, const float* add_in,
+                                    int B, int T, float* out, void* stream) {
+  if (!noise) return NWS_ERR_BAD_ARG;
+  return nws_fir_noise_window_table(fir, noise, noise_len, origin, nullptr, nullptr, add_in, B, T, out, stream);
+}
+
+extern "C" size_t nws_fir_noise_spectra_bytes(int T) {
+  if (T <= 0) return 0;
+  return (size_t)((T + kSpHops - 1) / kSpHops) * kSpRunEntries * sizeof(float4);
+}
+
+extern "C" int nws_fir_noise_spectra_stamped(const float* noise, int noise_len, int origin, int T, float* table, unsigned* stamp,
+                                             void* stream) {
+  if (!noise || !table || T <= 0 || noise_len < 2 || origin < 0) return NWS_ERR_BAD_ARG;
+  if (reinterpret_cast<uintptr_t>(table) & 15) return NWS_ERR_BAD_ARG;
+  if (T > (1 << 23)) return NWS_ERR_UNSUPPORTED;
+  fir_noise_spectra_kernel<<<(T + kSpHops - 1) / kSpHops, 64, 0, (hipStream_t)stream>>>(noise, T, noise_len, origin,
+                                                                                        reinterpret_cast<float4*>(table), stamp);
+  NWS_CHECK_LAUNCH();
+  return NWS_OK;
+}
+
+extern "C" int nws_fir_noise_spectra(const float* noise, int noise_len, int origin, int T, float* table, void* stream) {
+  return nws_fir_noise_spectra_stamped(noise, noise_len, origin, T, table, nullptr, stream);
+}
+
+extern "C" int nws_fir_noise_tabled(const float* fir, const float* table, const float* add_in, int B, int T, float* out,
+                                    void* stream) {
+  if (!table) return NWS_ERR_BAD_ARG;
+  if (B > 0 && B < 16) return NWS_ERR_UNSUPPORTED;
+  return nws_fir_noise_window_table(fir, nullptr, T * kHop - 1, kL / 2, table, nullptr, add_in, B, T, out, stream);
 }
 
 extern "C" int nws_fir_noise_window_rows(const float* fir, const float* noise, int origin, const int4* rows, int B, int T,
diff --git a/neural-waveshaping-synthesis_amd/csrc/forward.hip b/neural-waveshaping-synthesis_amd/csrc/forward.hip
--- a/neural-waveshaping-synthesis_amd/csrc/forward.hip
+++ b/neural-waveshaping-synthesis_amd/csrc/forward.hip
@@ -21,6 +21,9 @@
 
 size_t aligned(size_t b) { return (b + 255) & ~size_t(255); }
 
+constexpr int kSpectraMinB = 16;
+size_t spectra_bytes(int B, int T) { return B >= kSpectraMinB ? nws_fir_noise_spectra_bytes(T) + 4 * sizeof(unsigned) : 0; }
+
 constexpr int kStages = 6;
 struct Profile {
   int slots = 0;
@@ -44,6 +47,7 @@
   size_t total = 0;
   total += aligned((size_t)B * (N / 32) * sizeof(double));
   total += aligned((size_t)B * T * NWS_HIDDEN * sizeof(float));
+  total += aligned(spectra_bytes(B, T));
   total += aligned((size_t)B * T * NWS_FILM_CH * sizeof(float));
   total += aligned((size_t)B * T * NWS_FIR_HALF * sizeof(float));
   total += aligned((size_t)B * N * sizeof(float));
@@ -59,6 +63,8 @@
 struct Arena {
   double* carry;
   float *gru_out, *film, *fir, *noise_out, *pre;
+  float* spectra;
+  unsigned* stamp;
   void* rv_ws;
   size_t rv_bytes;
   bool ok;
@@ -70,6 +76,10 @@
   Arena a{};
   a.carry = static_cast<double*>(cv.take((size_t)B * (N / 32) * sizeof(double)));
   a.gru_out = static_cast<float*>(cv.take((size_t)B * T * NWS_HIDDEN * sizeof(float)));
+  if (const size_t sb = spectra_bytes(B, T)) {
+    a.spectra = static_cast<float*>(cv.take(sb));
+    a.stamp = a.spectra ? reinterpret_cast<unsigned*>(reinterpret_cast<char*>(a.spectra) + nws_fir_noise_spectra_bytes(T)) : nullptr;
+  }
   if (!head_only) {
     a.film = static_cast<float*>(cv.take((size_t)B * T * NWS_FILM_CH * sizeof(float)));
     a.fir = static_cast<float*>(cv.take((size_t)B * T * NWS_FIR_HALF * sizeof(float)));
@@ -91,15 +101,26 @@
     if (rc != NWS_OK) return rc;                               \
   } while (0)
 
-int control_half(const NwsWeights* w, const float* f0, const float* control, int B, int C, int T, int batched_gru,
-                 const Arena& a, void* stream) {
+int noise_spectra(const float* noise, int T, const Arena& a, void* stream) {
+  if (a.spectra == nullptr) return NWS_OK;
+  if (noise != nullptr) return nws_fir_noise_spectra_stamped(noise, T * NWS_HOP - 1, NWS_FIR_LEN / 2, T, a.spectra, a.stamp, stream);
+  const hipError_t e = hipMemsetAsync(a.stamp, 0, sizeof(unsigned), (hipStream_t)stream);
+  return e == hipSuccess ? NWS_OK : (int)e;
+}
+
+int control_half(const NwsWeights* w, const float* f0, const float* control, const float* noise, int B, int C, int T,
+                 int batched_gru, const Arena& a, void* stream) {
   hipStream_t st = (hipStream_t)stream;
   int rc = NWS_OK;
   if (batched_gru) {
-    NWS_STAGE(0, nws_phase_carry(f0, nullptr, B, T, a.carry, stream));
+    const auto stage0 = [&]() {
+      const int e = noise_spectra(noise, T, a, stream);
+      return e != NWS_OK ? e : nws_phase_carry(f0, nullptr, B, T, a.carry, stream);
+    };
+    NWS_STAGE(0, stage0());
     NWS_STAGE(1, nws_control_gru_batched(w, control, B, C, T, nullptr, a.gru_out, nullptr, stream));
   } else {
-    NWS_STAGE(0, NWS_OK);
+    NWS_STAGE(0, noise_spectra(noise, T, a, stream));
     NWS_STAGE(1, nws_control_gru_carry(w, control, f0, B, C, T, a.gru_out, a.carry, stream));
   }
   return NWS_OK;
@@ -112,7 +133,8 @@
   int rc = NWS_OK;
   const size_t N = (size_t)T * NWS_HOP;
   NWS_STAGE(2, nws_frame_mlps(w, a.gru_out, aux->fir_design, B, T, nullptr, a.film, nullptr, a.fir, stream));
-  NWS_STAGE(4, nws_fir_noise(a.fir, noise, nullptr, B, T, a.noise_out, stream));
+  NWS_STAGE(4, nws_fir_noise_window_table(a.fir, noise, T * NWS_HOP - 1, NWS_FIR_LEN / 2, a.spectra, a.stamp, nullptr, B, T,
+                                          a.noise_out, stream));
   if (wait_before_exciter != nullptr) {
     const hipError_t e = hipStreamWaitEvent(st, (hipEvent_t)wait_before_exciter, 0);
     if (e != hipSuccess) return (int)e;
@@ -151,7 +173,8 @@
 size_t nws_forward_control_bytes(int B, int T) {
   if (B <= 0 || T <= 0) return 0;
   const size_t N = (size_t)T * NWS_HOP;
-  return aligned((size_t)B * (N / 32) * sizeof(double)) + aligned((size_t)B * T * NWS_HIDDEN * sizeof(float));
+  return aligned((size_t)B * (N / 32) * sizeof(double)) + aligned((size_t)B * T * NWS_HIDDEN * sizeof(float)) +
+         aligned(spectra_bytes(B, T));
 }
 
 int nws_forward(const NwsWeights* w, const NwsForwardAux* aux, const float* f0, const float* control, int B, int C,
@@ -161,20 +184,27 @@
   if (!f0 || !control || !phase_u || !rand_phase || !noise || !out || !workspace) return NWS_ERR_BAD_ARG;
   if (B <= 0 || T < 2 || C < 2) return NWS_ERR_BAD_ARG;
   if (T > (1 << 23) || !nws_reverb_plan_serves(aux->plan, T * NWS_HOP, 0)) return NWS_ERR_BAD_ARG;
-  const Arena a = carve_arena(aux->plan, workspace, workspace_bytes, B, T, false);
-  if (!a.ok) return NWS_ERR_WORKSPACE;
-  const int rc = control_half(w, f0, control, B, C, T, 0, a, stream);
+  Arena a = carve_arena(aux->plan, workspace, workspace_bytes, B, T, false);
+  if (!a.ok) return NWS_ERR_WORKSPACE;
+  a.spectra = nullptr;
+  a.stamp = nullptr;
+  const int rc = control_half(w, f0, control, noise, B, C, T, 0, a, stream);
   if (rc != NWS_OK) return rc;
   return audio_half(w, aux, f0, B, T, sample_rate, phase_u, rand_phase, noise, out, a, stream);
 }
 
+int nws_forward_control_noise(const NwsWeights* w, const float* f0, const float* control, const float* noise, int B, int C,
+                              int T, int batched_gru, void* workspace, size_t workspace_bytes, void* stream) {
+  if (!w || !f0 || !control || !workspace) return NWS_ERR_BAD_ARG;
+  if (B <= 0 || T < 2 || C < 2 || T > (1 << 23)) return NWS_ERR_BAD_ARG;
+  const Arena a = carve_arena(nullptr, workspace, workspace_bytes, B, T, true);
+  if (!a.ok) return NWS_ERR_WORKSPACE;
+  return control_half(w, f0, control, noise, B, C, T, batched_gru, a, stream);
+}
+
 int nws_forward_control(const NwsWeights* w, const float* f0, const float* control, int B, int C, int T, int batched_gru,
                         void* workspace, size_t workspace_bytes, void* stream) {
-  if (!w || !f0 || !control || !workspace) return NWS_ERR_BAD_ARG;
-  if (B <= 0 || T < 2 || C < 2) return NWS_ERR_BAD_ARG;
-  const Arena a = carve_arena(nullptr, workspace, workspace_bytes, B, T, true);
-  if (!a.ok) return NWS_ERR_WORKSPACE;
-  return control_half(w, f0, control, B, C, T, batched_gru, a, stream);
+  return nws_forward_control_noise(w, f0, control, nullptr, B, C, T, batched_gru, workspace, workspace_bytes, stream);
 }
 
 int nws_forward_audio(const NwsWeights* w, const NwsForwardAux* aux, const float* f0, int B, int T, float sample_rate,
diff --git a/neural-waveshaping-synthesis_amd/csrc/nws_common.h b/neural-waveshaping-synthesis_amd/csrc/nws_common.h
--- a/neural-waveshaping-synthesis_amd/csrc/nws_common.h
+++ b/neural-waveshaping-synthesis_amd/csrc/nws_common.h
@@ -391,6 +391,12 @@
 extern "C" __attribute__((visibility("hidden"))) int nws_fir_noise_window_rows(const float* fir, const float* noise, int origin,
                                                                                const int4* rows, int B, int T, float* out,
                                                                                void* stream);
+extern "C" __attribute__((visibility("hidden"))) int nws_fir_noise_window_table(const float* fir, const float* noise, int noise_len,
+                                                                                int origin, const float* table, const unsigned* stamp,
+                                                                                const float* add_in, int B, int T, float* out,
+                                                                                void* stream);
+extern "C" __attribute__((visibility("hidden"))) int nws_fir_noise_spectra_stamped(const float* noise, int noise_len, int origin,
+                                                                                   int T, float* table, unsigned* stamp, void* stream);
 extern "C" __attribute__((visibility("hidden"))) int nws_control_gru_stream(const NwsWeights* w, const float* control, int B, int C,
                                                                             int T, const float* h0, float* gru_out, float* hT,
                                                                             const NwsStreamSide* side, void* stream);
diff --git a/neural-waveshaping-synthesis_amd/csrc/torch_ops.cpp b/neural-waveshaping-synthesis_amd/csrc/torch_ops.cpp
--- a/neural-waveshaping-synthesis_amd/csrc/torch_ops.cpp
+++ b/neural-waveshaping-synthesis_amd/csrc/torch_ops.cpp
@@ -147,16 +147,22 @@
   return out;
 }
 
-void forward_control(const Tensor& wdesc, const Tensor& f0, const Tensor& control, Tensor& workspace, bool batched_gru) {
+void forward_control(const Tensor& wdesc, const Tensor& f0, const Tensor& control, const OptTensor& noise, Tensor& workspace,
+                     bool batched_gru) {
   const NwsWeights* w = weights_of(wdesc);
   int64_t B, C, T;
   check_inputs(f0, control, B, C, T);
   check_dev(workspace, "workspace", at::kByte);
   check_same_device(f0, "f0", workspace, "workspace");
+  if (noise.has_value()) {
+    check_dev(*noise, "noise");
+    check_same_device(f0, "f0", *noise, "noise");
+    TORCH_CHECK(noise->numel() == NWS_HOP * T - 1, "noise: expected ", NWS_HOP * T - 1, " elements, got ", noise->sizes());
+  }
   Launch L(f0);
-  nws_check(nws_forward_control(w, f0.data_ptr<float>(), control.data_ptr<float>(), (int)B, (int)C, (int)T, batched_gru ? 1 : 0,
-                                workspace.data_ptr(), (size_t)workspace.numel(), L.stream),
-            "nws_forward_control");
+  nws_check(nws_forward_control_noise(w, f0.data_ptr<float>(), control.data_ptr<float>(), fptr(noise), (int)B, (int)C, (int)T,
+                                      batched_gru ? 1 : 0, workspace.data_ptr(), (size_t)workspace.numel(), L.stream),
+            "nws_forward_control_noise");
 }
 
 Tensor forward_audio(const Tensor& wdesc, const Tensor& f0, const Tensor& phase_u, const Tensor& rand_phase, const Tensor& noise,
@@ -369,6 +375,38 @@
     nws_check(nws_fir_noise_window(fir.data_ptr<float>(), noise.data_ptr<float>(), (int)noise.numel(), (int)origin, fptr(add_in),
                                    (int)B, (int)T, out.data_ptr<float>(), L.stream), "nws_fir_noise_window");
   }
+  return out;
+}
+
+Tensor fir_noise_spectra(const Tensor& noise, int64_t T) {
+  check_dev(noise, "noise");
+  TORCH_CHECK(T >= 2 && T <= (1 << 23) && noise.numel() == T * NWS_HOP - 1, "noise: expected ", T * NWS_HOP - 1, " samples (T >= 2), got ",
+              noise.sizes());
+  Launch L(noise);
+  Tensor table = at::empty({(int64_t)(nws_fir_noise_spectra_bytes((int)T) / (4 * 9 * 16 * 4 * sizeof(float))), 4, 9, 16, 4}, noise.options());
+  nws_check(nws_fir_noise_spectra(noise.data_ptr<float>(), (int)noise.numel(), NWS_FIR_LEN / 2, (int)T, table.data_ptr<float>(), L.stream),
+            "nws_fir_noise_spectra");
+  return table;
+}
+
+Tensor fir_noise_tabled(const Tensor& fir, const Tensor& table, const OptTensor& add_in) {
+  check_dev(fir, "fir");
+  check_dev(table, "table");
+  check_same_device(fir, "fir", table, "table");
+  TORCH_CHECK(fir.dim() == 3 && fir.size(2) == NWS_FIR_HALF, "fir: expected (B, T, 128) upper half-taps (nws_frame_mlps), got ", fir.sizes());
+  const int64_t B = fir.size(0), T = fir.size(1);
+  TORCH_CHECK(B >= 16, "fir_noise_tabled: the kernel that reads noise spectra serves B >= 16, got B = ", B);
+  TORCH_CHECK((size_t)table.numel() * sizeof(float) == nws_fir_noise_spectra_bytes((int)T), "table: expected the ",
+              nws_fir_noise_spectra_bytes((int)T), " bytes of fir_noise_spectra for T = ", T, ", got ", table.sizes());
+  if (add_in.has_value()) {
+    check_dev(*add_in, "add_in");
+    check_same_device(fir, "fir", *add_in, "add_in");
+    TORCH_CHECK(add_in->numel() == B * T * NWS_HOP, "add_in: expected (", B, ", ", T * NWS_HOP, "), got ", add_in->sizes());
+  }
+  Launch L(fir);
+  Tensor out = at::empty({B, T * NWS_HOP}, fir.options());
+  nws_check(nws_fir_noise_tabled(fir.data_ptr<float>(), table.data_ptr<float>(), fptr(add_in), (int)B, (int)T, out.data_ptr<float>(),
+                                 L.stream), "nws_fir_noise_tabled");
   return out;
 }
 
@@ -1292,7 +1330,7 @@
   m.def("abi_version() -> int", &abi_version);
   m.def("forward(Tensor wdesc, Tensor f0, Tensor control, Tensor phase_u, Tensor rand_phase, Tensor noise, Tensor fir_design, "
         "Tensor plan, Tensor reverb_tables, Tensor reverb_spectrum, Tensor(a!) workspace, float sample_rate) -> Tensor", &forward);
-  m.def("forward_control(Tensor wdesc, Tensor f0, Tensor control, Tensor(a!) workspace, bool batched_gru) -> ()", &forward_control);
+  m.def("forward_control(Tensor wdesc, Tensor f0, Tensor control, Tensor? noise, Tensor(a!) workspace, bool batched_gru) -> ()", &forward_control);
   m.def("forward_audio(Tensor wdesc, Tensor f0, Tensor phase_u, Tensor rand_phase, Tensor noise, Tensor fir_design, Tensor plan, "
         "Tensor reverb_tables, Tensor reverb_spectrum, Tensor(a!) workspace, float sample_rate, Tensor? out, int wait_event, "
         "int record_event) -> Tensor", &forward_audio);
@@ -1311,6 +1349,8 @@
   m.def("frame_mlps(Tensor wdesc, Tensor gru_out, Tensor fir_design, bool want_emb, bool want_H) -> (Tensor, Tensor, Tensor, Tensor)",
         &frame_mlps);
   m.def("fir_noise(Tensor fir, Tensor noise, Tensor? add_in, int origin) -> Tensor", &fir_noise);
+  m.def("fir_noise_spectra(Tensor noise, int T) -> Tensor", &fir_noise_spectra);
+  m.def("fir_noise_tabled(Tensor fir, Tensor table, Tensor? add_in) -> Tensor", &fir_noise_tabled);
   m.def("fir_from_h(Tensor H, Tensor fir_design) -> Tensor", &fir_from_h);
   m.def("fir_noise_grad(Tensor noise, Tensor grad_out) -> Tensor", &fir_noise_grad);
   m.def("fir_from_h_grad(Tensor grad_fir, Tensor fir_design) -> Tensor", &fir_from_h_grad);
diff --git a/neural-waveshaping-synthesis_amd/engine.py b/neural-waveshaping-synthesis_amd/engine.py
--- a/neural-waveshaping-synthesis_amd/engine.py
+++ b/neural-waveshaping-synthesis_amd/engine.py
@@ -438,6 +438,13 @@
         emb, film, H, fir = binding().frame_mlps(r.wdesc, gru_out, r.fir_design, want_emb, want_H)
         return (emb if want_emb else None), film, (H if want_H else None), fir
 
+    def fir_noise_spectra(self, noise, T):
+        return binding().fir_noise_spectra(noise, int(T))
+
+    def fir_noise_tabled(self, fir, table, add_in=None):
+        same_device(fir.device, table=table, add_in=add_in)
+        return binding().fir_noise_tabled(fir, table, add_in)
+
     def fir_noise(self, fir, noise, add_in=None, origin=None, noise_len=None):
         same_device(fir.device, noise=noise, add_in=add_in)
         nz = noise if noise_len is None or noise_len == noise.numel() else noise[:noise_len]
@@ -472,10 +479,10 @@
         plan, _, _, _ = self._reverb_aux(T * _lib.HOP)
         return torch.empty(_lib.lib().nws_forward_workspace_bytes(C.byref(plan), B, T), dtype=torch.uint8, device=dev)
 
-    def forward_control(self, f0, control, ws, batched_gru=True):
-        r = self._wd()
-        same_device(r.device, f0=f0, control=control, workspace=ws)
-        binding().forward_control(r.wdesc, f0, control, ws, bool(batched_gru))
+    def forward_control(self, f0, control, ws, batched_gru=True, noise=None):
+        r = self._wd()
+        same_device(r.device, f0=f0, control=control, workspace=ws, noise=noise)
+        binding().forward_control(r.wdesc, f0, control, noise, ws, bool(batched_gru))
 
     def forward_audio(self, f0, B, T, phase_u, noise, ws, out=None, wait_event=None, record_event=None, row_blocks=None,
                       on_block=None, block_events=None):
diff --git a/neural-waveshaping-synthesis_amd/pipeline.py b/neural-waveshaping-synthesis_amd/pipeline.py
--- a/neural-waveshaping-synthesis_amd/pipeline.py
+++ b/neural-waveshaping-synthesis_amd/pipeline.py
@@ -320,7 +320,7 @@
             pu = _req(pu.reshape(-1), "phase_u", _lib.N_HARMONICS)
             nz = torch.rand(m.control_hop * T - 1, out=slot.nz, generator=generator) if noise is None else noise
             nz = _req(nz, "noise", m.control_hop * T - 1)
-            self.eng.forward_control(f0, control, slot.ws, batched_gru=batched)
+            self.eng.forward_control(f0, control, slot.ws, batched_gru=batched, noise=nz)
             slot.ev_control.record(cs)
         with torch.cuda.stream(au):
             au.wait_event(ready)
```
